# HuiyangYu/TGSFilter

Hardware: AMD Instinct MI355X
Metric: filtered Gbases/sec (end-to-end, excl. gzip I/O) (higher is better)
Workload: dtype u8

## Files before the change

include/tgsf.h:

```cpp
#ifndef TGSF_H
#define TGSF_H

#include <stddef.h>
#include <stdint.h>

#ifdef __cplusplus
extern "C" {
#endif

#define TGSF_ABI_VERSION 3
#define TGSF_MAX_ADAPTERS 32
#define TGSF_MAX_ADAPTER_LEN 8192
#define TGSF_N_DROPINFO 17
#define TGSF_N_QBINS 256
#define TGSF_BIN_WIDTH 100

typedef enum tgsf_status {
    TGSF_OK = 0,
    TGSF_E_INVALID = -1,
    TGSF_E_NO_DEVICE = -2,
    TGSF_E_HIP = -3,
    TGSF_E_CAPACITY = -4,
    TGSF_E_UNSUPPORTED = -5,
    TGSF_E_DATA = -6
} tgsf_status;

typedef struct tgsf_params {
    uint32_t struct_size;
    int32_t  min_len;
    int32_t  max_len;
    float    min_q;
    float    max_q;
    int32_t  bc_len;
    int32_t  head_trim;
    int32_t  tail_trim;
    int32_t  end_len;
    int32_t  end_match_len;
    int32_t  mid_match_len;
    int32_t  extra_len;
    float    end_sim;
    float    mid_sim;
    int32_t  discard;
    int32_t  filter;
    int32_t  only_qc;
    int32_t  min_repeat;
    int32_t  kmer;
    int32_t  qtype;
    int32_t  n_adapters;
    const char* adapters[TGSF_MAX_ADAPTERS];
    int32_t  adapter_len[TGSF_MAX_ADAPTERS];
    uint64_t max_batch_bases;
    uint32_t max_batch_reads;
    uint32_t max_read_len;
    int32_t  no_qual;
    int32_t  reserved;
} tgsf_params;

typedef struct tgsf_batch_in {
    const uint8_t*  seq;
    const uint8_t*  qual;
    const uint64_t* offsets;
    const uint32_t* lengths;
    uint32_t        n_reads;
    uint32_t        reserved;
    uint64_t        n_bytes;
    const uint64_t* qual_offsets;
} tgsf_batch_in;

#define TGSF_RF_LOWQ       0x01u
#define TGSF_RF_AD5P       0x02u
#define TGSF_RF_AD3P       0x04u
#define TGSF_RF_ADMID      0x08u
#define TGSF_RF_DISCARDED  0x10u

typedef struct tgsf_read_result {
    uint64_t sum_q;
    uint32_t flags;
    uint32_t n_frags;
    uint32_t frag_begin;
    uint32_t trimmed;
    int32_t  reserved0;
    int32_t  reserved1;
} tgsf_read_result;

#define TGSF_FF_PASS    0x01u
#define TGSF_FF_REPEAT  0x02u

typedef struct tgsf_fragment {
    uint64_t sum_q;
    uint32_t read;
    int32_t  start;
    int32_t  len;
    uint32_t flags;
} tgsf_fragment;

typedef struct tgsf_batch_out {
    tgsf_read_result* reads;
    tgsf_fragment*    frags;
    uint32_t          frag_capacity;
    uint32_t          n_frags;
} tgsf_batch_out;

#define TGSF_CTR_DROPINFO    0
#define TGSF_CTR_RAW_DIFFQ   17
#define TGSF_CTR_CLEAN_DIFFQ 273
#define TGSF_CTR_ROWS        529
#define TGSF_CTR_END_TABLES  533

enum { TGSF_T_RAW5P_QUAL = 0, TGSF_T_RAW5P_CNT, TGSF_T_RAW3P_QUAL, TGSF_T_RAW3P_CNT,
       TGSF_T_CLEAN5P_QUAL, TGSF_T_CLEAN5P_CNT, TGSF_T_CLEAN3P_QUAL, TGSF_T_CLEAN3P_CNT };
enum { TGSF_B_RAW_QUAL = 0, TGSF_B_RAW_CNT, TGSF_B_CLEAN_QUAL, TGSF_B_CLEAN_CNT };

static inline size_t tgsf_ctr_end_table(int t, int bc_len) {
    return (size_t)TGSF_CTR_END_TABLES + (size_t)t * (size_t)bc_len * 5u;
}
static inline size_t tgsf_ctr_bin_table(int b, int bc_len, uint32_t n_bins) {
    return (size_t)TGSF_CTR_END_TABLES + 8u * (size_t)bc_len * 5u + (size_t)b * (size_t)n_bins * 5u;
}
static inline size_t tgsf_ctr_len(int bc_len, uint32_t n_bins) {
    return tgsf_ctr_bin_table(4, bc_len, n_bins);
}
static inline uint32_t tgsf_n_bins(uint32_t max_read_len) { return max_read_len / TGSF_BIN_WIDTH + 1u; }

typedef struct tgsf_ctx tgsf_ctx;

int tgsf_abi_version(void);

const char* tgsf_backend(void);

int tgsf_prepare_device(int device);

int tgsf_device_location(int device, char* bus_id, int len, int* numa_node);

int tgsf_create(const tgsf_params* params, int device, tgsf_ctx** out_ctx);
void tgsf_destroy(tgsf_ctx* ctx);

int tgsf_submit(tgsf_ctx* ctx, const tgsf_batch_in* in, tgsf_batch_out* out);
int tgsf_submit_async(tgsf_ctx* ctx, const tgsf_batch_in* in, tgsf_batch_out* out);

#define TGSF_MAX_ENQUEUED 64
#define TGSF_NFRAGS_NOT_FINAL 0xFFFFFFFFu
int tgsf_submit_device(tgsf_ctx* ctx, const tgsf_batch_in* in, tgsf_batch_out* out,
                       uint32_t* d_n_frags, void* hip_stream);

int tgsf_wait(tgsf_ctx* ctx);

int tgsf_counters_len(tgsf_ctx* ctx, uint64_t* n_words, int32_t* bc_len, uint32_t* n_bins);
int tgsf_counters(tgsf_ctx* ctx, uint64_t* dst, uint64_t n_words);
int tgsf_counters_used(tgsf_ctx* ctx, uint64_t* dst, uint64_t n_words, uint64_t rows[2]);
int tgsf_counters_merge(tgsf_ctx* dst, tgsf_ctx* src);
int tgsf_counters_device(tgsf_ctx* ctx, void** d_ptr, uint64_t* n_words);
int tgsf_reset_counters(tgsf_ctx* ctx);

#define TGSF_N_STAGES 12
int tgsf_profile(tgsf_ctx* ctx, int enable);
int tgsf_stage_times(tgsf_ctx* ctx, float ms[TGSF_N_STAGES], uint32_t* n_batches);
const char* tgsf_stage_name(int stage);

int tgsf_align_windows(tgsf_ctx* ctx, const uint8_t* seq, uint64_t n_bytes,
                       const uint64_t* win_off, const uint32_t* win_len,
                       const uint8_t* adapter_id, const int32_t* k, uint32_t n,
                       int32_t* res, int32_t* ends);

const char* tgsf_last_error(tgsf_ctx* ctx);

#ifdef __cplusplus
}
#endif
#endif
```

tgsfilter_amd/capi.py:

```python
from __future__ import annotations

import ctypes as C
import os

import numpy as np

from . import abi

_HERE = os.path.dirname(os.path.abspath(__file__))
DEFAULT_LIB = os.path.join(_HERE, "libtgsf.so")
_LIBS = {}

SYMBOLS = [
    "tgsf_abi_version", "tgsf_backend", "tgsf_prepare_device", "tgsf_device_location", "tgsf_create", "tgsf_destroy", "tgsf_submit", "tgsf_submit_async", "tgsf_submit_device",
    "tgsf_wait",
    "tgsf_counters_len", "tgsf_counters", "tgsf_counters_used", "tgsf_counters_merge", "tgsf_counters_device", "tgsf_reset_counters", "tgsf_profile",
    "tgsf_stage_times", "tgsf_stage_name", "tgsf_align_windows", "tgsf_last_error",
]


class TgsfError(RuntimeError):
    def __init__(self, code, msg):
        super().__init__(f"tgsf error {code}: {msg}")
        self.code = code


def load(path: str | None = None):
    explicit = path is not None
    path = path or os.environ.get("TGSF_LIB") or DEFAULT_LIB
    if path in _LIBS:
        if not explicit and not _LIBS[path].tgsf_backend().startswith(b"hip"):
            raise RuntimeError(f"{path} is not the HIP build of libtgsf (there is no CPU fallback; is TGSF_LIB set by accident?)")
        return _LIBS[path]
    if not os.path.exists(path):
        raise FileNotFoundError(
            f"{path} not found: build the HIP extension first (python -c 'import __graft_entry__ as g; g.build()')")
    L = C.CDLL(path)
    vp, u32, u64, i32 = C.c_void_p, C.c_uint32, C.c_uint64, C.c_int32
    L.tgsf_abi_version.restype = C.c_int
    L.tgsf_backend.restype = C.c_char_p
    L.tgsf_prepare_device.argtypes = [C.c_int]
    L.tgsf_device_location.argtypes = [C.c_int, C.c_char_p, C.c_int, C.POINTER(C.c_int)]
    L.tgsf_create.argtypes = [C.POINTER(abi.Params), C.c_int, C.POINTER(vp)]
    L.tgsf_destroy.argtypes = [vp]
    L.tgsf_destroy.restype = None
    L.tgsf_submit.argtypes = [vp, C.POINTER(abi.BatchIn), C.POINTER(abi.BatchOut)]
    L.tgsf_submit_async.argtypes = [vp, C.POINTER(abi.BatchIn), C.POINTER(abi.BatchOut)]
    L.tgsf_submit_device.argtypes = [vp, C.POINTER(abi.BatchIn), C.POINTER(abi.BatchOut), vp, vp]
    L.tgsf_wait.argtypes = [vp]
    L.tgsf_counters_len.argtypes = [vp, C.POINTER(u64), C.POINTER(i32), C.POINTER(u32)]
    L.tgsf_counters.argtypes = [vp, vp, u64]
    L.tgsf_counters_used.argtypes = [vp, vp, u64, vp]
    L.tgsf_counters_merge.argtypes = [vp, vp]
    L.tgsf_counters_device.argtypes = [vp, C.POINTER(vp), C.POINTER(u64)]
    L.tgsf_reset_counters.argtypes = [vp]
    L.tgsf_profile.argtypes = [vp, C.c_int]
    L.tgsf_stage_times.argtypes = [vp, C.POINTER(C.c_float * abi.N_STAGES), C.POINTER(u32)]
    L.tgsf_stage_name.argtypes = [C.c_int]
    L.tgsf_stage_name.restype = C.c_char_p
    L.tgsf_align_windows.argtypes = [vp, vp, u64, vp, vp, vp, vp, u32, vp, vp]
    L.tgsf_last_error.argtypes = [vp]
    L.tgsf_last_error.restype = C.c_char_p
    if L.tgsf_abi_version() != abi.ABI_VERSION:
        raise RuntimeError("libtgsf ABI version mismatch")
    if not explicit and not L.tgsf_backend().startswith(b"hip"):
        raise RuntimeError(f"{path} is the {L.tgsf_backend().decode()!r} build of libtgsf, not the HIP build "
                           "(there is no CPU fallback; is TGSF_LIB set by accident?)")
    _LIBS[path] = L
    return L


class Context:

    def __init__(self, params: abi.Params, device: int = 0, lib_path: str | None = None):
        self.lib = load(lib_path)
        self.params = params
        h = C.c_void_p()
        rc = self.lib.tgsf_create(C.byref(params), device, C.byref(h))
        if rc != 0:
            raise TgsfError(rc, self.lib.tgsf_last_error(None).decode())
        self.h = h
        nw, bc, nb = C.c_uint64(), C.c_int32(), C.c_uint32()
        self._chk(self.lib.tgsf_counters_len(self.h, C.byref(nw), C.byref(bc), C.byref(nb)))
        self.ctr_words, self.bc_len, self.n_bins = nw.value, bc.value, nb.value

    def _chk(self, rc):
        if rc != 0:
            raise TgsfError(rc, self.lib.tgsf_last_error(self.h).decode())

    def close(self):
        if getattr(self, "h", None):
            self.lib.tgsf_destroy(self.h)
            self.h = None

    def __del__(self):
        try:
            self.close()
        except Exception:
            pass

    def submit(self, seq, qual, offsets, lengths=None, frag_capacity=None, qual_offsets=None):
        self.submit_async(seq, qual, offsets, lengths, frag_capacity, qual_offsets)
        return self.wait_result()

    def submit_async(self, seq, qual, offsets, lengths=None, frag_capacity=None, qual_offsets=None):
        seq = np.ascontiguousarray(seq, dtype=np.uint8)
        qual = np.ascontiguousarray(qual, dtype=np.uint8)
        offsets = np.ascontiguousarray(offsets, dtype=np.uint64)
        if lengths is not None:
            lengths = np.ascontiguousarray(lengths, dtype=np.uint32)
            n = len(lengths)
            total = int(lengths.sum())
        else:
            n = len(offsets) - 1
            total = int(offsets[-1] - offsets[0])
        if frag_capacity is None:
            frag_capacity = total // 100 + n + 16
        reads = np.zeros(n, dtype=abi.READ_RESULT_DTYPE)
        frags = np.zeros(frag_capacity, dtype=abi.FRAGMENT_DTYPE)
        if qual_offsets is not None:
            qual_offsets = np.ascontiguousarray(qual_offsets, dtype=np.uint64)
        same = qual is seq or (qual.ctypes.data == seq.ctypes.data)
        bi = abi.BatchIn(seq.ctypes.data, seq.ctypes.data if same else qual.ctypes.data, offsets.ctypes.data,
                         lengths.ctypes.data if lengths is not None else None, n, 0, seq.size,
                         qual_offsets.ctypes.data if qual_offsets is not None else None)
        bo = abi.BatchOut(reads.ctypes.data, frags.ctypes.data, frag_capacity, 0)
        self._pending = (reads, frags, bi, bo, seq, qual, offsets, lengths, qual_offsets)
        rc = self.lib.tgsf_submit_async(self.h, C.byref(bi), C.byref(bo))
        if rc != 0:
            self._pending = None
            self._chk(rc)

    def wait_result(self):
        pend, self._pending = self._pending, None
        if pend is None:
            raise RuntimeError("no batch pending")
        self._chk(self.lib.tgsf_wait(self.h))
        reads, frags, _, bo = pend[:4]
        return reads, frags[:bo.n_frags].copy()

    def submit_device(self, d_seq, d_qual, d_offsets, d_lengths, n_reads, n_bytes, d_reads, d_frags,
                      frag_capacity, d_nfrags=None, stream=None, d_qual_offsets=None):
        bi = abi.BatchIn(d_seq, d_qual, d_offsets, d_lengths, n_reads, 0, n_bytes, d_qual_offsets)
        bo = abi.BatchOut(d_reads, d_frags, frag_capacity, 0)
        self._chk(self.lib.tgsf_submit_device(self.h, C.byref(bi), C.byref(bo), d_nfrags, stream))

    def wait(self):
        self._chk(self.lib.tgsf_wait(self.h))

    def counters(self) -> np.ndarray:
        out = np.zeros(self.ctr_words, dtype=np.uint64)
        self._chk(self.lib.tgsf_counters(self.h, out.ctypes.data, self.ctr_words))
        return out

    def counters_used(self, out=None, with_rows=True):
        if out is None:
            out = np.zeros(self.ctr_words, dtype=np.uint64)
        rows = (C.c_uint64 * 2)()
        self._chk(self.lib.tgsf_counters_used(self.h, out.ctypes.data, out.size, rows if with_rows else None))
        return out, ((rows[0], rows[1]) if with_rows else None)

    def merge_from(self, other: "Context"):
        self._chk(self.lib.tgsf_counters_merge(self.h, other.h))

    def counters_device_ptr(self):
        p, n = C.c_void_p(), C.c_uint64()
        self._chk(self.lib.tgsf_counters_device(self.h, C.byref(p), C.byref(n)))
        return p.value, n.value

    def reset_counters(self):
        self._chk(self.lib.tgsf_reset_counters(self.h))

    def profile(self, enable=True):
        self._chk(self.lib.tgsf_profile(self.h, int(enable)))

    def stage_times(self):
        arr = (C.c_float * abi.N_STAGES)()
        nb = C.c_uint32()
        self._chk(self.lib.tgsf_stage_times(self.h, C.byref(arr), C.byref(nb)))
        names = [self.lib.tgsf_stage_name(i).decode() for i in range(abi.N_STAGES)]
        return dict(zip(names, list(arr))), nb.value

    def align_windows(self, seq: bytes, win_off, win_len, adapter_id, k):
        seq = np.frombuffer(seq, dtype=np.uint8) if isinstance(seq, (bytes, bytearray)) else np.ascontiguousarray(seq, np.uint8)
        win_off = np.ascontiguousarray(win_off, dtype=np.uint64)
        win_len = np.ascontiguousarray(win_len, dtype=np.uint32)
        adapter_id = np.ascontiguousarray(adapter_id, dtype=np.uint8)
        k = np.ascontiguousarray(k, dtype=np.int32)
        n = len(win_off)
        res = np.zeros((n, 4), dtype=np.int32)
        ends = np.zeros((n, 2), dtype=np.int32)
        self._chk(self.lib.tgsf_align_windows(self.h, seq.ctypes.data, seq.size, win_off.ctypes.data,
                                              win_len.ctypes.data, adapter_id.ctypes.data, k.ctypes.data, n,
                                              res.ctypes.data, ends.ctypes.data))
        return res, ends
```

tgsfilter_amd/csrc/tgsf_emul.h:

```cpp
#pragma once
#include <stdint.h>
#include <string.h>

#define TGSF_HD inline
#define TGSF_D inline
#define TGSF_KERNEL static void
#define TGSF_INLINE_LAMBDA
#define TGSF_BOUNDS(threads, waves_per_simd)
#define TGSF_SHARED static thread_local
#define TGSF_BLOCK_SYNC() ((void)0)
#define TGSF_WAVE_SYNC() ((void)0)
#define TGSF_COOP_BEGIN 0u
#define TGSF_COOP_STRIDE 1u
#define TGSF_WCOOP_BEGIN(lane) 0u
#define TGSF_WCOOP_STRIDE 1u
#define TGSF_ON_DEVICE(...)
#define TGSF_ON_EMUL(...) __VA_ARGS__
constexpr bool kTgsfEmul = true;
#define TGSF_WAVE_PRIO(p) ((void)0)

struct alignas(16) uint4 { uint32_t x, y, z, w; };
namespace tgsf_emul {
struct Dim3 { unsigned x, y, z; };
extern thread_local Dim3 threadIdx, blockIdx, blockDim, gridDim;
}
using tgsf_emul::threadIdx; using tgsf_emul::blockIdx; using tgsf_emul::blockDim; using tgsf_emul::gridDim;
template <class T> static inline T atomicAdd(T* p, T v) { T o = *p; *p = o + v; return o; }
template <class T> static inline T atomicMax(T* p, T v) { T o = *p; if (v > o) *p = v; return o; }
template <class T> static inline T atomicMin(T* p, T v) { T o = *p; if (v < o) *p = v; return o; }
template <class T> static inline T atomicExch(T* p, T v) { T o = *p; *p = v; return o; }
template <class T> static inline T atomicOr(T* p, T v) { T o = *p; *p = o | v; return o; }
template <class T> static inline T atomicCAS(T* p, T cmp, T v) { T o = *p; if (o == cmp) *p = v; return o; }

namespace tgsf {

TGSF_HD uint32_t popc32(uint32_t x) { return (uint32_t)__builtin_popcount(x); }
TGSF_HD uint32_t popc64(uint64_t x) { return (uint32_t)__builtin_popcountll(x); }
TGSF_HD uint32_t udot4(uint32_t a, uint32_t b, uint32_t c) {
    uint32_t s = c;
    for (int i = 0; i < 4; i++) s += ((a >> (8 * i)) & 0xFF) * ((b >> (8 * i)) & 0xFF);
    return s;
}
TGSF_HD uint32_t alignbyte(uint32_t hi, uint32_t lo, uint32_t sh) { return (uint32_t)((((uint64_t)hi << 32) | lo) >> (8 * sh)); }
TGSF_HD uint32_t alignbit(uint32_t hi, uint32_t lo, uint32_t sh) { return (uint32_t)((((uint64_t)hi << 32) | lo) >> (sh & 31u)); }
TGSF_HD uint32_t perm_bytes(uint32_t hi, uint32_t lo, uint32_t sel) {
    uint64_t v = ((uint64_t)hi << 32) | lo;
    uint32_t r = 0;
    for (int i = 0; i < 4; i++) r |= (uint32_t)((v >> (8 * ((sel >> (8 * i)) & 7u))) & 0xFF) << (8 * i);
    return r;
}
template <int TT>
TGSF_HD uint32_t bitop3(uint32_t a, uint32_t b, uint32_t c) {
    uint32_t r = 0;
    for (int i = 0; i < 32; i++) {
        const int idx = (int)(((a >> i) & 1u) << 2 | ((b >> i) & 1u) << 1 | ((c >> i) & 1u));
        r |= (uint32_t)((TT >> idx) & 1) << i;
    }
    return r;
}
TGSF_HD void pin(uint64_t&) {}
TGSF_HD void pin(uint32_t&) {}
struct QcConsts { uint32_t k[4]; };
TGSF_HD QcConsts qc_consts() { return QcConsts{{0x41414141u, 0x54545454u, 0x47474747u, 0x43434343u}}; }
TGSF_HD uint32_t xad7f(uint32_t x7, uint32_t k) { return (x7 ^ k) + 0x7F7F7F7Fu; }
TGSF_HD uint4 load16u(const uint8_t* p) { uint4 v; memcpy(&v, p, 16); return v; }

TGSF_HD uint64_t wave_sum(uint64_t v) { return v; }
TGSF_HD int32_t wave_sum_i32(int32_t v) { return v; }
TGSF_HD uint32_t wave_max(uint32_t v) { return v; }
TGSF_HD uint32_t wave_or(uint32_t v) { return v; }
TGSF_HD bool wave_leader() { return true; }
TGSF_HD bool wave_any(bool b) { return b; }
TGSF_HD uint32_t wave_bcast(uint32_t v, uint32_t) { return v; }
TGSF_HD uint32_t wave_pick(uint32_t v, uint32_t) { return v; }

}
```

tgsfilter_amd/csrc/tgsf_hip.h:

```cpp
#pragma once
#include <hip/hip_runtime.h>
#include <stdint.h>

#define TGSF_HD __host__ __device__ __forceinline__
#define TGSF_D __device__ __forceinline__
#define TGSF_KERNEL __global__ void
#define TGSF_INLINE_LAMBDA __attribute__((always_inline))
#define TGSF_BOUNDS(threads, waves_per_simd) __launch_bounds__(threads, waves_per_simd)
#define TGSF_SHARED __shared__
#define TGSF_BLOCK_SYNC() __syncthreads()
#define TGSF_WAVE_SYNC() do { __builtin_amdgcn_fence(__ATOMIC_SEQ_CST, "wavefront"); __builtin_amdgcn_wave_barrier(); } while (0)
#define TGSF_COOP_BEGIN threadIdx.x
#define TGSF_COOP_STRIDE blockDim.x
#define TGSF_WCOOP_BEGIN(lane) (lane)
#define TGSF_WCOOP_STRIDE 64u
#define TGSF_ON_DEVICE(...) __VA_ARGS__
#define TGSF_ON_EMUL(...)
constexpr bool kTgsfEmul = false;
#define TGSF_WAVE_PRIO(p) __builtin_amdgcn_s_setprio(p)

namespace tgsf {

TGSF_HD uint32_t popc32(uint32_t x) { return (uint32_t)__builtin_popcount(x); }
TGSF_HD uint32_t popc64(uint64_t x) { return (uint32_t)__builtin_popcountll(x); }
TGSF_D uint32_t udot4(uint32_t a, uint32_t b, uint32_t c) { return __builtin_amdgcn_udot4(a, b, c, false); }
TGSF_D uint32_t alignbyte(uint32_t hi, uint32_t lo, uint32_t sh) { return __builtin_amdgcn_alignbyte(hi, lo, sh); }
TGSF_D uint32_t alignbit(uint32_t hi, uint32_t lo, uint32_t sh) { return __builtin_amdgcn_alignbit(hi, lo, sh); }
TGSF_D uint32_t perm_bytes(uint32_t hi, uint32_t lo, uint32_t sel) { return __builtin_amdgcn_perm(hi, lo, sel); }
template <int TT>
TGSF_D uint32_t bitop3(uint32_t a, uint32_t b, uint32_t c) { return __builtin_amdgcn_bitop3_b32(a, b, c, TT); }
TGSF_D void pin(uint64_t& v) { asm volatile("" : "+v"(v)); }
TGSF_D void pin(uint32_t& v) { asm volatile("" : "+v"(v)); }
struct QcConsts { uint32_t k[4]; };
TGSF_D QcConsts qc_consts() {
    QcConsts c;
    asm volatile("v_mov_b32 %0, 0x41414141" : "=v"(c.k[0]));
    asm volatile("v_mov_b32 %0, 0x54545454" : "=v"(c.k[1]));
    asm volatile("v_mov_b32 %0, 0x47474747" : "=v"(c.k[2]));
    asm volatile("v_mov_b32 %0, 0x43434343" : "=v"(c.k[3]));
    return c;
}
TGSF_D uint32_t xad7f(uint32_t x7, uint32_t k) {
    uint32_t t;
    const uint32_t c7f = 0x7F7F7F7Fu;
    asm("v_xad_u32 %0, %1, %2, %3" : "=v"(t) : "v"(x7), "v"(k), "s"(c7f));
    return t;
}
struct __attribute__((packed, aligned(1))) U4u { uint32_t x, y, z, w; };
TGSF_D uint4 load16u(const uint8_t* p) { const U4u* q = reinterpret_cast<const U4u*>(p); return make_uint4(q->x, q->y, q->z, q->w); }

TGSF_D uint64_t wave_sum(uint64_t v) {
#pragma unroll
    for (int o = 32; o > 0; o >>= 1) v += __shfl_xor(v, o, 64);
    return v;
}
TGSF_D int32_t wave_sum_i32(int32_t v) {
    v += __builtin_amdgcn_update_dpp(0, v, 0xB1, 0xF, 0xF, false);
    v += __builtin_amdgcn_update_dpp(0, v, 0x4E, 0xF, 0xF, false);
    v += __builtin_amdgcn_update_dpp(0, v, 0x141, 0xF, 0xF, false);
    v += __builtin_amdgcn_update_dpp(0, v, 0x140, 0xF, 0xF, false);
    v += __builtin_amdgcn_update_dpp(0, v, 0x142, 0xA, 0xF, false);
    v += __builtin_amdgcn_update_dpp(0, v, 0x143, 0xC, 0xF, false);
    return __builtin_amdgcn_readlane(v, 63);
}
TGSF_D uint32_t wave_max(uint32_t v) {
#pragma unroll
    for (int o = 32; o > 0; o >>= 1) { uint32_t u = __shfl_xor(v, o, 64); v = u > v ? u : v; }
    return v;
}
TGSF_D uint32_t wave_or(uint32_t v) {
#pragma unroll
    for (int o = 32; o > 0; o >>= 1) v |= __shfl_xor(v, o, 64);
    return v;
}
TGSF_D bool wave_leader() { return (threadIdx.x & 63u) == 0u; }
TGSF_D bool wave_any(bool b) { return __builtin_amdgcn_ballot_w64(b) != 0ull; }
TGSF_D uint32_t wave_bcast(uint32_t v, uint32_t src_lane) { return (uint32_t)__shfl((int)v, (int)src_lane, 64); }
TGSF_D uint32_t wave_pick(uint32_t v, uint32_t src_lane) { return (uint32_t)__builtin_amdgcn_readlane((int)v, (int)src_lane); }

}
```

tgsfilter_amd/csrc/tgsf_kernels.h:

```cpp
#pragma once
#include <type_traits>
#include "tgsf_dev.h"
#include "../../include/tgsf.h"
static_assert(TGSF_CTR_END_TABLES == 533, "tally layout");

namespace tgsf {

typedef unsigned long long ull;

TGSF_D void wave_add_u64(uint64_t* dst, uint64_t v) {
    uint64_t t = wave_sum(v);
    if (wave_leader() && t) atomicAdd((ull*)dst, (ull)t);
}
TGSF_D void wave_max_u64(uint64_t* dst, uint32_t v) {
    uint32_t t = wave_max(v);
    if (wave_leader() && t) atomicMax((ull*)dst, (ull)t);
}
TGSF_D void set_status(const DevBatch& B, uint32_t code, uint32_t detail) {
    if (atomicMax(&B.status[0], code) < code) B.status[1] = detail;
}

TGSF_D bool pool_overflowed(const DevBatch& B) { return *B.ovf != 0u; }

TGSF_D uint32_t stored_frags(const DevBatch& B) { uint32_t nf = B.nfr[B.n]; return nf < B.fcap ? nf : B.fcap; }
// ... 2075 lines not shown
    uint32_t f = next_s;
    prefetch(f);
    while (f < nf) {
        const uint4* base; int a, L;
        chunks_of(f, base, a, L);
        const int total = L - k + 1;
        const int words = (a + L + 15) / 16;
        const int kwords = total > 0 ? (a + total + 15) / 16 : 0;
        const bool one_window = words <= W;
        TGSF_BLOCK_SYNC();
        if (tid == 0) { over_s = 0; next_s = take(); }
        TGSF_BLOCK_SYNC();
        if (kTgsfEmul) load_window(base, words, 0);
        else {
#pragma unroll
            for (int sl = 0; sl < kRepSlots; sl++) { const int g = tid + sl * NT; if (g < words) codes[g] = base_codes16(raw[sl]); }
            if (tid < 8) codes[(words < W ? words : W) + tid] = 0;
        }
        TGSF_BLOCK_SYNC();
        const uint32_t fnext = next_s;
        prefetch(fnext);
        bool drop = false;
        if (total <= 0) {
            drop = 0 < P.min_repeat;
        } else if (k >= 32) {
            ull first = 0;
            const uint8_t* seq = B.seq + B.frag_off[f];
            for (int i = 0; i < k; i++) first = (first << 2) | base_code(seq[i]);
            const int distinct = (total > 1 && first != 0ull) ? 2 : 1;
            drop = total - distinct < P.min_repeat;
        } else {
            uint32_t plog = 0;
            uint32_t rot = 19u;
            while (plog < 20u && ((uint32_t)total >> plog) > kRepShare) plog++;
            for (;;) {
                const uint32_t passes = 1u << plog;
                uint32_t repeat = 0;
                uint32_t flagged = 0;
                bool decided = false;
                for (uint32_t pass = 0; pass < passes && !decided; pass++) {
                    uint32_t c0 = 0, c1 = 0;
                    auto scan = [&](auto phase_tag, auto multi_tag) TGSF_INLINE_LAMBDA {
                        constexpr int PHASE = decltype(phase_tag)::value;
                        constexpr bool MULTI = decltype(multi_tag)::value;
                        auto hash_of = [&](uint32_t x0, uint32_t x1) TGSF_INLINE_LAMBDA -> uint32_t {
                            return KEY64 ? ((x1 & tail_mask) ^ alignbit(x0, x0, rot)) * 0x9E3779B1u : x0 * 0x9E3779B1u;
                        };
                        auto owned = [&](uint32_t h) TGSF_INLINE_LAMBDA -> bool {
                            return !MULTI || ((h ^ (h >> 7)) & (passes - 1u)) == pass;
                        };
                        auto a_word = [&](uint32_t h) TGSF_INLINE_LAMBDA -> uint32_t { return ((h >> 16) * (kRepAQ * 4u)) >> 16; };
                        auto a_mask = [&](uint32_t h) TGSF_INLINE_LAMBDA -> uint32_t {
                            const uint32_t g = h ^ (h >> 15);
                            return (1u << (g & 31u)) | (1u << ((g >> 5) & 31u)) | (1u << ((g >> 10) & 31u));
                        };
                        for (int wb = 0;; wb += W - OV) {
                            if (!one_window) {
                                TGSF_BLOCK_SYNC();
                                load_window(base, words, wb);
                            }
                            TGSF_BLOCK_SYNC();
                            const bool last = wb + W >= words;
                            const int gend = last ? kwords - wb : W - OV;
                            for (int g = tid; g < gend; g += NT) {
                                const uint32_t w0 = codes[g], w1 = codes[g + 1], w2 = codes[g + 2];
                                const int first = a - 16 * (wb + g);
                                const int v = a + total - 16 * (wb + g);
                                uint32_t m = 0x55555555u;
                                if (first <= 0 && v >= 16) {
                                    m = 0;
#pragma unroll
                                    for (int j0 = 0; j0 < 16; j0 += 8) {
                                        uint32_t hv[8], oldv[8], mkv[8];
#pragma unroll
                                        for (int jj = 0; jj < 8; jj++) {
                                            const int j = j0 + jj;
                                            const uint32_t x0 = j ? alignbit(w0, w1, 32u - 2u * (uint32_t)j) : w0;
                                            uint32_t h;
                                            if (KEY64) {
                                                const uint32_t x1 = j ? alignbit(w1, w2, 32u - 2u * (uint32_t)j) : w1;
                                                h = hash_of(x0, x1);
                                            } else {
                                                h = hash_of(x0 >> (32 - kb), 0u);
                                            }
                                            hv[jj] = h;
                                            if (PHASE == 0) {
                                                mkv[jj] = owned(h) ? a_mask(h) : 0u;
                                                oldv[jj] = atomicOr(&Am[a_word(h)], mkv[jj]);
                                            } else {
                                                oldv[jj] = Bm[h >> 19];
                                            }
                                        }
                                        uint32_t hits = 0;
#pragma unroll
                                        for (int jj = 0; jj < 8; jj++) {
                                            bool hit;
                                            if (PHASE == 0) hit = (mkv[jj] & ~oldv[jj]) == 0u && (!MULTI || mkv[jj] != 0u);
                                            else hit = ((oldv[jj] >> ((hv[jj] >> 14) & 31u)) & 1u) && owned(hv[jj]);
                                            if (hit) hits |= 1u << (30 - 2 * (j0 + jj));
                                        }
                                        if (PHASE == 0) {
                                            if (hits) {
                                                c0 += popc32(hits);
#pragma unroll
                                                for (int jj = 0; jj < 8; jj++)
                                                    if (hits & (1u << (30 - 2 * (j0 + jj)))) atomicOr(&Bm[hv[jj] >> 19], 1u << ((hv[jj] >> 14) & 31u));
                                            }
                                        } else {
                                            m |= hits;
                                        }
                                    }
                                } else {
                                    if (first > 0) m &= 0xFFFFFFFFu >> (2 * first);
                                    if (v < 16) m &= ~(0xFFFFFFFFu >> (2 * v));
                                }
                                while (m) {
                                    const int b = __builtin_ctz(m);
                                    m &= m - 1u;
                                    const uint32_t sb = (uint32_t)(30 - b);
                                    const uint32_t x0 = sb ? alignbit(w0, w1, 32u - sb) : w0;
                                    key_t key;
                                    uint32_t lo32, hi32 = 0, h;
                                    if (KEY64) {
                                        const uint32_t x1 = sb ? alignbit(w1, w2, 32u - sb) : w1;
                                        const ull k64 = (((ull)x0 << 32) | x1) >> (64 - kb);
                                        key = (key_t)k64;
                                        lo32 = (uint32_t)k64; hi32 = (uint32_t)(k64 >> 32);
                                        h = hash_of(x0, x1);
                                    } else {
                                        lo32 = x0 >> (32 - kb);
                                        key = (key_t)lo32;
                                        h = hash_of(lo32, 0u);
                                    }
                                    if (!owned(h)) continue;
                                    const uint32_t bbit = 1u << ((h >> 14) & 31u);
                                    if (PHASE == 0) {
                                        const uint32_t mk = a_mask(h);
                                        const uint32_t old = atomicOr(&Am[a_word(h)], mk);
                                        if ((mk & ~old) == 0u) { c0++; atomicOr(&Bm[h >> 19], bbit); }
                                    } else if (Bm[h >> 19] & bbit) {
                                        c0++;
                                        uint32_t slot = (((lo32 * 0xC2B2AE35u) ^ (hi32 * 0x27D4EB2Fu) ^ (lo32 >> 15)) * 0x165667B1u) >> (32u - TLOG);
                                        for (int probes = 0;; probes++) {
                                            const key_t old = atomicCAS(&tab[slot], kEmpty, key);
                                            if (old == kEmpty) { c1++; break; }
                                            if (old == key) break;
                                            if (probes >= 64) { over_s = 1; break; }
                                            slot = (slot + 1u) & ((1u << TLOG) - 1u);
                                        }
                                    }
                                }
                            }
                            if (last) break;
                        }
                    };
                    if (tid == 0) acc_s[0] = acc_s[1] = acc_s[2] = 0;
                    if (plog == 0) scan(std::integral_constant<int, 0>(), std::false_type());
                    else scan(std::integral_constant<int, 0>(), std::true_type());
                    TGSF_BLOCK_SYNC();
                    flagged = block_sum(c0, 0);
                    const bool skip = flagged == 0 || (pass + 1 == passes && repeat + flagged < (uint32_t)P.min_repeat);
                    if (skip) {
                        if (flagged) repeat += flagged;
                        TGSF_BLOCK_SYNC();
                        clear_maps(flagged != 0);
                        TGSF_BLOCK_SYNC();
                        continue;
                    }
                    for (uint32_t w = (uint32_t)tid; w < kRepTabQ; w += (uint32_t)NT) A4[w] = ones4;
                    c0 = c1 = 0;
                    if (plog == 0) scan(std::integral_constant<int, 1>(), std::false_type());
                    else scan(std::integral_constant<int, 1>(), std::true_type());
                    TGSF_BLOCK_SYNC();
                    const uint32_t occ = block_sum(c0, 1), ins = block_sum(c1, 2);
                    clear_maps(true);
                    TGSF_BLOCK_SYNC();
                    if (over_s) break;
                    repeat += occ - ins;
                    if (repeat >= (uint32_t)P.min_repeat) decided = true;
                }
                if (!over_s) { drop = !decided && repeat < (uint32_t)P.min_repeat; break; }
                TGSF_BLOCK_SYNC();
                if (tid == 0) over_s = 0;
                uint32_t want = plog + 1u;
                while (want < B.rep_max_plog && (flagged >> (want - plog)) > (1u << (TLOG - 1u))) want++;
                if (plog >= B.rep_max_plog) {
                    const uint32_t distinct = rep_distinct_in_memory(B, B.seq + B.frag_off[f], total, k, tid, NT, &acc_s[0]);
                    drop = (uint32_t)total - distinct < (uint32_t)P.min_repeat;
                    break;
                }
                plog = want;
                rot = (rot + 6u) & 31u;
                TGSF_BLOCK_SYNC();
            }
        }
        if (tid == 0 && drop) {
            B.frag_flags[f] |= TGSF_FF_REPEAT;
            drop_n++; drop_b += (uint64_t)L;
        }
        f = fnext;
    }
    if (tid == 0 && drop_n) {
        atomicAdd((ull*)&B.ctr[TGSF_CTR_DROPINFO + 15], (ull)drop_n);
        atomicAdd((ull*)&B.ctr[TGSF_CTR_DROPINFO + 16], (ull)drop_b);
    }
}

TGSF_KERNEL k_gate_frags(DevParams P, DevBatch B)
{
    if (pool_overflowed(B)) return;
    TGSF_SHARED ull hq[TGSF_N_QBINS];
    for (uint32_t i = TGSF_COOP_BEGIN; i < (uint32_t)TGSF_N_QBINS; i += TGSF_COOP_STRIDE) hq[i] = 0;
    TGSF_BLOCK_SYNC();
    const uint32_t nf = stored_frags(B);
    const bool diff = clean_by_difference(B);
    uint64_t lq_n = 0, lq_b = 0;
    uint32_t erows = 0;
    for (uint32_t f0 = blockIdx.x * blockDim.x; f0 < nf; f0 += gsize()) {
        const uint32_t f = f0 + threadIdx.x;
        if (f >= nf || (B.frag_flags[f] & TGSF_FF_REPEAT)) continue;
        const uint32_t L = B.frag_len[f];
        if (diff && B.whole[B.frag_read[f]]) B.frag_sum[f] = clean_by_product(B) ? B.spec_sum[B.frag_read[f]] : B.sumq[B.frag_read[f]];
        const double cm = mean_q(B.frag_sum[f], L);
        if (!P.no_qual) {
            if (P.filter && q_fail(cm, P.min_q, P.max_q)) { lq_n++; lq_b += L; continue; }
            if (!(cm >= 0.0 && cm < 256.0)) { set_status(B, DS_BAD_MEANQ, B.frag_read[f]); continue; }
            atomicAdd(&hq[(int)cm], (ull)L);
        }
        B.frag_flags[f] = TGSF_FF_PASS;
        uint32_t er = (uint32_t)P.bc_len < L ? (uint32_t)P.bc_len : L;
        erows = er > erows ? er : erows;
    }
    wave_add_u64(&B.ctr[TGSF_CTR_DROPINFO + 13], lq_n);
    wave_add_u64(&B.ctr[TGSF_CTR_DROPINFO + 14], lq_b);
    wave_max_u64(&B.ctr[TGSF_CTR_ROWS + 3], erows);
    TGSF_BLOCK_SYNC();
    for (uint32_t i = TGSF_COOP_BEGIN; i < (uint32_t)TGSF_N_QBINS; i += TGSF_COOP_STRIDE)
        if (hq[i]) atomicAdd((ull*)&B.ctr[TGSF_CTR_CLEAN_DIFFQ + i], hq[i]);
}

TGSF_KERNEL k_ctr_merge(uint64_t* dst, const uint64_t* src, uint64_t n)
{
    for (uint64_t i = gtid(); i < n; i += gsize()) {
        const uint64_t a = dst[i], b = src[i];
        dst[i] = (i >= TGSF_CTR_ROWS && i < TGSF_CTR_ROWS + 4) ? (a > b ? a : b) : a + b;
    }
}

TGSF_KERNEL k_finalize(DevBatch B, tgsf_read_result* out_reads, tgsf_fragment* out_frags,
                       uint32_t out_fcap, uint32_t* out_nfrags)
{
    if (pool_overflowed(B)) {
        if (gtid() == 0 && out_nfrags) *out_nfrags = TGSF_NFRAGS_NOT_FINAL;
        return;
    }
    const uint32_t nf = B.nfr[B.n];
    if (gtid() == 0) {
        if (out_nfrags) *out_nfrags = nf;
        if (nf > out_fcap) set_status(B, DS_FRAG_CAP, nf);
    }
    for (uint32_t r = gtid(); r < B.n; r += gsize()) {
        tgsf_read_result o;
        o.sum_q = B.sumq[r];
        o.flags = B.flags[r];
        o.n_frags = B.nfr[r + 1] - B.nfr[r];
        o.frag_begin = B.nfr[r];
        o.trimmed = B.trimmed[r];
        o.reserved0 = 0; o.reserved1 = 0;
        out_reads[r] = o;
    }
    for (uint32_t f = gtid(); f < nf && f < out_fcap; f += gsize()) {
        tgsf_fragment o;
        o.sum_q = B.frag_sum[f];
        o.read = B.frag_read[f];
        o.start = B.frag_start[f];
        o.len = (int32_t)B.frag_len[f];
        o.flags = B.frag_flags[f];
        out_frags[f] = o;
    }
}

template <int MAXNW>
TGSF_KERNEL k_align_windows(DevParams P, DevBatch B, const uint8_t* seq, const uint64_t* win_off, const uint32_t* win_len,
                            const uint8_t* adapter_id, const int32_t* kk, uint32_t n, int32_t* res, int32_t* ends)
{
    const uint32_t i = gtid();
    if (i >= n) return;
    const int a = adapter_id[i];
    const int Q = P.Q[a];
    int k = kk[i];
    if (k > Q) k = Q;
    const LaneScratch sc = lane_scratch(B, 0);
    const uint8_t* t = seq + win_off[i];
    const int T = (int)win_len[i];
    WinAln w = by_length<MAXNW>(Q, [=, &P](auto f) TGSF_INLINE_LAMBDA { return align_window<typename decltype(f)::col>(P, a, t, T, k, 0, sc, true); });
    res[i * 4 + 0] = w.best;
    res[i * 4 + 1] = w.best < 0 ? 0 : w.n;
    res[i * 4 + 2] = w.best < 0 ? 0 : w.mlen + w.best;
    res[i * 4 + 3] = w.best < 0 ? -1 : w.start0;
    ends[i * 2 + 0] = w.best < 0 ? -1 : w.first_end;
    ends[i * 2 + 1] = w.best < 0 ? -1 : w.last_end;
}

}
```

tgsfilter_amd/csrc/tgsf_lib.hip:

```cpp
#include <algorithm>
#include <type_traits>

#include "tgsf_kernels.h"
constexpr size_t kErrorCap = 512;
#include "tgsf_rt.h"
#if defined(TGSF_EMUL)
namespace tgsf_emul { thread_local Dim3 threadIdx, blockIdx, blockDim, gridDim; }
#endif

using namespace tgsf;

static const char* knob(const char* name)
{
    static const bool on = [] { const char* e = getenv("TGSF_DEBUG_KNOBS"); return e && e[0] == '1'; }();
    return on ? getenv(name) : nullptr;
}

struct tgsf_ctx : rt_ctx {
    tgsf_params params;
    std::vector<std::string> adapters;
    DevParams P;
    DevBatch B;
    rt_stream stream;
    rt_stream last_stream;
    bool own_stream;
    uint64_t cap_bases, cap_chunks;
    uint32_t cap_reads, max_read_len, n_bins;
    static constexpr unsigned endtab_grid = 512;
    static constexpr unsigned stats_grid = 768;
    bool flat_scan = true;
    int suffix_filter = 2;
    bool no_hot32 = false;
    uint64_t ctr_words;
    int scratch_cols;
    uint8_t *d_seq, *d_qual;
    uint64_t* d_off;
    uint64_t* d_qoff;
    uint32_t* d_lenin;
    tgsf_read_result* d_out_reads;
    tgsf_fragment* d_out_frags;
    uint32_t* d_out_nfrags;
    bool profile;
    float stage_ms[TGSF_N_STAGES];
    uint32_t prof_batches;
    static constexpr int kProfRing = 64;
    rt_event ev[kProfRing][TGSF_N_STAGES + 1];
    rt_event ev_aux[kProfRing][3];
    int prof_pending;
    rt_stream aux;
    rt_event ev_fork, ev_join;
    uint32_t* h_pinned = nullptr;
    static constexpr size_t kStageBytes = 32u << 20;
    uint8_t* stage[2] = {nullptr, nullptr};
    rt_event stage_ev[2] = {nullptr, nullptr};
    uint32_t h_words_[8];
    uint32_t* h_status;
    uint32_t* pend_nf_p;
    tgsf_batch_out* pend_out = nullptr;
    struct Pending { tgsf_batch_in in; tgsf_read_result* reads; tgsf_fragment* frags; uint32_t fcap; uint32_t* nfrags; rt_stream st; };
    Pending pending[TGSF_MAX_ENQUEUED];
    uint32_t n_pending = 0;
    uint32_t* ovf_ring = nullptr;
    uint32_t* bp_ring = nullptr;
    uint32_t h_ovf[TGSF_MAX_ENQUEUED];
    uint32_t pool_regrown = 0;
};

static const int kMaxLenParam = 1 << 28;
static void adapter_rules(const tgsf_params& p, DevParams& P)
{
    P.max_nw = 1;
    P.min_Q = 1 << 30;
    for (int a = 0; a < p.n_adapters; a++) {
        const int Q = p.adapter_len[a];
        P.Q[a] = Q;
        if (Q > 64 && P.max_nw < 2) P.max_nw = 2;
        if (Q > 128 && P.max_nw < 4) P.max_nw = 4;
        if (Q > 256) P.max_nw = kWideNW;
        if (Q < P.min_Q) P.min_Q = Q;
        int km = Q - p.mid_match_len + 1;
        int ke = Q - p.end_match_len + 1;
        P.k_mid[a] = km > Q - 1 ? Q - 1 : km;
        P.k_end[a] = ke > Q - 1 ? Q - 1 : ke;
        const float w = (float)Q / p.end_sim;
        P.w5[a] = p.end_len + (w < (float)kMaxLenParam ? (int)w : kMaxLenParam);
        P.need_end[a] = P.need_mid[a] = Q + 1;
        for (int m = Q; m >= 0; m--) {
            if (m >= p.end_match_len && (float)m / (float)Q >= p.end_sim) P.need_end[a] = m;
            if (m >= p.mid_match_len && (float)m / (float)Q >= p.mid_sim) P.need_mid[a] = m;
        }
    }
}

static void fill_peq(const std::vector<std::string>& adapters, size_t slots, int W, std::vector<uint64_t>& fwd, std::vector<uint64_t>& rev)
{
    const size_t per_ad = (size_t)256 * W;
    fwd.assign(slots * per_ad, 0);
    rev.assign(slots * per_ad, 0);
    for (size_t a = 0; a < adapters.size(); a++) {
        const std::string& s = adapters[a];
        const int Q = (int)s.size();
        for (int r = 0; r < Q && r < 64 * W; r++) {
            const uint8_t cf = (uint8_t)s[r], cr = (uint8_t)s[Q - 1 - r];
            fwd[a * per_ad + (size_t)cf * W + (r >> 6)] |= 1ull << (r & 63);
            rev[a * per_ad + (size_t)cr * W + (r >> 6)] |= 1ull << (r & 63);
        }
    }
}

static int build_tables(tgsf_ctx* c)
{
    DevParams& P = c->P;
    const int A = c->params.n_adapters;
    std::vector<uint8_t> ad((size_t)kMaxAdapters * kMaxQ, 0);
    std::vector<uint64_t> fwd, rev, top((size_t)kMaxAdapters * 256, 0);
    fill_peq(c->adapters, kMaxAdapters, kPeqW, fwd, rev);
    for (int a = 0; a < A; a++) {
        const int Q = P.Q[a];
        memcpy(&ad[(size_t)a * kMaxQ], c->adapters[a].data(), (size_t)Q);
        if (Q <= 64) {
            const int sh = 64 - Q;
            const uint64_t pad = sh ? ((1ull << sh) - 1ull) : 0ull;
            for (int sym = 0; sym < 256; sym++)
                top[(size_t)a * 256 + sym] = (fwd[((size_t)a * 256 + sym) * kPeqW] << sh) | pad;
        }
    }
    uint8_t* d_ad; uint64_t *d_f, *d_r, *d_t;
    int e;
    if ((e = dev_alloc(c, &d_ad, ad.size()))) return e;
    if ((e = dev_alloc(c, &d_f, fwd.size()))) return e;
    if ((e = dev_alloc(c, &d_r, rev.size()))) return e;
    if ((e = dev_alloc(c, &d_t, top.size()))) return e;
    rt_h2d(d_ad, ad.data(), ad.size(), c->stream);
    rt_h2d(d_f, fwd.data(), fwd.size() * 8, c->stream);
    rt_h2d(d_r, rev.data(), rev.size() * 8, c->stream);
    rt_h2d(d_t, top.data(), top.size() * 8, c->stream);
    rt_sync(c->stream);
    P.adapter = d_ad; P.peq_fwd = d_f; P.peq_rev = d_r; P.peq_top = d_t;
    P.peq_fwd_w = P.peq_rev_w = nullptr;
    if (P.max_nw > 4) {
        fill_peq(c->adapters, (size_t)A, kWideNW, fwd, rev);
        uint64_t *d_fw, *d_rw;
        if ((e = dev_alloc(c, &d_fw, fwd.size()))) return e;
        if ((e = dev_alloc(c, &d_rw, rev.size()))) return e;
        rt_h2d(d_fw, fwd.data(), fwd.size() * 8, c->stream);
        rt_h2d(d_rw, rev.data(), rev.size() * 8, c->stream);
        rt_sync(c->stream);
        P.peq_fwd_w = d_fw; P.peq_rev_w = d_rw;
    }
    return 0;
}

extern "C" int tgsf_abi_version(void) { return TGSF_ABI_VERSION; }
extern "C" const char* tgsf_backend(void) { return kTgsfEmul ? "emulation" : "hip:gfx950"; }

#if !defined(TGSF_EMUL)
__global__ void k_noop(int* p) { if (p) *p = 0; }
static void set_wait_mode(int device)
{
    const char* e = getenv("TGSF_SYNC");
    if (!e || strcmp(e, "blocking") != 0) return;
    if (hipSetDevice(device) == hipSuccess) { (void)hipSetDeviceFlags(hipDeviceScheduleBlockingSync); (void)hipGetLastError(); }
}
#endif
extern "C" int tgsf_prepare_device(int device)
{
#if !defined(TGSF_EMUL)
    int ndev = 0;
    if (hipGetDeviceCount(&ndev) != hipSuccess || device < 0 || device >= ndev) return TGSF_E_NO_DEVICE;
    set_wait_mode(device);
    if (hipSetDevice(device) != hipSuccess) return TGSF_E_HIP;
    hipLaunchKernelGGL(k_noop, dim3(1), dim3(64), 0, 0, (int*)nullptr);
    if (hipDeviceSynchronize() != hipSuccess) return TGSF_E_HIP;
    {
        static const char a0[] = "GTTTTCGCATTTATCGTGAAACGCTTTCGCGTTTTTCGTGCGCCGCTTCA";
        static const char a1[] = "TGAAGCGGCGCACGAAAAACGCGAAAGCGTTTCACGATAAATGCGAAAAC";
        tgsf_params p;
        memset(&p, 0, sizeof p);
        p.struct_size = sizeof p;
        p.min_len = 100; p.max_len = 2147483647; p.min_q = 0; p.max_q = 255; p.bc_len = 150;
        p.end_len = 150; p.end_match_len = 4; p.mid_match_len = 35; p.extra_len = 50;
        p.end_sim = 0.75f; p.mid_sim = 0.9f; p.filter = 1; p.qtype = 33; p.kmer = 11;
        p.n_adapters = 2; p.adapters[0] = a0; p.adapters[1] = a1; p.adapter_len[0] = p.adapter_len[1] = 50;
        p.max_batch_bases = 1 << 16; p.max_batch_reads = 16; p.max_read_len = 1 << 14;
        tgsf_ctx* c = nullptr;
        if (tgsf_create(&p, device, &c) == TGSF_OK) {
            std::vector<uint8_t> seq(8192), qual(8192, (uint8_t)'5');
            for (size_t i = 0; i < seq.size(); i++) seq[i] = "ACGT"[(i * 2654435761u >> 13) & 3];
            memcpy(&seq[4096 + 1000], a0, 50);
            const uint64_t off[2] = {0, 4096};
            const uint32_t len[2] = {3000, 4000};
            tgsf_read_result res[2];
            tgsf_fragment fr[64];
            tgsf_batch_in in;
            memset(&in, 0, sizeof in);
            in.seq = seq.data(); in.qual = qual.data(); in.offsets = off; in.lengths = len; in.n_reads = 2; in.n_bytes = seq.size();
            tgsf_batch_out out{res, fr, 64, 0};
            (void)tgsf_submit(c, &in, &out);
            tgsf_destroy(c);
        }
    }
#else
    (void)device;
#endif
    return TGSF_OK;
}

extern "C" int tgsf_device_location(int device, char* bus_id, int len, int* numa_node)
{
    if (numa_node) *numa_node = -1;
    if (bus_id && len > 0) bus_id[0] = 0;
#if !defined(TGSF_EMUL)
    int ndev = 0;
    if (hipGetDeviceCount(&ndev) != hipSuccess || device < 0 || device >= ndev) return TGSF_E_NO_DEVICE;
    char id[64] = {0};
    if (hipDeviceGetPCIBusId(id, (int)sizeof id, device) != hipSuccess) return TGSF_E_HIP;
    for (char* p = id; *p; p++) if (*p >= 'A' && *p <= 'F') *p = (char)(*p - 'A' + 'a');
    if (bus_id && len > 0) { strncpy(bus_id, id, (size_t)len - 1); bus_id[len - 1] = 0; }
    if (numa_node) {
        const std::string path = std::string("/sys/bus/pci/devices/") + id + "/numa_node";
        if (FILE* f = fopen(path.c_str(), "r")) {
            int v = -1;
            if (fscanf(f, "%d", &v) == 1) *numa_node = v;
            fclose(f);
        }
    }
    return TGSF_OK;
#else
    if (bus_id && len > 0) snprintf(bus_id, (size_t)len, "emul:%d", device);
    if (numa_node)
        if (const char* e = knob("TGSF_EMUL_NUMA")) {
            int k = 0;
            for (const char* c = e; *c; k++) {
                if (k == device) { *numa_node = atoi(c); break; }
                while (*c && *c != ',') c++;
                if (*c == ',') c++;
            }
        }
    return TGSF_OK;
#endif
}

extern "C" const char* tgsf_last_error(tgsf_ctx* ctx) { return ctx ? ctx->error.c_str() : g_create_error.c_str(); }

extern "C" void tgsf_destroy(tgsf_ctx* c)
{
    if (!c) return;
    if (c->B.bp_allowed && c->B.bp_state && knob("TGSF_TRACE_BP")) {
        uint32_t w[4] = {0, 0, 0, 0};
        uint64_t pl[4] = {0, 0, 0, 0};
        uint32_t sg[4] = {0, 0, 0, 0};
        if (!rt_d2h(w, c->B.bp_state, sizeof w, c->stream) && !rt_d2h(pl, c->B.plan, sizeof pl, c->stream) && !rt_d2h(sg, c->B.seg_info, sizeof sg, c->stream) && !rt_sync(c->stream))
            fprintf(stderr, "tgsf: clean tables as a by-product of the raw pass: %u batches speculated; the next would%s; the last batch: %llu bases a direct clean pass scans, "
                            "%llu bases its own did, %u work items in that pass\n", w[1], w[0] ? "" : " not", (unsigned long long)pl[2], (unsigned long long)pl[3], sg[2]);
    }
    if (c->stream) { (void)rt_set_device(c->device); (void)rt_sync(c->stream); }
    for (int k = 0; k < tgsf_ctx::kProfRing; k++) {
        for (rt_event e : c->ev[k]) rt_event_destroy(e);
        for (rt_event e : c->ev_aux[k]) rt_event_destroy(e);
    }
    if (c->h_pinned) rt_host_free(c->h_pinned);
    for (int i = 0; i < 2; i++) {
        if (c->stage[i]) rt_host_free(c->stage[i]);
        rt_event_destroy(c->stage_ev[i]);
    }
    rt_event_destroy(c->ev_fork);
    rt_event_destroy(c->ev_join);
    if (c->aux) rt_stream_destroy(c->aux);
    if (c->own_stream && c->stream) rt_stream_destroy(c->stream);
    dev_free_all(c);
    delete c;
}

static int check_params(const tgsf_params* p)
{
    if (p->struct_size != sizeof(tgsf_params))
        return fail(nullptr, TGSF_E_INVALID, "tgsf_params.struct_size %u != %zu (ABI mismatch)", p->struct_size, sizeof(tgsf_params));
    if (p->n_adapters < 0 || p->n_adapters > TGSF_MAX_ADAPTERS)
        return fail(nullptr, TGSF_E_INVALID, "n_adapters %d outside [0,%d]", p->n_adapters, TGSF_MAX_ADAPTERS);
    if (p->min_repeat > 0 && (p->kmer < 1 || p->kmer > 32))
        return fail(nullptr, TGSF_E_UNSUPPORTED, "kmer (-k) %d: the repeat gate supports k-mer sizes 1..32 (the reference's k-mers are 64 bits)", p->kmer);
    if (p->min_len < 0) return fail(nullptr, TGSF_E_INVALID, "min_len (-l) %d: must be >= 0", p->min_len);
    if (p->end_len > kMaxLenParam) return fail(nullptr, TGSF_E_INVALID, "end_len (-E) %d: must be <= 2^28", p->end_len);
    if (p->extra_len > kMaxLenParam) return fail(nullptr, TGSF_E_INVALID, "extra_len (-T) %d: must be <= 2^28", p->extra_len);
    if (p->qtype != 33 && p->qtype != 64) return fail(nullptr, TGSF_E_INVALID, "qtype must be 33 or 64");
    if (p->bc_len < 0 || p->bc_len > kMaxBcLenTotal) return fail(nullptr, TGSF_E_INVALID, "bc_len (-e) outside [0,%d]", kMaxBcLenTotal);
    if (p->filter && p->n_adapters > 0) {
        if (!(p->end_sim > 0.f)) return fail(nullptr, TGSF_E_INVALID, "end_sim must be > 0");
        if (!(p->mid_sim > 0.f)) return fail(nullptr, TGSF_E_INVALID, "mid_sim must be > 0");
        if (p->end_len < 0) return fail(nullptr, TGSF_E_INVALID, "end_len must be >= 0");
        if (p->extra_len < 0) return fail(nullptr, TGSF_E_INVALID, "extra_len must be >= 0");
        if (p->end_match_len < 1) return fail(nullptr, TGSF_E_INVALID, "end_match_len must be >= 1");
        if (p->mid_match_len < 1) return fail(nullptr, TGSF_E_INVALID, "mid_match_len must be >= 1");
    }
    for (int a = 0; a < p->n_adapters; a++) {
        if (!p->adapters[a] || p->adapter_len[a] < 1 || p->adapter_len[a] > TGSF_MAX_ADAPTER_LEN)
            return fail(nullptr, TGSF_E_UNSUPPORTED, "adapter %d: length %d outside [1,%d]", a, p->adapter_len[a], TGSF_MAX_ADAPTER_LEN);
    }
    if (!p->max_batch_bases) return fail(nullptr, TGSF_E_INVALID, "max_batch_bases must be set");
    if (!p->max_batch_reads) return fail(nullptr, TGSF_E_INVALID, "max_batch_reads must be set");
    if (!p->max_read_len) return fail(nullptr, TGSF_E_INVALID, "max_read_len must be set");
    if (p->max_read_len > (1u << 28)) return fail(nullptr, TGSF_E_INVALID, "max_read_len above 2^28");
    return TGSF_OK;
}

struct Sizing {
    DevBatch B;
    uint64_t cap_bytes, cap_chunks;
    size_t nitems, scratch_waves;
    int scratch_cols, seg_cols, suffix_filter;
    bool flat_scan, no_hot32;
};

static Sizing size_context(const tgsf_params& p, const DevParams& P)
{
    Sizing S;
    DevBatch& B = S.B;
    memset(&B, 0, sizeof B);
    S.seg_cols = kSegCols; S.no_hot32 = false; S.flat_scan = true; S.suffix_filter = 2;
    if (const char* e = knob("TGSF_NO_HOT32")) S.no_hot32 = atoi(e) > 0;
    if (const char* e = knob("TGSF_SEG_COLS")) { int v = atoi(e); if (v >= 256 && v <= 65536) S.seg_cols = v & ~15; }
    if (const char* e = knob("TGSF_MID_FLAT")) S.flat_scan = atoi(e) > 0;
    if (const char* e = knob("TGSF_MID_FILTER")) { int v = atoi(e); if (v >= 0 && v <= 2) S.suffix_filter = v; }
    B.flat_pmax = 256; B.flat_pmin = 16; B.flat_f0 = 224;
    if (const char* e = knob("TGSF_FLAT_PMIN")) { int v = atoi(e); if (v >= 1 && v <= (1 << 20)) B.flat_pmin = (uint32_t)v; }
    if (const char* e = knob("TGSF_FLAT_PMAX")) { int v = atoi(e); if (v >= 1 && v <= (1 << 20)) B.flat_pmax = (uint32_t)v; }
    if (const char* e = knob("TGSF_FLAT_F0")) { int v = atoi(e); if (v >= 0 && v <= 256) B.flat_f0 = (uint32_t)v; }
    B.flat_pmin = 1u << flat_log2(B.flat_pmin); B.flat_pmax = 1u << flat_log2(B.flat_pmax);
    if (B.flat_pmax < B.flat_pmin) B.flat_pmax = B.flat_pmin;
    const uint64_t cap_bases = p.max_batch_bases;
    const size_t n = p.max_batch_reads;
    const int A = p.n_adapters > 0 ? p.n_adapters : 1;
    S.cap_bytes = cap_bases + 16ull * n + 64;
    const int min_len = p.min_len > 0 ? p.min_len : 1;
    uint64_t fcap64 = p.filter ? (cap_bases / (uint64_t)min_len + 16) : (uint64_t)n + 16;
    if (fcap64 > cap_bases + 16) fcap64 = cap_bases + 16;
    if (fcap64 < n + 16 && !p.filter) fcap64 = n + 16;
    B.fcap = (uint32_t)std::min<uint64_t>(fcap64, 0x7FFFFFF0ull);
    B.max_tiles = (p.max_read_len + kTileBases - 1) / kTileBases;
    uint64_t pool = cap_bases / 64 + 65536 + (uint64_t)n * 16u * (uint64_t)A;
    B.pool_cap = (uint32_t)std::min<uint64_t>(pool, 1ull << 28);
    if (const char* e = knob("TGSF_POOL_CAP")) { const long long v = atoll(e); if (v >= 1 && v < (1ll << 28)) B.pool_cap = (uint32_t)v; }
    S.nitems = n + (size_t)B.fcap;
    S.cap_chunks = cap_bases / 16u + 2ull * n;
    if (S.cap_chunks >= 0xFFFFFFF0ull) S.flat_scan = false;
    if (S.cap_chunks >= (1ull << 30) || !S.flat_scan) S.suffix_filter = 0;
    bool any = false;
    for (int a = 0; a < p.n_adapters; a++) any |= P.Q[a] > 32 && P.Q[a] <= 64 && P.k_mid[a] >= 0 && P.k_mid[a] <= kSuffixMaxK;
    if (!any || !p.filter) S.suffix_filter = 0;
    if (S.suffix_filter) {
        B.rc_cap = (uint32_t)std::min<uint64_t>(S.cap_chunks / 25u + 4096u, 1ull << 24);
        if (const char* e = knob("TGSF_RECHECK_CAP")) { int v = atoi(e); if (v >= 0) B.rc_cap = (uint32_t)v; }
    }
    B.rep_long_cap = (uint32_t)std::min<uint64_t>((cap_bases + 16ull * n) / kRepShare + 16, (uint64_t)B.fcap + 16);
    if (p.min_repeat > 0 && p.kmer >= 12 && p.kmer <= 31) {
        B.rep_tab_log2 = 4;
        while (B.rep_tab_log2 < 40 && (1ull << B.rep_tab_log2) < 2ull * p.max_read_len) B.rep_tab_log2++;
        B.rep_max_plog = kRepMaxPlog;
        if (const char* e = knob("TGSF_REP_MAX_PLOG")) { int v = atoi(e); if (v >= 0 && v <= 20) B.rep_max_plog = (uint32_t)v; }
    }
    B.work_cap = (uint32_t)std::min<uint64_t>(2 * (cap_bases / kTileBases) + S.nitems + 16, 0x7FFFFFF0ull);
    B.clean_force = p.only_qc ? 1u : 0u;
    B.bp_allowed = (p.filter && !p.only_qc && (p.head_trim > 0 || p.tail_trim > 0) &&
                    p.head_trim >= 0 && p.tail_trim >= 0) ? 1u : 0u;
    static_assert(kTileBases < (1 << 13), "staged bytes of a tile fit the work list's 13 bits");
    if (const char* f = knob("TGSF_CLEAN_TABLES")) {
        if (!strcmp(f, "direct")) { B.clean_force = 1; B.bp_allowed = 0; }
        else if (!strcmp(f, "difference") && !p.only_qc) { B.clean_force = 2; B.bp_allowed = 0; }
        else if (!strcmp(f, "byproduct") && B.bp_allowed) B.clean_force = 3;
    }
    int maxcols = 1;
    for (int a = 0; a < p.n_adapters; a++) {
        int kmax = std::max(std::max(P.k_end[a], P.k_mid[a]), 0);
        maxcols = std::max(maxcols, P.Q[a] + std::min(P.Q[a], kmax) + 1);
    }
    S.scratch_cols = maxcols;
    int col_words = P.max_nw;
    if (P.max_nw > 4) { col_words = 1; for (int a = 0; a < p.n_adapters; a++) col_words = std::max(col_words, (P.Q[a] + 63) / 64); }
    size_t lane_words = (size_t)(maxcols + 1) * 2 * (size_t)col_words;
    if (P.max_nw > 4) lane_words = std::min<size_t>(lane_words, (1u << 17) + 2 * (size_t)col_words) + 4 * (size_t)col_words + 64;
    B.scratch_wave_words = lane_words * 64;
    B.scratch_mid_wave0 = ((size_t)n * A * 2 + 63) / 64 + 1;
    S.scratch_waves = B.scratch_mid_wave0 + ((size_t)n * A + 63) / 64 + 1;
    return S;
}

static int bring_up(tgsf_ctx* c)
{
    c->h_status = c->h_words_; c->pend_nf_p = c->h_words_ + 4;
#if !defined(TGSF_EMUL)
    int ndev = 0;
    hipError_t he = hipGetDeviceCount(&ndev);
    if (he != hipSuccess || ndev <= 0)
        return fail(nullptr, TGSF_E_NO_DEVICE, "no HIP device available (%s); libtgsf has no CPU fallback", hipGetErrorString(he));
    if (c->device < 0 || c->device >= ndev) return fail(nullptr, TGSF_E_NO_DEVICE, "device %d out of range (%d devices)", c->device, ndev);
    set_wait_mode(c->device);
    if ((he = hipSetDevice(c->device)) != hipSuccess) return fail(nullptr, TGSF_E_HIP, "hipSetDevice: %s", hipGetErrorString(he));
    if ((he = hipStreamCreateWithFlags(&c->stream, hipStreamNonBlocking)) != hipSuccess) return fail(nullptr, TGSF_E_HIP, "hipStreamCreate: %s", hipGetErrorString(he));
    c->own_stream = true;
    uint32_t* pw = nullptr;
    if (hipHostMalloc((void**)&pw, 64, hipHostMallocDefault) == hipSuccess && pw) {
        memset(pw, 0, 64);
        c->h_pinned = pw; c->h_status = pw; c->pend_nf_p = pw + 4;
    }
    int lo = 0, hi = 0;
    (void)hipDeviceGetStreamPriorityRange(&lo, &hi);
    he = hipStreamCreateWithPriority(&c->aux, hipStreamNonBlocking, hi);
    if (he != hipSuccess ||
        (he = hipEventCreateWithFlags(&c->ev_fork, hipEventDisableTiming)) != hipSuccess ||
        (he = hipEventCreateWithFlags(&c->ev_join, hipEventDisableTiming)) != hipSuccess)
        return fail(nullptr, TGSF_E_HIP, "auxiliary stream: %s", hipGetErrorString(he));
    if (c->params.max_batch_bases > (8u << 20)) {
        for (int i = 0; i < 2; i++)
            if (hipHostMalloc((void**)&c->stage[i], tgsf_ctx::kStageBytes, hipHostMallocDefault) != hipSuccess ||
                hipEventCreateWithFlags(&c->stage_ev[i], hipEventDisableTiming) != hipSuccess)
                return fail(nullptr, TGSF_E_HIP, "pinned staging buffers: allocation failed");
    }
#endif
    c->last_stream = c->stream;
    return TGSF_OK;
}

static int allocate(tgsf_ctx* c, const Sizing& S)
{
    DevBatch& B = c->B;
    const size_t n = c->cap_reads;
    const int A = std::max(c->params.n_adapters, 1);
    const size_t tiles = 2 * ((size_t)B.max_tiles + 2);
    int e = 0;
    if (!e) e = dev_alloc(c, &c->d_seq, S.cap_bytes);
    if (!e) e = dev_alloc(c, &c->d_qual, S.cap_bytes);
    if (!e) e = dev_alloc(c, &c->d_off, n + 1);
    if (!e) e = dev_alloc(c, &c->d_qoff, n + 1);
    if (!e) e = dev_alloc(c, &c->d_lenin, n);
    if (!e) e = dev_alloc(c, &B.len, n);
    if (!e) e = dev_alloc(c, &B.sumq, n);
    if (!e) e = dev_alloc(c, &B.flags, n);
    if (!e) e = dev_alloc(c, &B.clip5, n * A);
    if (!e) e = dev_alloc(c, &B.clip3, n * A);
    if (!e) e = dev_alloc(c, &B.mid_head, n);
    if (!e) e = dev_alloc(c, &B.mid_best, n * A);
    if (!e) e = dev_alloc(c, &B.mid_cnt, n);
    if (!e) e = dev_alloc(c, &B.mid_gate, n * A);
    if (!e) e = dev_alloc(c, &B.pool, (size_t)B.pool_cap);
    if (!e) e = dev_alloc(c, &B.pool_n, 4);
    if (!e) e = dev_alloc(c, &B.seg_cnt, n + 1);
    if (!e) e = dev_alloc(c, &B.chk_cnt, n + 1);
    if (c->suffix_filter) {
        if (!e) e = dev_alloc(c, &B.chk_mark, (size_t)4 * (size_t)(S.cap_chunks / 32u + 8u));
        if (!e) e = dev_alloc(c, &B.rc_list, (size_t)B.rc_cap + 1);
        if (!e) e = dev_alloc(c, &B.rc_n, 4);
    }
    if (!e) e = dev_alloc(c, &B.nfr, n + 1);
    if (!e) e = dev_alloc(c, &B.scan_part, n / kScanTile + 2);
    if (!e) e = dev_alloc(c, &B.trimmed, n);
    if (!e) e = dev_alloc(c, &B.rep_next, 2 + (size_t)B.rep_long_cap);
    if (B.rep_tab_log2) {
        if (!e) e = dev_alloc(c, &B.rep_tab, (size_t)1 << B.rep_tab_log2);
        if (!e) e = dev_alloc(c, &B.rep_lock, 4);
        if (!e) rt_memset(B.rep_lock, 0, 16, c->stream);
    }
    if (!e) e = dev_alloc(c, &B.tile_hist, tiles);
    if (!e) e = dev_alloc(c, &B.tile_cnt, tiles);
    if (!e) e = dev_alloc(c, &B.tile_base, tiles);
    if (!e) e = dev_alloc(c, &B.tile_fill, tiles);
    if (!e) e = dev_alloc(c, &B.seg_info, 4);
    if (!e) e = dev_alloc(c, &B.perm, S.nitems);
    if (!e) e = dev_alloc(c, &B.work, 2 * (size_t)B.work_cap);
    if (!e) e = dev_alloc(c, &B.frag_off, (size_t)B.fcap);
    if (!e) e = dev_alloc(c, &B.frag_qoff, (size_t)B.fcap);
    if (!e) e = dev_alloc(c, &B.frag_len, (size_t)B.fcap);
    if (!e) e = dev_alloc(c, &B.frag_sum, (size_t)B.fcap);
    if (!e) e = dev_alloc(c, &B.frag_read, (size_t)B.fcap);
    if (!e) e = dev_alloc(c, &B.frag_start, (size_t)B.fcap);
    if (!e) e = dev_alloc(c, &B.frag_flags, (size_t)B.fcap);
    if (!e) e = dev_alloc(c, &B.raw_tab, 2 * (size_t)c->n_bins * 5);
    if (!e) e = dev_alloc(c, &B.whole, n);
    if (!e) e = dev_alloc(c, &B.plan, 4);
    if (B.bp_allowed) {
        if (!e) e = dev_alloc(c, &B.spec, n);
        if (!e) e = dev_alloc(c, &B.spec_sum, n);
        if (!e) e = dev_alloc(c, &B.bp_state, 4);
        if (!e) e = dev_alloc(c, &c->bp_ring, TGSF_MAX_ENQUEUED);
    }
    if (!e) e = dev_alloc(c, &B.scratch, S.scratch_waves * B.scratch_wave_words);
    if (!e) e = dev_alloc(c, &B.ctr, (size_t)c->ctr_words);
    if (!e) e = dev_alloc(c, &B.status, 4);
    if (!e) e = dev_alloc(c, &c->ovf_ring, TGSF_MAX_ENQUEUED);
    if (!e) e = dev_alloc(c, &c->d_out_reads, n);
    if (!e) e = dev_alloc(c, &c->d_out_frags, (size_t)B.fcap);
    if (!e) e = dev_alloc(c, &c->d_out_nfrags, 4);
    if (e) return e;
    rt_memset(B.ctr, 0, c->ctr_words * 8, c->stream);
    rt_memset(B.status, 0, 16, c->stream);
    rt_memset(c->ovf_ring, 0, TGSF_MAX_ENQUEUED * 4, c->stream);
    B.ovf = c->ovf_ring;
    if (B.bp_allowed) {
        const uint32_t init[4] = {1u, 0u, 0u, 0u};
        rt_memset(c->bp_ring, 0, TGSF_MAX_ENQUEUED * 4, c->stream);
        (void)rt_h2d(B.bp_state, init, sizeof init, c->stream);
        B.bp_used = c->bp_ring;
    }
    rt_memset(B.raw_tab, 0, 2 * (size_t)c->n_bins * 5 * 8, c->stream);
    rt_sync(c->stream);
    return TGSF_OK;
}

extern "C" int tgsf_create(const tgsf_params* p, int device, tgsf_ctx** out)
{
    if (!p || !out) return fail(nullptr, TGSF_E_INVALID, "null argument");
    *out = nullptr;
    int e = check_params(p);
    if (e) return e;
    tgsf_ctx* c = new tgsf_ctx();
    c->alloc_slack = 64;
    c->params = *p;
    c->device = device;
    for (int a = 0; a < p->n_adapters; a++) {
        c->adapters.emplace_back(p->adapters[a], (size_t)p->adapter_len[a]);
        c->params.adapters[a] = c->adapters.back().data();
    }
    DevParams& P = c->P;
    P.min_len = p->min_len; P.max_len = p->max_len; P.min_q = p->min_q; P.max_q = p->max_q;
    P.bc_len = p->bc_len; P.head_trim = p->head_trim; P.tail_trim = p->tail_trim; P.end_len = p->end_len;
    P.end_match_len = p->end_match_len; P.mid_match_len = p->mid_match_len; P.extra_len = p->extra_len;
    P.end_sim = p->end_sim; P.mid_sim = p->mid_sim; P.discard = p->discard; P.filter = p->filter;
    P.only_qc = p->only_qc; P.qtype = p->qtype; P.n_adapters = p->n_adapters;
    P.no_qual = p->no_qual ? 1 : 0;
    P.min_repeat = p->min_repeat; P.kmer = p->kmer;
    c->cap_bases = p->max_batch_bases;
    c->cap_reads = p->max_batch_reads;
    c->max_read_len = p->max_read_len;
    c->n_bins = tgsf_n_bins(p->max_read_len);
    P.n_bins = c->n_bins;
    c->ctr_words = tgsf_ctr_len(p->bc_len, c->n_bins);
    adapter_rules(*p, P);
    const Sizing S = size_context(*p, P);
    c->B = S.B; c->cap_chunks = S.cap_chunks; c->scratch_cols = S.scratch_cols; P.seg_cols = S.seg_cols;
    c->flat_scan = S.flat_scan; c->suffix_filter = S.suffix_filter; c->no_hot32 = S.no_hot32;

    if ((e = bring_up(c)) || (e = build_tables(c)) || (e = allocate(c, S))) {
        if (!c->error.empty()) g_create_error = c->error;
        tgsf_destroy(c);
        return e;
    }
    *out = c;
    return TGSF_OK;
}

static const char* kStageNames[TGSF_N_STAGES] = {
    "prepare+sort", "stats_raw", "gate_reads", "end_tables_raw", "end_windows", "mid_scan",
    "mid_resolve", "regions", "repeat_gate", "stats_clean", "gate_frags+end_tables_clean", "finalize"};

extern "C" const char* tgsf_stage_name(int s) { return (s >= 0 && s < TGSF_N_STAGES) ? kStageNames[s] : ""; }

static unsigned blocks_for(uint64_t n, unsigned block) { return (unsigned)std::max<uint64_t>(1, (n + block - 1) / block); }

static int harvest_profile(tgsf_ctx* c, rt_stream st)
{
    if (!c->prof_pending) return TGSF_OK;
    const int he = rt_sync(st);
    if (he) return fail(c, TGSF_E_HIP, "stream synchronize failed: %s", rt_errstr(he));
    (void)rt_sync(c->aux);
    for (int k = 0; k < c->prof_pending; k++)
        for (int i = 0; i < TGSF_N_STAGES; i++) {
            float ms = 0.f;
            const int e = (i == 3 || i == 4) ? rt_event_ms(&ms, c->ev_aux[k][i - 3], c->ev_aux[k][i - 2])
                                             : rt_event_ms(&ms, c->ev[k][i], c->ev[k][i + 1]);
            if (!e) c->stage_ms[i] += ms;
        }
    c->prof_pending = 0;
    return TGSF_OK;
}

template <int V> using int_c = std::integral_constant<int, V>;

template <class F>
static void with_width(int max_nw, F&& f)
{
    if (max_nw > 4) f(int_c<kWideNW>());
    else if (max_nw > 2) f(int_c<4>());
    else f(int_c<2>());
}

template <int MAXNA, class F>
static void with_adapters(int na, F&& f)
{
    static_assert(MAXNA == 2 || MAXNA == 4, "a pass takes up to two or up to four adapters");
    if (na == 1) return f(int_c<1>());
    if constexpr (MAXNA == 4) {
        if (na == 3) return f(int_c<3>());
        if (na != 2) return f(int_c<4>());
    }
    f(int_c<2>());
}

static void scan_u32(const DevBatch& B, uint32_t* a, uint32_t n, rt_stream st, uint32_t* part = nullptr)
{
    if (!part) part = B.scan_part;
    const unsigned nb = (n + kScanTile - 1) / kScanTile;
    TGSF_LAUNCH_COOP(k_scan_tiles, nb, 256, st, a, n, part);
    TGSF_LAUNCH_COOP(k_scan_top, 1, 64, st, part, (uint32_t)nb, a + n);
    TGSF_LAUNCH_COOP(k_scan_add, nb, 256, st, a, n, (const uint32_t*)part);
}

static int drain_pending(tgsf_ctx* c, bool implicit = false);

struct Run {
    tgsf_ctx* c;
    const tgsf_batch_in* in;
    DevBatch B;
    rt_stream st, ax;
    bool redo, profile;
    rt_event *evs, *evx;
    int stage, A;
    uint32_t n;
    unsigned gsmall, gstats, gfold, gwork, gfr;
    size_t tl;
    bool flat;
    unsigned gflat, gseg;
    uint64_t flat_chunks, max_segs;
};
static constexpr unsigned kBlock = 256;
static_assert(kMidThreads == kBlock, "k_mid_flat / k_mid_scan1 are launched with kBlock lanes a workgroup");

static void stage_mark(Run& r)
{
    if (r.profile) (void)rt_event_record(r.evs[r.stage], r.st);
    r.stage++;
}

static void stage_prepare(Run& r)
{
    const DevParams& P = r.c->P; const DevBatch& B = r.B; const rt_stream st = r.st;
    rt_memset(B.ovf, 0, 4, st);
    rt_memset(B.tile_hist, 0, r.tl, st);
    rt_memset(B.tile_fill, 0, r.tl, st);
    rt_memset(B.pool_n, 0, 4, st);
    rt_memset(B.plan, 0, 32, st);
    TGSF_LAUNCH(k_prepare, r.gsmall, kBlock, st, P, B, r.c->max_read_len);
    TGSF_LAUNCH_COOP(k_tile_scan, 1, 64, st, B, B.bp_allowed ? 2u : 1u);
    TGSF_LAUNCH(k_tile_scatter<false>, r.gsmall, kBlock, st, P, B);
    TGSF_LAUNCH(k_build_work<false>, r.gwork, kBlock, st, P, B);
}

static void stage_raw_stats(Run& r)
{
    const DevParams& P = r.c->P; const DevBatch& B = r.B; const rt_stream st = r.st;
    if (B.bp_allowed) {
        TGSF_LAUNCH((k_stats<false, true, true>), r.gstats, 64 * kStatsWaves, st, P, B);
        if (P.tail_trim > 0) TGSF_LAUNCH(k_tail_fix, grid_cap(std::min(blocks_for(r.n, 1024), 128u)), 1024, st, P, B);
    } else TGSF_LAUNCH((k_stats<false, true>), r.gstats, 64 * kStatsWaves, st, P, B);
    if (!r.redo) TGSF_LAUNCH(k_fold_raw<false>, r.gfold, kBlock, st, P, B);
}

static void stage_fork_ends(Run& r)
{
    tgsf_ctx* c = r.c;
    const DevParams& P = c->P; const DevBatch& B = r.B; const rt_stream ax = r.ax;
    (void)rt_event_record(c->ev_fork, r.st);
    (void)rt_stream_wait(ax, c->ev_fork);
    if (r.profile) (void)rt_event_record(r.evx[0], ax);
    for (uint32_t slab = 0; !r.redo && slab * (uint32_t)kMaxBcLen < (uint32_t)P.bc_len; slab++)
        TGSF_LAUNCH(k_end_tables<false>, grid_cap(c->endtab_grid), 64 * kEndWaves, ax, P, B, slab);
    if (r.profile) (void)rt_event_record(r.evx[1], ax);
    if (P.filter && r.A > 0)
        with_width(P.max_nw, [&](auto nw) { TGSF_LAUNCH(k_end_windows<decltype(nw)::value>, blocks_for((uint64_t)r.n * r.A * 2, 64), 64, ax, P, B); });
    if (r.profile) (void)rt_event_record(r.evx[2], ax);
    (void)rt_event_record(c->ev_join, ax);
}

static void launch_scans(Run& r, uint32_t mode)
{
    tgsf_ctx* c = r.c;
    const DevParams& P = c->P; const rt_stream ms = r.st;
    const int A = r.A;
    DevBatch Bm = r.B;
    Bm.mid_mode = mode;
    int a = 0;
    while (a < A) {
        if (P.Q[a] > 256) { TGSF_LAUNCH(k_mid_scanw<BvW>, r.gseg, kBlock, ms, P, Bm, a); a++; continue; }
        if (P.Q[a] > 192) { TGSF_LAUNCH(k_mid_scanw<Bv<4>>, r.gseg, kBlock, ms, P, Bm, a); a++; continue; }
        if (P.Q[a] > 128) { TGSF_LAUNCH(k_mid_scanw<Bv<3>>, r.gseg, kBlock, ms, P, Bm, a); a++; continue; }
        if (P.Q[a] > 64) { TGSF_LAUNCH(k_mid_scanw<Bv<2>>, r.gseg, kBlock, ms, P, Bm, a); a++; continue; }
        auto cls = [&](int x) {
            if (P.Q[x] <= 32 && !c->no_hot32) return 0;
            if (r.flat && mode == 0 && c->suffix_filter && P.Q[x] > 32 && P.k_mid[x] >= 0 && P.k_mid[x] <= kSuffixMaxK) return 2;
            return 1;
        };
        const int kind = cls(a);
        const bool narrow = kind == 0;
        const int width = narrow ? 2 : 4;
        int na = 0;
        while (a + na < A && na < width && P.Q[a + na] <= 64 && cls(a + na) == kind) na++;
        if (kind == 2) {
            Bm.mark_stride = (uint32_t)((r.flat_chunks / 32u + 7u) & ~3ull);
            rt_memset(Bm.chk_mark, 0, (size_t)na * Bm.mark_stride * 4u, ms);
            rt_memset(Bm.rc_n, 0, 4, ms);
            with_adapters<4>(na, [&](auto nc) {
                constexpr int NA = decltype(nc)::value;
                if (c->suffix_filter == 1) TGSF_LAUNCH((k_mid_flat<NA, Hot32, 1>), r.gflat, kBlock, ms, P, Bm, a, na);
                else TGSF_LAUNCH((k_mid_flat<NA, Hot32, 2>), r.gflat, kBlock, ms, P, Bm, a, na);
            });
            const unsigned grc = grid_cap(blocks_for(r.flat_chunks / 32u + 1u, (unsigned)kRecheckWords));
            TGSF_LAUNCH_COOP(k_mid_marks, grc, kBlock, ms, P, Bm, a, na);
            TGSF_LAUNCH(k_mid_recheck, grid_cap(2048u), kBlock, ms, P, Bm, a, na);
        } else if (r.flat && mode == 0) {
            if (narrow) with_adapters<2>(na, [&](auto nc) { constexpr int NA = decltype(nc)::value; TGSF_LAUNCH((k_mid_flat<NA, Hot32>), r.gflat, kBlock, ms, P, Bm, a, na); });
            else with_adapters<4>(na, [&](auto nc) { constexpr int NA = decltype(nc)::value; TGSF_LAUNCH((k_mid_flat<NA, Hot>), r.gflat, kBlock, ms, P, Bm, a, na); });
        } else {
            if (narrow) with_adapters<2>(na, [&](auto nc) { constexpr int NA = decltype(nc)::value; TGSF_LAUNCH((k_mid_scan1<NA, Hot32>), r.gseg, kBlock, ms, P, Bm, a, na); });
            else with_adapters<4>(na, [&](auto nc) { constexpr int NA = decltype(nc)::value; TGSF_LAUNCH((k_mid_scan1<NA, Hot>), r.gseg, kBlock, ms, P, Bm, a, na); });
        }
        a += na;
    }
}

static void launch_resolve(Run& r, const DevBatch& B)
{
    with_width(r.c->P.max_nw, [&](auto nw) { TGSF_LAUNCH(k_mid_resolve<decltype(nw)::value>, blocks_for((uint64_t)r.n * r.A, 64), 64, r.st, r.c->P, B); });
}

static void stage_mid_scan(Run& r)
{
    tgsf_ctx* c = r.c;
    const DevBatch& B = r.B;
    r.flat = c->flat_scan;
    r.gflat = 1;
    r.flat_chunks = 0;
    scan_u32(B, B.seg_cnt, r.n, r.st);
    if (r.flat) {
        scan_u32(B, B.chk_cnt, r.n, r.st);
        FlatSchedule S;
        r.flat_chunks = std::min<uint64_t>(r.in->n_bytes / 16u + (uint64_t)r.n, c->cap_chunks);
        flat_schedule((uint32_t)r.flat_chunks, B.flat_pmax, B.flat_pmin, B.flat_f0, S);
        r.gflat = grid_cap(blocks_for((uint64_t)S.d0[S.nph] + 128ull * (B.flat_pmax / B.flat_pmin) + 512u, kBlock));
    }
    r.max_segs = r.in->n_bytes / (uint64_t)c->P.seg_cols + 2ull * r.n + 1;
    r.gseg = blocks_for(r.max_segs, kBlock);
    launch_scans(r, 0);
}

static int replay_in_order(Run& r)
{
    tgsf_ctx* c = r.c;
    const DevParams& P = c->P; DevBatch& B = r.B; const rt_stream ms = r.st;
    const int A = r.A;
    const uint64_t cells = r.max_segs * (uint64_t)A + 1;
    if (cells > 0xFFFFFFF0ull) return fail(c, TGSF_E_CAPACITY, "middle scan: too many (segment, adapter) cells for the position-ordered pass");
    uint32_t *seg_n = nullptr, *part = nullptr;
    if (rt_malloc((void**)&seg_n, (size_t)(cells + 1) * 4 + 64) || rt_malloc((void**)&part, (size_t)(cells / kScanTile + 4) * 4 + 64)) {
        if (seg_n) rt_free(seg_n);
        return fail(c, TGSF_E_CAPACITY, "middle scan: no device memory for the position-ordered pass (%.1f GB)", (double)cells * 4e-9);
    }
    B.seg_n = seg_n;
    int rc = TGSF_OK;
    do {
        rt_memset(seg_n, 0, (size_t)(cells + 1) * 4, ms);
        TGSF_LAUNCH(k_mid_reset, r.gsmall, kBlock, ms, B, A);
        launch_scans(r, 1);
        scan_u32(B, seg_n, (uint32_t)cells, ms, part);
        uint32_t need = 0;
        int he = rt_d2h(&need, seg_n + cells, 4, ms);
        if (!he) he = rt_sync(ms);
        if (he) { rc = fail(c, TGSF_E_HIP, "middle scan (counting pass) failed: %s", rt_errstr(he)); break; }
        if (need > B.pool_cap) {
            const uint64_t want = (uint64_t)need + 1024;
            if (want > 0x7FFFFFF0ull) { rc = fail(c, TGSF_E_CAPACITY, "middle-adapter candidates: %u columns tie their reads' minima, more than one batch can list", need); break; }
            void* np = nullptr;
            if (rt_malloc(&np, (size_t)want * sizeof(MidCand) + 64)) {
                rc = fail(c, TGSF_E_CAPACITY, "middle-adapter candidates: no device memory for %llu slots (%.1f GB)", (unsigned long long)want, (double)want * sizeof(MidCand) * 1e-9);
                break;
            }
            for (void*& q : c->allocs) if (q == (void*)c->B.pool) q = np;
            rt_free(c->B.pool);
            c->B.pool = (MidCand*)np; c->B.pool_cap = (uint32_t)want;
            B.pool = c->B.pool; B.pool_cap = c->B.pool_cap;
            c->pool_regrown++;
        }
        if (knob("TGSF_TRACE_POOL"))
            fprintf(stderr, "tgsf: candidate pool overflow (or a read with a long candidate list): %u columns at their reads' minima, pool of %u slots%s; scanning again in position order\n", need, B.pool_cap,
                    c->pool_regrown ? " (grown)" : "");
        rt_memset(B.ovf, 0, 4, ms);
        launch_scans(r, 2);
        TGSF_LAUNCH(k_mid_link, r.gsmall, kBlock, ms, B, A);
        DevBatch Bm = B;
        Bm.mid_mode = 2;
        launch_resolve(r, Bm);
        const unsigned geach = grid_cap(std::min(blocks_for(need, 64), 65536u));
        if (need) with_width(P.max_nw, [&](auto nw) { TGSF_LAUNCH(k_mid_resolve_each<decltype(nw)::value>, geach, 64, ms, P, Bm); });
        he = rt_sync(ms);
        if (he) rc = fail(c, TGSF_E_HIP, "middle scan (position-ordered pass) failed: %s", rt_errstr(he));
    } while (0);
    rt_free(seg_n);
    rt_free(part);
    B.seg_n = nullptr;
    return rc;
}

static void stage_regions(Run& r)
{
    const DevParams& P = r.c->P; const DevBatch& B = r.B; const rt_stream st = r.st;
    (void)rt_stream_wait(st, r.c->ev_join);
    TGSF_LAUNCH(k_regions<false>, r.gsmall, kBlock, st, P, B);
    scan_u32(B, B.nfr, r.n, st);
    TGSF_LAUNCH(k_regions<true>, r.gsmall, kBlock, st, P, B);
}

static void stage_repeat_gate(Run& r)
{
    const DevParams& P = r.c->P; const DevBatch& B = r.B; const rt_stream st = r.st;
    rt_memset(B.rep_next, 0, 2 * sizeof(uint32_t), st);
    if (P.kmer < 12) TGSF_LAUNCH(k_repeat, grid_cap(256u), kRepThreads, st, P, B);
    else {
        TGSF_LAUNCH(k_repeat_long, r.gsmall, kBlock, st, P, B);
        if (P.kmer <= 15) TGSF_LAUNCH(k_repeat_keys<false>, grid_cap(256u), kRepThreads, st, P, B);
        else TGSF_LAUNCH(k_repeat_keys<true>, grid_cap(256u), kRepThreads, st, P, B);
    }
}

static void stage_clean_stats(Run& r)
{
    const DevParams& P = r.c->P; const DevBatch& B = r.B; const rt_stream st = r.st;
    rt_memset(B.tile_hist, 0, r.tl, st);
    rt_memset(B.tile_fill, 0, r.tl, st);
    const unsigned gfr = r.gfr;
    TGSF_LAUNCH(k_clean_plan, r.gsmall, kBlock, st, P, B);
    if (B.bp_allowed && !r.redo) TGSF_LAUNCH(k_clean_plan_next, 1, 64, st, B);
    TGSF_LAUNCH(k_fold_raw<true>, r.gfold, kBlock, st, P, B);
    TGSF_LAUNCH(k_frag_prepare, gfr, kBlock, st, P, B);
    TGSF_LAUNCH_COOP(k_tile_scan, 1, 64, st, B, 2u);
    TGSF_LAUNCH(k_tile_scatter<true>, gfr, kBlock, st, P, B);
    TGSF_LAUNCH(k_build_work<true>, r.gwork, kBlock, st, P, B);
    TGSF_LAUNCH((k_stats<true, true>), r.gstats, 64 * kStatsWaves, st, P, B);
}

static void stage_clean_tables(Run& r)
{
    const DevParams& P = r.c->P; const DevBatch& B = r.B; const rt_stream st = r.st;
    TGSF_LAUNCH(k_gate_frags, r.gfr, kBlock, st, P, B);
    for (uint32_t slab = 0; slab * (uint32_t)kMaxBcLen < (uint32_t)P.bc_len; slab++)
// ... 88 lines not shown
            he |= (int)hipEventRecord(c->stage_ev[k], st);
        }
        return he;
    }
#endif
    (void)c;
    return rt_h2d(dst, src, n, st);
}

static int check_batch(tgsf_ctx* c, const tgsf_batch_in* in)
{
    if (!in || !in->seq || (!in->qual && !c->P.no_qual) || !in->offsets) return fail(c, TGSF_E_INVALID, "null batch pointer");
    if (in->n_reads == 0) return fail(c, TGSF_E_INVALID, "empty batch");
    if (in->n_reads > c->cap_reads) return fail(c, TGSF_E_CAPACITY, "batch has %u reads, context was sized for %u", in->n_reads, c->cap_reads);
    if (in->qual_offsets && !in->lengths) return fail(c, TGSF_E_INVALID, "qual_offsets requires explicit lengths");
    return TGSF_OK;
}

static int check_status(tgsf_ctx* c)
{
    const uint32_t code = c->h_status[0], detail = c->h_status[1];
    if (!code) return TGSF_OK;
    rt_memset(c->B.status, 0, 16, c->stream);
    rt_sync(c->stream);
    switch (code) {
    case DS_BAD_LEN: return fail(c, TGSF_E_DATA, "read %u: length 0 or above max_read_len %u", detail, c->max_read_len);
    case DS_TOO_MANY_REGIONS: return fail(c, TGSF_E_CAPACITY, "read %u has more than %d disjoint drop regions", detail, kMaxRegions);
    case DS_FRAG_CAP: return fail(c, TGSF_E_CAPACITY, "fragment capacity exceeded (%u)", detail);
    case DS_BAD_MEANQ: return fail(c, TGSF_E_DATA, "read %u: mean quality outside [0,256)", detail);
    default: return fail(c, TGSF_E_HIP, "device status %u", code);
    }
}

static int finish_pending(tgsf_ctx* c)
{
    tgsf_batch_out* out = c->pend_out;
    if (!out) return TGSF_OK;
    c->pend_out = nullptr;
    const uint32_t nf = *c->pend_nf_p;
    out->n_frags = nf;
    if (nf > out->frag_capacity || (nf && !out->frags))
        return fail(c, TGSF_E_CAPACITY, "batch produced %u fragments, caller provided room for %u", nf, out->frag_capacity);
    if (nf) {
        int he = rt_d2h(out->frags, c->d_out_frags, (size_t)nf * sizeof(tgsf_fragment), c->stream);
        if (!he) he = rt_sync(c->stream);
        if (he) return fail(c, TGSF_E_HIP, "device to host copy failed");
    }
    return TGSF_OK;
}

static int drain_pending(tgsf_ctx* c, bool implicit)
{
    int e = 0;
    const uint32_t np = c->n_pending;
    (void)rt_set_device(c->device);
    if (implicit) e = rt_device_sync();
    for (uint32_t i = 0; i < np && !e && !implicit; i++) {
        bool seen = c->pending[i].st == c->stream;
        for (uint32_t j = 0; j < i && !seen; j++) seen = c->pending[j].st == c->pending[i].st;
        if (!seen) e = rt_sync(c->pending[i].st);
    }
    if (!e) e = rt_sync(c->aux);
    if (!e) e = rt_d2h(c->h_status, c->B.status, 16, c->stream);
    if (!e && np) e = rt_d2h(c->h_ovf, c->ovf_ring, (size_t)np * 4, c->stream);
    if (!e) e = rt_sync(c->stream);
    c->n_pending = 0;
    if (e) { c->pend_out = nullptr; return fail(c, TGSF_E_HIP, "stream synchronize failed: %s", rt_errstr(e)); }
    e = check_status(c);
    if (e) { c->pend_out = nullptr; return e; }
    for (uint32_t i = 0; i < np; i++) {
        if (!c->h_ovf[i]) continue;
        if (implicit) {
            c->pend_out = nullptr;
            return fail(c, TGSF_E_INVALID, "batch %u of the %u enqueued since the last tgsf_wait has to be run again from its inputs (its middle-adapter candidates "
                                           "outgrew the pool) and only tgsf_wait may do that: call tgsf_wait at least every TGSF_MAX_ENQUEUED (%d) batches", i, np, TGSF_MAX_ENQUEUED);
        }
        const tgsf_ctx::Pending pd = c->pending[i];
        e = run_pipeline(c, &pd.in, pd.reads, pd.frags, pd.fcap, pd.nfrags, pd.st, true, i);
        if (!e && c->pend_out && pd.reads == c->d_out_reads) {
            int he = rt_d2h(c->pend_nf_p, c->d_out_nfrags, 4, pd.st);
            he |= rt_d2h(c->pend_out->reads, c->d_out_reads, (size_t)pd.in.n_reads * sizeof(tgsf_read_result), pd.st);
            if (he) e = fail(c, TGSF_E_HIP, "device to host copy failed");
        }
        uint32_t again = 0;
        if (!e) {
            int he = rt_d2h(c->h_status, c->B.status, 16, pd.st);
            if (!he) he = rt_d2h(&again, c->ovf_ring + i, 4, pd.st);
            if (!he) he = rt_sync(pd.st);
            if (!he) he = rt_sync(c->aux);
            if (he) e = fail(c, TGSF_E_HIP, "stream synchronize failed: %s", rt_errstr(he));
        }
        if (!e) e = check_status(c);
        if (!e && again) e = fail(c, TGSF_E_HIP, "middle-adapter candidate pool overflowed again after it was sized to fit");
        if (e) { c->pend_out = nullptr; return e; }
    }
    return TGSF_OK;
}

extern "C" int tgsf_wait(tgsf_ctx* c)
{
    if (!c) return TGSF_E_INVALID;
    const int e = drain_pending(c);
    if (e) return e;
    return finish_pending(c);
}

extern "C" int tgsf_submit_device(tgsf_ctx* c, const tgsf_batch_in* in, tgsf_batch_out* out,
                                  uint32_t* d_n_frags, void* hip_stream)
{
    if (!c) return TGSF_E_INVALID;
    int e = check_batch(c, in);
    if (e) return e;
    if (!out || !out->reads) return fail(c, TGSF_E_INVALID, "null output");
    if (((uintptr_t)in->seq & 15u) || (!c->P.no_qual && ((uintptr_t)in->qual & 15u))) return fail(c, TGSF_E_INVALID, "seq/qual device pointers must be 16-byte aligned");
    if (!in->n_bytes) return fail(c, TGSF_E_INVALID, "n_bytes is 0: a device batch must state the bytes it spans");
    if (in->n_bytes > c->cap_bases + 16ull * c->cap_reads) return fail(c, TGSF_E_CAPACITY, "batch spans %llu bytes, context was sized for %llu bases", (unsigned long long)in->n_bytes, (unsigned long long)c->cap_bases);
    (void)rt_set_device(c->device);
    rt_stream st = hip_stream ? (rt_stream)hip_stream : c->stream;
    return run_pipeline(c, in, out->reads, out->frags, out->frags ? out->frag_capacity : 0u, d_n_frags, st);
}

extern "C" int tgsf_submit_async(tgsf_ctx* c, const tgsf_batch_in* in, tgsf_batch_out* out)
{
    if (!c) return TGSF_E_INVALID;
    if (c->pend_out) return fail(c, TGSF_E_INVALID, "a batch is already pending on this context: call tgsf_wait first");
    int e = check_batch(c, in);
    if (e) return e;
    if (!out || !out->reads) return fail(c, TGSF_E_INVALID, "null output");
    const uint32_t n = in->n_reads;
    uint64_t span = in->n_bytes;
    if (!span) {
        span = in->lengths ? in->offsets[n - 1] + in->lengths[n - 1] : in->offsets[n];
        if (in->qual_offsets) span = std::max<uint64_t>(span, in->qual_offsets[n - 1] + in->lengths[n - 1]);
    }
    if (span > c->cap_bases + 16ull * c->cap_reads) return fail(c, TGSF_E_CAPACITY, "batch spans %llu bytes, context was sized for %llu bases", (unsigned long long)span, (unsigned long long)c->cap_bases);
    (void)rt_set_device(c->device);
    rt_stream st = c->stream;
    int he = 0;
    const bool one_buffer = in->qual == in->seq || c->P.no_qual;
    he |= text_h2d(c, c->d_seq, in->seq, span, st);
    if (!one_buffer) he |= text_h2d(c, c->d_qual, in->qual, span, st);
    he |= rt_h2d(c->d_off, in->offsets, (size_t)(in->lengths ? n : n + 1) * 8, st);
    if (in->lengths) he |= rt_h2d(c->d_lenin, in->lengths, (size_t)n * 4, st);
    if (in->qual_offsets) he |= rt_h2d(c->d_qoff, in->qual_offsets, (size_t)n * 8, st);
    if (he) return fail(c, TGSF_E_HIP, "host to device copy failed");
    tgsf_batch_in din = *in;
    din.seq = c->d_seq; din.qual = one_buffer ? c->d_seq : c->d_qual; din.offsets = c->d_off;
    din.lengths = in->lengths ? c->d_lenin : nullptr;
    din.qual_offsets = in->qual_offsets ? c->d_qoff : nullptr;
    din.n_bytes = span;
    e = run_pipeline(c, &din, c->d_out_reads, c->d_out_frags, c->B.fcap, c->d_out_nfrags, st);
    if (e) return e;
    *c->pend_nf_p = 0;
    he |= rt_d2h(c->pend_nf_p, c->d_out_nfrags, 4, st);
    he |= rt_d2h(out->reads, c->d_out_reads, (size_t)n * sizeof(tgsf_read_result), st);
    if (he) return fail(c, TGSF_E_HIP, "device to host copy failed");
    c->pend_out = out;
    return TGSF_OK;
}

extern "C" int tgsf_submit(tgsf_ctx* c, const tgsf_batch_in* in, tgsf_batch_out* out)
{
    const int e = tgsf_submit_async(c, in, out);
    return e ? e : tgsf_wait(c);
}

extern "C" int tgsf_counters_len(tgsf_ctx* c, uint64_t* n_words, int32_t* bc_len, uint32_t* n_bins)
{
    if (!c) return TGSF_E_INVALID;
    if (n_words) *n_words = c->ctr_words;
    if (bc_len) *bc_len = c->P.bc_len;
    if (n_bins) *n_bins = c->n_bins;
    return TGSF_OK;
}

extern "C" int tgsf_counters(tgsf_ctx* c, uint64_t* dst, uint64_t n_words)
{
    if (!c || !dst) return TGSF_E_INVALID;
    if (n_words < c->ctr_words) return fail(c, TGSF_E_CAPACITY, "counter buffer too small");
    int e = tgsf_wait(c);
    if (e) return e;
    int he = rt_d2h(dst, c->B.ctr, c->ctr_words * 8, c->stream);
    if (!he) he = rt_sync(c->stream);
    return he ? fail(c, TGSF_E_HIP, "device to host copy failed") : TGSF_OK;
}

extern "C" int tgsf_counters_used(tgsf_ctx* c, uint64_t* dst, uint64_t n_words, uint64_t rows[2])
{
    if (!c || !dst) return TGSF_E_INVALID;
    if (n_words < c->ctr_words) return fail(c, TGSF_E_CAPACITY, "counter buffer too small");
    int e = tgsf_wait(c);
    if (e) return e;
    const size_t head = tgsf_ctr_bin_table(0, c->P.bc_len, c->n_bins);
    int he = rt_d2h(dst, c->B.ctr, head * 8, c->stream);
    if (!he) he = rt_sync(c->stream);
    if (he) return fail(c, TGSF_E_HIP, "device to host copy failed");
    const uint64_t used[2] = {std::min<uint64_t>(dst[TGSF_CTR_ROWS], c->n_bins), std::min<uint64_t>(dst[TGSF_CTR_ROWS + 1], c->n_bins)};
    for (int b = 0; b < 4 && !he; b++) {
        const size_t at = tgsf_ctr_bin_table(b, c->P.bc_len, c->n_bins);
        const uint64_t r = used[b >> 1];
        if (r) he = rt_d2h(dst + at, c->B.ctr + at, (size_t)r * 5 * 8, c->stream);
    }
    if (!he) he = rt_sync(c->stream);
    if (rows) { rows[0] = used[0]; rows[1] = used[1]; }
    return he ? fail(c, TGSF_E_HIP, "device to host copy failed") : TGSF_OK;
}

extern "C" int tgsf_counters_merge(tgsf_ctx* dst, tgsf_ctx* src)
{
    if (!dst || !src || dst == src) return TGSF_E_INVALID;
    if (dst->ctr_words != src->ctr_words || dst->P.bc_len != src->P.bc_len || dst->device != src->device)
        return fail(dst, TGSF_E_INVALID, "tgsf_counters_merge: the contexts differ in tally layout or device");
    int e = tgsf_wait(src);
    if (e) return fail(dst, e, "%s", src->error.c_str());
    if ((e = tgsf_wait(dst))) return e;
    TGSF_LAUNCH(k_ctr_merge, grid_cap(blocks_for(dst->ctr_words, 256)), 256, dst->stream, dst->B.ctr, (const uint64_t*)src->B.ctr, dst->ctr_words);
    const int he = rt_sync(dst->stream);
    return he ? fail(dst, TGSF_E_HIP, "tgsf_counters_merge failed") : TGSF_OK;
}

extern "C" int tgsf_counters_device(tgsf_ctx* c, void** d_ptr, uint64_t* n_words)
{
    if (!c || !d_ptr) return TGSF_E_INVALID;
    *d_ptr = c->B.ctr;
    if (n_words) *n_words = c->ctr_words;
    return TGSF_OK;
}

extern "C" int tgsf_reset_counters(tgsf_ctx* c)
{
    if (!c) return TGSF_E_INVALID;
    int he = rt_memset(c->B.ctr, 0, c->ctr_words * 8, c->stream);
    if (!he) he = rt_memset(c->B.raw_tab, 0, 2 * (size_t)c->n_bins * 5 * 8, c->stream);
    if (!he) he = rt_sync(c->stream);
    return he ? fail(c, TGSF_E_HIP, "memset failed") : TGSF_OK;
}

extern "C" int tgsf_profile(tgsf_ctx* c, int enable)
{
    if (!c) return TGSF_E_INVALID;
    { int e = harvest_profile(c, c->last_stream); if (e) return e; }
    c->profile = enable != 0;
    memset(c->stage_ms, 0, sizeof c->stage_ms);
    c->prof_batches = 0;
    return TGSF_OK;
}

extern "C" int tgsf_stage_times(tgsf_ctx* c, float ms[TGSF_N_STAGES], uint32_t* n_batches)
{
    if (!c || !ms) return TGSF_E_INVALID;
    { int e = harvest_profile(c, c->last_stream); if (e) return e; }
    memcpy(ms, c->stage_ms, sizeof c->stage_ms);
    if (n_batches) *n_batches = c->prof_batches;
    return TGSF_OK;
}

extern "C" int tgsf_align_windows(tgsf_ctx* c, const uint8_t* seq, uint64_t n_bytes, const uint64_t* win_off,
                                  const uint32_t* win_len, const uint8_t* adapter_id, const int32_t* k, uint32_t n,
                                  int32_t* res, int32_t* ends)
{
    if (!c || !seq || !win_off || !win_len || !adapter_id || !k || !res || !ends) return TGSF_E_INVALID;
    if (!n) return TGSF_OK;
    for (uint32_t i = 0; i < n; i++) {
        if (adapter_id[i] >= c->P.n_adapters) return fail(c, TGSF_E_INVALID, "problem %u: adapter id out of range", i);
        if (win_len[i] == 0 || win_off[i] + win_len[i] > n_bytes) return fail(c, TGSF_E_INVALID, "problem %u: window outside the buffer", i);
        if (k[i] < 0) return fail(c, TGSF_E_INVALID, "problem %u: k < 0", i);
        const int Q = c->P.Q[adapter_id[i]];
        if (Q + std::min(Q, (int)k[i]) + 1 > c->scratch_cols)
            return fail(c, TGSF_E_CAPACITY, "problem %u: k larger than the context's thresholds allow for", i);
    }
    if ((size_t)n > (size_t)c->cap_reads * std::max(c->P.n_adapters, 1) * 2)
        return fail(c, TGSF_E_CAPACITY, "more alignment problems than the context was sized for");
    (void)rt_set_device(c->device);
    uint8_t *d_seq = nullptr, *d_aid = nullptr; uint64_t* d_off = nullptr; uint32_t* d_len = nullptr;
    int32_t *d_k = nullptr, *d_res = nullptr, *d_ends = nullptr;
    int e = 0;
    e |= rt_malloc((void**)&d_seq, n_bytes + 16);
    e |= rt_malloc((void**)&d_aid, n);
    e |= rt_malloc((void**)&d_off, (size_t)n * 8);
    e |= rt_malloc((void**)&d_len, (size_t)n * 4);
    e |= rt_malloc((void**)&d_k, (size_t)n * 4);
    e |= rt_malloc((void**)&d_res, (size_t)n * 16);
    e |= rt_malloc((void**)&d_ends, (size_t)n * 8);
    rt_stream st = c->stream;
    if (!e) {
        e |= rt_h2d(d_seq, seq, n_bytes, st);
        e |= rt_h2d(d_aid, adapter_id, n, st);
        e |= rt_h2d(d_off, win_off, (size_t)n * 8, st);
        e |= rt_h2d(d_len, win_len, (size_t)n * 4, st);
        e |= rt_h2d(d_k, k, (size_t)n * 4, st);
    }
    if (!e) {
        with_width(c->P.max_nw, [&](auto nw) {
            TGSF_LAUNCH(k_align_windows<decltype(nw)::value>, blocks_for(n, 64), 64, st, c->P, c->B, (const uint8_t*)d_seq, (const uint64_t*)d_off,
                        (const uint32_t*)d_len, (const uint8_t*)d_aid, (const int32_t*)d_k, n, d_res, d_ends);
        });
        e |= rt_d2h(res, d_res, (size_t)n * 16, st);
        e |= rt_d2h(ends, d_ends, (size_t)n * 8, st);
        e |= rt_sync(st);
    }
    rt_free(d_seq); rt_free(d_aid); rt_free(d_off); rt_free(d_len); rt_free(d_k); rt_free(d_res); rt_free(d_ends);
    return e ? fail(c, TGSF_E_HIP, "tgsf_align_windows: device operation failed") : TGSF_OK;
}
```

tgsfilter_amd/host/api.cpp:

```cpp
#include "api.h"
#include "cputime.h"
#include "fatal.h"

#include <dlfcn.h>
#include <unistd.h>

#include <chrono>
#include <cstdio>
#include <cstdlib>
#include <iostream>
#include <string>
#include <thread>

#ifndef TGSF_LIB_REL
#define TGSF_LIB_REL "../libtgsf.so"
#endif
#ifndef TGSF_EXPECT_BACKEND
#define TGSF_EXPECT_BACKEND "hip"
#endif

namespace host {

namespace {
Api g_api;
std::thread g_thread;
std::string g_error;
double g_load_s = 0, g_device_s = 0;
bool g_started = false;

double now_s() { return std::chrono::duration<double>(std::chrono::steady_clock::now().time_since_epoch()).count(); }

std::string lib_path()
{
    if (const char* e = getenv("TGSF_LIB")) return e;
    char exe[4096];
    const ssize_t n = readlink("/proc/self/exe", exe, sizeof exe - 1);
    std::string dir = n > 0 ? std::string(exe, (size_t)n) : std::string(".");
    const size_t slash = dir.rfind('/');
    dir = slash == std::string::npos ? "." : dir.substr(0, slash);
    return dir + "/" + TGSF_LIB_REL;
}

void load(std::vector<int> devices)
{
    CpuScope cpu(CPU_LOADER);
    const double t0 = now_s();
    const std::string path = lib_path();
    void* h = dlopen(path.c_str(), RTLD_NOW | RTLD_LOCAL);
    if (!h) { g_error = std::string("cannot load ") + path + ": " + dlerror() + " (there is no CPU fallback)"; return; }
#define BIND(field, sym) \
    g_api.field = reinterpret_cast<decltype(g_api.field)>(dlsym(h, sym)); \
    if (!g_api.field) { g_error = std::string("symbol ") + sym + " missing in " + path; return; }
    BIND(abi_version, "tgsf_abi_version")
    BIND(backend, "tgsf_backend")
    BIND(prepare_device, "tgsf_prepare_device")
    BIND(create, "tgsf_create")
    BIND(destroy, "tgsf_destroy")
    BIND(submit, "tgsf_submit")
    BIND(wait, "tgsf_wait")
    BIND(counters_len, "tgsf_counters_len")
    BIND(counters, "tgsf_counters")
    BIND(counters_used, "tgsf_counters_used")
    BIND(align_windows, "tgsf_align_windows")
    BIND(last_error, "tgsf_last_error")
    BIND(profile, "tgsf_profile")
    BIND(stage_times, "tgsf_stage_times")
    BIND(stage_name, "tgsf_stage_name")
    BIND(device_location, "tgsf_device_location")
    BIND(counters_merge, "tgsf_counters_merge")
#undef BIND
    if (g_api.abi_version() != TGSF_ABI_VERSION) { g_error = path + ": ABI version mismatch"; return; }
    {
        const char* b = g_api.backend();
        const std::string want = TGSF_EXPECT_BACKEND;
        if (!b || std::string(b).compare(0, want.size(), want) != 0) {
            g_error = path + " is the \"" + (b ? b : "?") + "\" build of the library; this program runs on the \"" + want +
                      "\" build only (there is no CPU fallback; is TGSF_LIB set by accident?)";
            return;
        }
    }
    g_load_s = now_s() - t0;
    std::vector<std::thread> up;
    for (size_t i = 1; i < devices.size(); i++) {
        bool seen = false;
        for (size_t j = 0; j < i; j++) seen = seen || devices[j] == devices[i];
        if (!seen) up.emplace_back([d = devices[i]] { CpuScope c2(CPU_LOADER); (void)g_api.prepare_device(d); });
    }
    if (!devices.empty()) (void)g_api.prepare_device(devices[0]);
    for (std::thread& t : up) t.join();
    g_device_s = now_s() - t0 - g_load_s;
}
}

void lib_start(const std::vector<int>& devices)
{
    g_started = true;
    g_thread = std::thread(load, devices);
}

const Api& lib()
{
    if (!g_started) lib_start({});
    if (g_thread.joinable()) g_thread.join();
    if (!g_error.empty()) {
        std::cerr << "Error: " << g_error << std::endl;
        quit(255);
    }
    return g_api;
}

namespace {
RcclApi g_rccl;
bool g_rccl_ok = false, g_rccl_started = false;
std::thread g_rccl_thread;

void load_rccl()
{
    std::string path = lib_path();
    const size_t slash = path.rfind('/');
    path = (slash == std::string::npos ? std::string(".") : path.substr(0, slash)) + "/libtgsf_rccl.so";
    void* h = dlopen(path.c_str(), RTLD_NOW | RTLD_LOCAL);
    if (!h) return;
#define BIND(field, sym) g_rccl.field = reinterpret_cast<decltype(g_rccl.field)>(dlsym(h, sym)); if (!g_rccl.field) return;
    BIND(unique_id, "tgsf_rccl_unique_id")
    BIND(comm_init, "tgsf_rccl_comm_init")
    BIND(comm_count, "tgsf_rccl_comm_count")
    BIND(comm_destroy, "tgsf_rccl_comm_destroy")
    BIND(allreduce_counters, "tgsf_rccl_allreduce_counters")
    BIND(last_error, "tgsf_rccl_last_error")
#undef BIND
    g_rccl_ok = true;
}
}

void rccl_start()
{
    if (g_rccl_started) return;
    g_rccl_started = true;
    g_rccl_thread = std::thread(load_rccl);
}

const RcclApi* rccl_lib()
{
    rccl_start();
    if (g_rccl_thread.joinable()) g_rccl_thread.join();
    return g_rccl_ok ? &g_rccl : nullptr;
}

void lib_times(double& load_s, double& device_s) { load_s = g_load_s; device_s = g_device_s; }

}
```

tgsfilter_amd/host/api.h:

```cpp
#pragma once
#include <vector>

#include "tgsf.h"
#include "tgsf_rccl.h"

namespace host {

struct Api {
    decltype(&tgsf_abi_version) abi_version;
    decltype(&tgsf_backend) backend;
    decltype(&tgsf_prepare_device) prepare_device;
    decltype(&tgsf_create) create;
    decltype(&tgsf_destroy) destroy;
    decltype(&tgsf_submit) submit;
    decltype(&tgsf_wait) wait;
    decltype(&tgsf_counters_len) counters_len;
    decltype(&tgsf_counters) counters;
    decltype(&tgsf_counters_used) counters_used;
    decltype(&tgsf_align_windows) align_windows;
    decltype(&tgsf_last_error) last_error;
    decltype(&tgsf_profile) profile;
    decltype(&tgsf_stage_times) stage_times;
    decltype(&tgsf_stage_name) stage_name;
    decltype(&tgsf_device_location) device_location;
    decltype(&tgsf_counters_merge) counters_merge;
};

struct RcclApi {
    decltype(&tgsf_rccl_unique_id) unique_id;
    decltype(&tgsf_rccl_comm_init) comm_init;
    decltype(&tgsf_rccl_comm_count) comm_count;
    decltype(&tgsf_rccl_comm_destroy) comm_destroy;
    decltype(&tgsf_rccl_allreduce_counters) allreduce_counters;
    decltype(&tgsf_rccl_last_error) last_error;
};
void rccl_start();
const RcclApi* rccl_lib();

void lib_start(const std::vector<int>& devices);
const Api& lib();
void lib_times(double& load_s, double& device_s);

}
```

tgsfilter_amd/host/prepass.cpp:

```cpp
#include "prepass.h"
#include <chrono>
#include <cstdio>

#include <unistd.h>

#include <algorithm>
#include <cstdlib>
#include <cstring>
#include <iostream>
#include <thread>
#include <unordered_map>
#include <vector>

#include "api.h"
#include "fatal.h"

namespace host {

const char* const kAdapterLib[22] = {
    "ATCTCTCTCTTTTCCTCCTCCTCCGTTGTTGTTGTTGAGAGAGAT",
    "ATCTCTCTCAACAACAACAACGGAGGAGGAGGAAAAGAGAGAGAT",
    "AAAAAAAAAAAAAAAAAATTAACGGAGGAGGAGGA",
    "TCCTCCTCCTCCGTTAATTTTTTTTTTTTTTTTTT",
    "AATGTACTTCGTTCAGTTACGTATTGCT",
    "AGCAATACGTAACTGAACGAAGTACATT",
    "GCAATACGTAACTGAACGAAGT",
    "ACTTCGTTCAGTTACGTATTGC",
    "GTTTTCGCATTTATCGTGAAACGCTTTCGCGTTTTTCGTGCGCCGCTTCA",
    "TGAAGCGGCGCACGAAAAACGCGAAAGCGTTTCACGATAAATGCGAAAAC",
    "GGCGTCTGCTTGGGTGTTTAACCTTTTTGTCAGAGAGGTTCCAAGTCAGAGAGGTTCCT",
    "AGGAACCTCTCTGACTTGGAACCTCTCTGACAAAAAGGTTAAACACCCAAGCAGACGCC",
    "GGAACCTCTCTGACTTGGAACCTCTCTGACAAAAAGGTTAAACACCCAAGCAGACGCCAGCAAT",
    "ATTGCTGGCGTCTGCTTGGGTGTTTAACCTTTTTGTCAGAGAGGTTCCAAGTCAGAGAGGTTCC",
    "TTTTTTTTCCTGTACTTCGTTCAGTTACGTATTGCT",
    "AGCAATACGTAACTGAACGAAGTACAGGAAAAAAAA",
    "GCAATACGTAACTGAACGAAGTACAGG",
    "CCTGTACTTCGTTCAGTTACGTATTGC",
    "ACGTAACTGAACGAAGTACAGG",
    "CCTGTACTTCGTTCAGTTACGT",
    "CTTGCGGGCGGCGGACTCTCCTCTGAAGATAGAGCGACAGGCAAG",
    "CTTGCCTGTCGCTCTATCTTCAGAGGAGAGTCCGCCGCCCGCAAG",
};

std::string rev_comp(const std::string& s)
{
    static char comp[256];
    static bool init = false;
    if (!init) {
        memset(comp, 'N', sizeof comp);
        const char* a = "AGCTagctMRWSYKmrwsyk";
        const char* b = "TCGAtcgaKYWSRMkywsrm";
        for (int i = 0; a[i]; i++) comp[(unsigned char)a[i]] = b[i];
        init = true;
    }
    std::string r;
    r.reserve(s.size());
    for (size_t i = s.size(); i-- > 0;) r += comp[(unsigned char)s[i]];
    return r;
}

static int check_base_content(const std::vector<std::string>& ends, int check_len, int seq_num, float end_bias)
{
    static const struct Col { uint8_t of[256]; Col() { memset(of, 4, sizeof of); of['A'] = of['a'] = 0; of['T'] = of['t'] = 1; of['G'] = of['g'] = 2; of['C'] = of['c'] = 3; } } col;
    std::vector<int> cnt5((size_t)check_len * 5, 0);
    for (const std::string& s : ends) {
        const size_t n = std::min(s.size(), (size_t)check_len);
        for (size_t i = 0; i < n; i++) cnt5[i * 5 + col.of[(unsigned char)s[i]]]++;
    }
    std::vector<int> cnt((size_t)check_len * 4, 0);
    for (int i = 0; i < check_len; i++) for (int j = 0; j < 4; j++) cnt[(size_t)i * 4 + j] = cnt5[(size_t)i * 5 + j];
    const int max_diff = (int)((seq_num * end_bias) / 100);
    int trim = 0;
    for (int i = 1; i < check_len - 1; i++) {
        const int ld = std::min(i, 5), rd = std::min(check_len - i - 1, 5);
        bool left = false, right = false;
        for (int j = 0; j < 4; j++) {
            for (int x = 1; x <= ld; x++)
                if (abs(cnt[(size_t)i * 4 + j] - cnt[(size_t)(i - x) * 4 + j]) > max_diff) { left = true; break; }
            for (int x = 1; x <= rd; x++)
                if (abs(cnt[(size_t)(i + x) * 4 + j] - cnt[(size_t)i * 4 + j]) > max_diff) { right = true; break; }
        }
        if (left && right) trim = i + 1;
    }
    return trim;
}

static double pp_now() { return std::chrono::duration<double>(std::chrono::steady_clock::now().time_since_epoch()).count(); }
static double g_pp_create = 0, g_pp_align = 0; static int g_pp_calls = 0;

static void adapter_search(const Options& o, const std::vector<std::string>& ends, std::string& adapter, float& depth)
{
    adapter.clear(); depth = 0.f;
    float min_sim = o.mid_sim;
    if (min_sim < 0.9) min_sim = 0.9f;
    if (ends.empty()) return;

    tgsf_params p;
    memset(&p, 0, sizeof p);
    p.struct_size = sizeof p;
    p.min_len = 100; p.max_len = 2147483647; p.min_q = 0; p.max_q = 255; p.bc_len = 0;
    p.end_len = 0; p.extra_len = 0; p.end_sim = 0.75f; p.mid_sim = 0.9f; p.filter = 1; p.qtype = 33;
    p.n_adapters = 22;
    int k[22];
    size_t max_q = 0;
    for (int a = 0; a < 22; a++) {
        p.adapters[a] = kAdapterLib[a];
        p.adapter_len[a] = (int)strlen(kAdapterLib[a]);
        k[a] = (int)((1 - min_sim) * p.adapter_len[a]) + 1;
        max_q = std::max(max_q, (size_t)p.adapter_len[a]);
    }
    p.end_match_len = 2; p.mid_match_len = (int)max_q;
    const size_t per_call = 4096;
    p.max_batch_reads = (uint32_t)(per_call * 22 / (22 * 2) + 64);
    p.max_batch_bases = 1 << 20; p.max_read_len = 1 << 16;
    tgsf_ctx* ctx = nullptr;
    const double c0 = pp_now();
    if (lib().create(&p, o.devices.empty() ? o.device : o.devices[0], &ctx) != TGSF_OK) { std::cerr << "Error: " << lib().last_error(nullptr) << std::endl; quit(255); }

    g_pp_create += pp_now() - c0;
    std::unordered_map<int, int> maps;
    std::vector<uint8_t> buf; std::vector<uint64_t> off; std::vector<uint32_t> len; std::vector<uint8_t> aid;
    std::vector<int32_t> kk, res, eds;
    for (size_t b = 0; b < ends.size(); b += per_call) {
        const size_t e = std::min(ends.size(), b + per_call);
        buf.clear(); off.clear(); len.clear(); aid.clear(); kk.clear();
        for (size_t i = b; i < e; i++) {
            const uint64_t o0 = buf.size();
            buf.insert(buf.end(), ends[i].begin(), ends[i].end());
            if (ends[i].empty()) continue;
            for (int a = 0; a < 22; a++) { off.push_back(o0); len.push_back((uint32_t)ends[i].size()); aid.push_back((uint8_t)a); kk.push_back(k[a]); }
        }
        const uint32_t n = (uint32_t)off.size();
        if (!n) continue;
        res.assign((size_t)n * 4, 0); eds.assign((size_t)n * 2, 0);
        const double a0 = pp_now();
        if (lib().align_windows(ctx, buf.data(), buf.size(), off.data(), len.data(), aid.data(), kk.data(), n, res.data(), eds.data()) != TGSF_OK) {
            std::cerr << "Error: " << lib().last_error(ctx) << std::endl; quit(255);
        }
        g_pp_align += pp_now() - a0; g_pp_calls++;
        for (uint32_t i = 0; i < n; i++)
            if (res[(size_t)i * 4 + 1] > 0)
                maps[(int)aid[i]] += res[(size_t)i * 4 + 2] - res[(size_t)i * 4 + 0];
    }
    lib().destroy(ctx);
    std::vector<std::pair<int, int>> vec(maps.begin(), maps.end());
    std::sort(vec.begin(), vec.end(), [](const std::pair<int, int>& a, const std::pair<int, int>& b) { return a.second > b.second; });
    if (vec.empty()) return;
    const int best = vec.front().first;
    const std::string cand = kAdapterLib[best];
    const float mean_dep = (float)maps[best] / (float)cand.size();
    if (mean_dep >= 2 * min_sim) { adapter = cand; depth = mean_dep; }
}

PrepassResult run_prepass(Options& o, const std::function<bool(Rec&)>& next_record)
{
    PrepassResult R;
    const double t0 = pp_now();
    int check_len = std::max(std::max(o.end_len, o.bc_len), 100);
    int min_len = std::max(o.min_len, 2 * check_len);
    const int max_seq = std::max(o.ad_num, o.bc_num);
    std::vector<std::string> ends5, ends3;
    const bool need5 = o.filter && (o.head_trim < 0 || o.adapter_file.empty());
    const bool need3 = o.filter && (o.tail_trim < 0 || o.adapter_file.empty());
    int seq_num = 0, min_qc = 255, max_qc = 0;
    {
        Rec r;
        const bool has_qual = o.in_type != 0;
        while (next_record(r)) {
            const int L = (int)r.len;
            if (L < min_len) continue;
            if (seq_num >= max_seq) break;
            seq_num++;
            if (need5) ends5.emplace_back(r.seq, (size_t)check_len);
            if (need3) ends3.emplace_back(rev_comp(std::string(r.seq + (L - check_len), (size_t)check_len)));
            if (has_qual)
                for (int i = 0; i < check_len; i++) { const char c = r.qual[i]; if (min_qc > c) min_qc = c; if (max_qc < c) max_qc = c; }
        }
    }
    const double t_read = pp_now() - t0;
    if (o.in_type == 1 || o.in_type == 2) {
        if (min_qc >= 33 && min_qc <= 78 && max_qc >= 33 && max_qc <= 127) R.qtype = 33;
        else if (min_qc >= 64 && min_qc <= 108 && max_qc >= 64 && max_qc <= 127) R.qtype = 64;
        else R.qtype = min_qc < 55 ? 33 : 64;
        std::cerr << "INFO: base quality scoring: Phred" << R.qtype << std::endl;
        const int maxq = max_qc - R.qtype;
        if (o.min_q >= 0) {
            if (o.min_q >= maxq) {
                std::cerr << "Warning: max base quality score was: " << maxq << std::endl;
                std::cerr << "INFO: Please reset -q parameter." << std::endl;
                quit(255);
            }
        } else {
            if (maxq > 10 && o.read_type == "clr") o.min_q = 10;
            else if (maxq > 20 && o.read_type == "hifi") o.min_q = 20;
            else if (maxq > 10 && o.read_type == "ont") o.min_q = 10;
            else o.min_q = 0;
        }
    }
    const double t1 = pp_now();
    double t_bc = 0;
    if (o.filter) {
        {
            std::thread t3;
            if (o.tail_trim < 0) t3 = std::thread([&] { R.trim3p = check_base_content(ends3, check_len, seq_num, o.end_bias); });
            if (o.head_trim < 0) R.trim5p = check_base_content(ends5, check_len, seq_num, o.end_bias);
            if (t3.joinable()) t3.join();
        }
        if (o.head_trim < 0 && o.tail_trim < 0 && R.trim5p > o.bc_len) R.trim5p = o.bc_len;
        t_bc = pp_now() - t1;
        if (o.adapter_file.empty()) {
            adapter_search(o, ends5, R.adapter5p, R.depth5p);
            adapter_search(o, ends3, R.adapter3p, R.depth3p);
        }
    }
    if (getenv("TGSF_TIMING"))
        fprintf(stderr, "PREPASS: %d reads looked at in %.3f s | base content %.3f | adapter search %.3f (contexts %.3f, %d alignment calls %.3f)\n",
                seq_num, t_read, t_bc, pp_now() - t1 - t_bc, g_pp_create, g_pp_calls, g_pp_align);
    return R;
}

}
```

tgsfilter_amd/host/prepass.h:

```cpp
#pragma once
#include <functional>
#include <string>
#include <vector>

#include "fastx.h"
#include "options.h"

namespace host {

extern const char* const kAdapterLib[22];

std::string rev_comp(const std::string& s);

struct PrepassResult {
    int qtype = 0;
    int trim5p = 0, trim3p = 0;
    std::string adapter5p, adapter3p;
    float depth5p = 0.f, depth3p = 0.f;
};

PrepassResult run_prepass(Options& o, const std::function<bool(Rec&)>& next_record);

}
```

tgsfilter_amd/host/run.h:

```cpp
#pragma once
#include <memory>

#include "api.h"
#include "pipeline.h"
#include "prepass.h"
#include "report.h"
#include "shard.h"

namespace host {

int cpu_budget();
[[noreturn]] void leave(int code);
bool detached();

struct Run {
    explicit Run(Options& opts) : o(opts) {}

    int set_up_ranks();
    int check_file_types();
    void open_input();
    void open_output_early();
    void prepass();
    void make_contexts();
    void filter_pass();
    void downsample();
    void sum_tallies();
    void report();
    void timing_lines();

    Options& o;
    RankLink link;
    bool shard_may_use_rccl = false;
    bool sharded = false;
    bool timing = false;
    double t_epoch0 = 0, t_start = 0;
    double t_prepass = 0, t_pipe = 0, t_parse = 0, t_gpu = 0, t_write = 0, t_widle = 0, t_first = 0;

    std::string html;
    bool fasta_in = false;
    InputBytes in;
    bool streaming = false;
    size_t chunk_bytes = 64u << 20;
    int scan_threads = 1;
    size_t text_off = 0, text_size = 0;
    const char* text = nullptr;
    std::unique_ptr<RecordIndex> records_p;
    std::unique_ptr<ChunkReader> open_stream();

    std::string out_path;
    bool plain_file_out() const;
    MappedWriter mapped;
    Output out;
    bool fastq_out = false, run_filter_pass = true;

    PrepassResult pp;
    std::vector<std::string> adapters;

    uint64_t batch_text = 0;
    uint32_t batch_reads = 1u << 16;
    const Api* api = nullptr;
    double t_load = 0, t_dev = 0, t_libwait = 0;
    const RcclApi* R = nullptr;
    struct RcclUp { std::atomic<int> done{0}; int rc = TGSF_OK; std::string err; void* comm = nullptr; };
    std::shared_ptr<RcclUp> rccl_state = std::make_shared<RcclUp>();
    std::thread rccl_up;
    bool use_rccl = false;
    bool ranks_own_gpus = false;
    tgsf_params p;
    std::vector<int> ctx_dev;
    std::vector<tgsf_ctx*> ctxs;
    double t_p0 = 0;

    std::unique_ptr<Channel<std::shared_ptr<Batch>>> to_gpu, to_writer;
    std::vector<int> raw_lens, clean_lens;
    uint64_t raw_bases = 0, clean_bases = 0;
    uint64_t own_raw_bases = 0;
    std::vector<CleanRec> clean_recs;
    BatchStore store;
    std::atomic<uint64_t> stream_text{0};
    std::atomic<double> stream_share{0.0};
    std::mutex gpu_time_m;
    bool numa_bind = false;
    std::vector<int> dev_node;
    std::vector<double> dev_submit_s;
    std::vector<uint64_t> dev_bytes, dev_batches;
    int fill_threads = 1, populate_threads = 1;
    uint64_t fill_min = 1u << 20, stride_bytes = 2ull << 30;
    bool release_input = false, release_output = false;
    bool mapped_out = false;
    void reader_body();
    void feed(size_t k);
    void bind_to_node_of(size_t k);
    void writer_body();
    void fill_job(const std::shared_ptr<Batch>& b, size_t lo, size_t hi);
    void batch_done(std::shared_ptr<Batch> b);

    MappedWriter down_mapped;
    bool open_down_mapped(uint64_t capacity, uint64_t speculative);
    uint64_t down_bases = 0, down_job_recs = 0, down_job_bases = 0;
    std::vector<int> down_lens;
    std::vector<uint64_t> down_t;
    double t_dsel = 0, t_dcreate = 0, t_dqc = 0, t_dwrite = 0, t_dclose = 0, t_dsubmit = 0, t_dfirst = 0, d_kept = 0, d_span = 0;
    int n_dsubmit = 0;
    bool d_in_place = false, d_mapped = false;
    std::vector<char> select_kept();
    void second_pass(const std::vector<char>& keep);
    std::thread start_qc_feed(const std::vector<char>& keep, tgsf_ctx*& qctx, tgsf_ctx*& qctx2);
    void feed_in_place(const std::vector<uint32_t>& by_addr, const tgsf_params& qp, uint64_t kept_span, tgsf_ctx* qctx, tgsf_ctx*& qctx2);
    void feed_packed(const std::vector<char>& keep, const tgsf_params& qp, size_t room, tgsf_ctx* qctx);
    void write_kept(const std::vector<char>& keep);
    void merge_down_tallies(tgsf_ctx* qctx, tgsf_ctx* qctx2);

    uint64_t nw = 0;
    int32_t bc = 0;
    uint32_t nbins = 0;
    std::vector<uint64_t> t;
    double t_x0 = 0, t_rccl_wait = 0, t_allreduce = 0;
    int rccl_ranks = 0;
    std::string tally_route;
    bool reports() const { return !sharded || link.rank == 0; }
};

void add_tallies(std::vector<uint64_t>& v, const std::vector<uint64_t>& part, int32_t bc, uint32_t nbins);
std::vector<uint64_t> pack_rows(const std::vector<uint64_t>& v, int32_t bc, uint32_t nbins);
void add_rows(std::vector<uint64_t>& v, const std::vector<uint64_t>& ru, int32_t bc, uint32_t nbins);

}
```

tgsfilter_amd/host/run_pipeline.cpp:

```cpp
#include "run.h"

#include <sched.h>

namespace host {

void Run::reader_body()
{
    CpuScope cpu(CPU_BATCHER);
    if (!run_filter_pass) { for (size_t d = 0; d < ctxs.size(); d++) to_gpu->put(nullptr); return; }
    std::unique_ptr<RecordIndex::Cursor> rd;
    if (!streaming) rd.reset(new RecordIndex::Cursor(*records_p));
    std::unique_ptr<ChunkReader> cr;
    if (streaming) cr = open_stream();
    std::shared_ptr<Chunk> ch;
    size_t ch_at = 0;
    bool over = false;
    Rec r;
    auto fresh = [&] { return store.get(); };
    std::shared_ptr<Batch> b = fresh();
    const double t0 = now_s();
    double waited = 0;
    uint64_t next_id = 0;
    auto flush = [&] {
        if (b->recs.empty()) return;
        const double w0 = now_s();
        b->id = next_id++;
        to_gpu->put(std::move(b));
        waited += now_s() - w0;
        b = fresh();
    };
    auto next_record = [&]() {
        if (!streaming) return rd->next(r);
        while (!over && (!ch || ch_at >= ch->recs.size())) {
            flush();
            if (ch && !ch->message.empty()) std::cerr << ch->message << std::endl;
            if (ch && ch->last) { over = true; break; }
            ch = cr->next(o.in_file);
            ch_at = 0;
            if (!ch) { over = true; break; }
            stream_text.store(cr->text_bytes());
            stream_share.store(cr->consumed());
        }
        if (over) return false;
        r = ch->recs[ch_at++];
        return true;
    };
    auto bad_cut = [&](size_t at) {
        die("--ranks / --shard: the input cannot be cut near byte " + std::to_string(at) + " the way one sequential reader would read it "
            "(lines the reader skips, or a malformed record, near there): run it without --ranks / --shard");
    };
    const char* last_end = nullptr;
    while (next_record()) {
        const size_t L = r.len;
        if (L > p.max_read_len) die("read longer than the supported maximum");
        const char* rec_end = (fasta_in ? r.seq : r.qual) + L;
        if (sharded && !last_end && link.rank > 0 && r.name != text + 1) bad_cut(text_off);
        last_end = rec_end;
        if (!b->recs.empty() && ((uint64_t)(rec_end - b->base) > batch_text || b->recs.size() >= batch_reads)) flush();
        if (b->recs.empty()) { b->base = r.name; b->hold = ch; }
        b->off.push_back((uint64_t)(r.seq - b->base));
        b->qoff.push_back(fasta_in ? b->off.back() : (uint64_t)(r.qual - b->base));
        b->len.push_back((uint32_t)L); b->recs.push_back(r);
        b->span = (uint64_t)(rec_end - b->base);
        if (b->span > p.max_batch_bases) die("record larger than a batch");
        b->bases += L;
        raw_bases += L; raw_lens.push_back((int)L);
    }
    if (sharded && link.rank + 1 < link.world) {
        const char* e = last_end ? last_end : text;
        const char* const end = text + text_size;
        if (e < end && *e == '\r') e++;
        if (e < end && *e == '\n') e++;
        if (e != end || !records_p->end_message().empty()) bad_cut(text_off + text_size);
    }
    flush();
    for (size_t d = 0; d < ctxs.size(); d++) to_gpu->put(nullptr);
    t_parse = now_s() - t0 - waited;
    std::sort(raw_lens.begin(), raw_lens.end());
}

void Run::bind_to_node_of(size_t k)
{
    const Api& L = *api;
    int node = -1;
    char bus[64];
    if (L.device_location(ctx_dev[k], bus, (int)sizeof bus, &node) == TGSF_OK && node >= 0) {
        const char* sysfs = knob("TGSF_SYSFS_NODES");
        std::ifstream f(std::string(sysfs ? sysfs : "/sys/devices/system/node") + "/node" + std::to_string(node) + "/cpulist");
        std::string list;
        cpu_set_t set;
        CPU_ZERO(&set);
        int n_set = 0;
        if (f && std::getline(f, list)) {
            size_t i = 0;
            while (i < list.size()) {
                const int a = atoi(list.c_str() + i);
                int b = a;
                size_t j = list.find_first_of(",-", i);
                if (j != std::string::npos && list[j] == '-') { b = atoi(list.c_str() + j + 1); j = list.find(',', j); }
                for (int c2 = a; c2 <= b && c2 < CPU_SETSIZE; c2++) { CPU_SET(c2, &set); n_set++; }
                i = j == std::string::npos ? list.size() : j + 1;
            }
        }
        cpu_set_t allowed;
        if (n_set > 0 && sched_getaffinity(0, sizeof allowed, &allowed) == 0) {
            n_set = 0;
            for (int c2 = 0; c2 < CPU_SETSIZE; c2++) {
                if (CPU_ISSET(c2, &set) && !CPU_ISSET(c2, &allowed)) CPU_CLR(c2, &set);
                if (CPU_ISSET(c2, &set)) n_set++;
            }
        }
        if (n_set > 0 && sched_setaffinity(0, sizeof set, &set) == 0) dev_node[k] = node;
    }
}

void Run::feed(size_t k)
{
    CpuScope cpu(CPU_FEEDER);
    const Api& L = *api;
    if (numa_bind) bind_to_node_of(k);
    if (L.create(&p, ctx_dev[k], &ctxs[k]) != TGSF_OK) die(L.last_error(nullptr));
    tgsf_ctx* fctx = ctxs[k];
    if (timing) (void)L.profile(fctx, 1);
    for (;;) {
        std::shared_ptr<Batch> b = to_gpu->get();
        if (!b) break;
        const double g0 = now_s();
        if (b->res.size() < b->recs.size()) b->res.resize(b->recs.size());
        const size_t fneed = (size_t)(b->bases / (uint64_t)std::max(p.min_len, 1)) + b->recs.size() + 16;
        if (b->frags.size() < fneed) b->frags.resize(fneed);
        const uint8_t* btext = reinterpret_cast<const uint8_t*>(b->base);
        tgsf_batch_in bi;
        memset(&bi, 0, sizeof bi);
        bi.seq = btext; bi.qual = btext;
        bi.offsets = b->off.data(); bi.qual_offsets = b->qoff.data(); bi.lengths = b->len.data();
        bi.n_reads = (uint32_t)b->recs.size(); bi.n_bytes = b->span;
        tgsf_batch_out bo{b->res.data(), b->frags.data(), (uint32_t)b->frags.size(), 0};
        if (L.submit(fctx, &bi, &bo) != TGSF_OK) die(L.last_error(fctx));
        { std::lock_guard<std::mutex> l(gpu_time_m); t_gpu += now_s() - g0; if (t_first == 0) t_first = now_s() - t_p0; }
        dev_submit_s[k] += now_s() - g0; dev_bytes[k] += b->span; dev_batches[k]++;
        b->n_frags = bo.n_frags;
        to_writer->put(std::move(b));
    }
    to_writer->put(nullptr);
}

void Run::batch_done(std::shared_ptr<Batch> b)
{
    if (b->out_bytes && release_output) mapped.release(b->dst, b->out_bytes);
    if (release_input) mapped.release(b->base, b->span);
    store.put(std::move(b));
}

void Run::filter_pass()
{
    to_gpu.reset(new Channel<std::shared_ptr<Batch>>(2 + ctxs.size()));
    to_writer.reset(new Channel<std::shared_ptr<Batch>>(256));
    if (!run_filter_pass) {
        RecordIndex::Cursor rd(*records_p);
        Rec r;
        while (rd.next(r)) {
            clean_recs.push_back({std::string_view(r.name, r.name_len), 1, r.seq, r.qual, r.len});
            clean_bases += r.len;
        }
    }

    std::thread reader([this] { reader_body(); });

    numa_bind = o.devices.size() > 1 || (link.world > 1 && ranks_own_gpus);
    if (const char* e = getenv("TGSF_NUMA")) numa_bind = atoi(e) > 0;
    dev_node.assign(ctx_dev.size(), -1);
    dev_submit_s.assign(ctx_dev.size(), 0.0);
    dev_bytes.assign(ctx_dev.size(), 0);
    dev_batches.assign(ctx_dev.size(), 0);
    std::vector<std::thread> feeders;
    for (size_t k = 0; k < ctxs.size(); k++) feeders.emplace_back([this, k] { feed(k); });

    fill_threads = std::max(1, std::min(o.n_thread, 16));
    fill_min = 1u << 20;
    if (const char* e = knob("TGSF_FILL_MIN_BYTES")) { const long long v = atoll(e); if (v > 0) fill_min = (uint64_t)v; }
    populate_threads = std::max(1, std::min(o.n_thread, 32));
    if (const char* e = knob("TGSF_POPULATE_THREADS")) { const int v = atoi(e); if (v >= 1 && v <= 64) populate_threads = v; }
    stride_bytes = streaming ? (128ull << 20) : (2ull << 30);
    if (const char* e = knob("TGSF_STRIDE_BYTES")) { const long long v = atoll(e); if (v > 0) stride_bytes = (uint64_t)v; }
    mapped.start_reserving(populate_threads, stride_bytes, (!streaming && text_size > (256u << 20)) ? (uint64_t)text_size / 4 : 0);
    {
        uint64_t early_min = 1ull << 30;
        if (const char* e = knob("TGSF_DOWN_EARLY_MIN")) early_min = strtoull(e, nullptr, 10);
        if (o.downsample && !streaming && in.mapped() && (uint64_t)text_size >= early_min) {
            uint64_t spec = (uint64_t)text_size / 4;
            if (o.genome_size > 0 && o.desired_depth > 0) spec = std::min<uint64_t>(spec, (2 * o.genome_size * (uint64_t)o.desired_depth) / (uint64_t)link.world + (uint64_t)text_size / 64);
            open_down_mapped(4 * (uint64_t)text_size + (1ull << 30), spec);
        }
    }
    const bool sync_exit = !detached();
    release_input = sync_exit && !streaming && in.mapped() && !o.downsample;
    release_output = sync_exit || streaming;
    mapped.start_filling(fill_threads, 16u << 20);
    std::thread writer([this] { writer_body(); });
    reader.join();
    for (std::thread& f : feeders) f.join();
    writer.join();
    mapped_out = mapped.is_open();
    mapped.finish();
    t_pipe = now_s() - t_p0;
}

}
```

tgsfilter_amd/host/run_report.cpp:

```cpp
#include "run.h"

#include <sys/stat.h>

namespace host {

std::vector<uint64_t> pack_rows(const std::vector<uint64_t>& v, int32_t bc2, uint32_t nb2)
{
    const size_t head = tgsf_ctr_bin_table(0, bc2, nb2);
    std::vector<uint64_t> out(v.begin(), v.begin() + (long)head);
    for (int b = 0; b < 4; b++) {
        const size_t at = tgsf_ctr_bin_table(b, bc2, nb2), n = (size_t)std::min<uint64_t>(v[TGSF_CTR_ROWS + (b >> 1)], nb2) * 5;
        out.insert(out.end(), v.begin() + (long)at, v.begin() + (long)(at + n));
    }
    return out;
}

void add_tallies(std::vector<uint64_t>& v, const std::vector<uint64_t>& part, int32_t bc2, uint32_t nb2)
{
    uint64_t rows[4];
    for (int q = 0; q < 4; q++) rows[q] = std::max(v[TGSF_CTR_ROWS + q], part[TGSF_CTR_ROWS + q]);
    const size_t head = tgsf_ctr_bin_table(0, bc2, nb2);
    for (size_t i = 0; i < head; i++) v[i] += part[i];
    for (int b = 0; b < 4; b++) {
        const size_t at = tgsf_ctr_bin_table(b, bc2, nb2), n = (size_t)std::min<uint64_t>(part[TGSF_CTR_ROWS + (b >> 1)], nb2) * 5;
        for (size_t i = 0; i < n; i++) v[at + i] += part[at + i];
    }
    for (int q = 0; q < 4; q++) v[TGSF_CTR_ROWS + q] = rows[q];
}

void add_rows(std::vector<uint64_t>& v, const std::vector<uint64_t>& ru, int32_t bc2, uint32_t nb2)
{
    const size_t head = tgsf_ctr_bin_table(0, bc2, nb2);
    if (ru.size() < head) die("a rank of the job sent a tally vector of another layout");
    std::vector<uint64_t> whole(v.size(), 0);
    std::copy(ru.begin(), ru.begin() + (long)head, whole.begin());
    size_t from = head;
    for (int b = 0; b < 4; b++) {
        const size_t at = tgsf_ctr_bin_table(b, bc2, nb2), n = (size_t)std::min<uint64_t>(ru[TGSF_CTR_ROWS + (b >> 1)], nb2) * 5;
        if (from + n > ru.size()) die("a rank of the job sent a tally vector of another layout");
        std::copy(ru.begin() + (long)from, ru.begin() + (long)(from + n), whole.begin() + (long)at);
        from += n;
    }
    add_tallies(v, whole, bc2, nb2);
}

static void add_context(const Api& L, tgsf_ctx* c, std::vector<uint64_t>& v, std::vector<uint64_t>& part, int32_t bc, uint32_t nbins)
{
    if (L.counters_used(c, part.data(), part.size(), nullptr) != TGSF_OK) die(L.last_error(c));
    add_tallies(v, part, bc, nbins);
}

void Run::sum_tallies()
{
    const Api& L = *api;
    tgsf_ctx* ctx = ctxs[0];
    void* rccl_comm = nullptr;
    int rccl_rc = TGSF_OK;
    std::string rccl_err;
    L.counters_len(ctx, &nw, &bc, &nbins);
    t.assign(nw, 0);
    std::vector<uint64_t> part(nw);
    t_x0 = now_s();
    own_raw_bases = raw_bases;
    const char* ex = getenv("TGSF_SHARD_EXCHANGE");
    const bool must_rccl = ex && !strcmp(ex, "rccl");
    for (tgsf_ctx* c : ctxs) add_context(L, c, t, part, bc, nbins);
    if (!sharded) return;

    if (use_rccl) {
        double rccl_patience = 120.0;
        if (const char* e = knob("TGSF_RCCL_INIT_TIMEOUT_S")) rccl_patience = atof(e);
        while (!rccl_state->done.load(std::memory_order_acquire) && now_s() - t_x0 < rccl_patience) usleep(2000);
        if (rccl_state->done.load(std::memory_order_acquire)) {
            rccl_up.join();
            rccl_rc = rccl_state->rc; rccl_err = rccl_state->err; rccl_comm = rccl_state->comm;
        } else {
            rccl_up.detach();
            rccl_rc = TGSF_E_HIP;
            rccl_err = "the communicator was not up " + std::to_string((int)rccl_patience) + " s after the filtering ended";
        }
        t_rccl_wait = now_s() - t_x0;
        if (link.max_u64(rccl_rc != TGSF_OK ? 1 : 0) != 0) {
            if (must_rccl) die("RCCL communicator: " + (rccl_err.empty() ? std::string("it failed on another rank") : rccl_err));
            if (rccl_rc != TGSF_OK) std::cerr << "Warning: rank " << link.rank << ": RCCL communicator: " << rccl_err << " -- the tallies are summed over the ranks' sockets" << std::endl;
            rccl_comm = nullptr;
            use_rccl = false;
        }
    }
    std::vector<uint64_t> reduced;
    if (use_rccl) {
        for (size_t k = 1; k < ctxs.size(); k++)
            if (L.counters_merge(ctxs[0], ctxs[k]) != TGSF_OK) die(L.last_error(ctxs[0]));
        struct Reduce { std::atomic<int> done{0}; int rc = TGSF_OK; std::string err; double s = 0; };
        const std::shared_ptr<Reduce> rd = std::make_shared<Reduce>();
        double patience = 60.0;
        if (const char* e = knob("TGSF_RCCL_ALLREDUCE_TIMEOUT_S")) patience = atof(e);
        const double a0 = now_s();
        std::thread helper([R = R, rd, c0 = ctxs[0], rccl_comm, rank = link.rank, world = link.world, a0] {
            if (const char* e = knob("TGSF_RCCL_ALLREDUCE_STALL_S")) usleep((useconds_t)(atof(e) * 1e6));
            rd->rc = R->allreduce_counters(c0, rccl_comm, rank, world, 0, nullptr);
            if (rd->rc != TGSF_OK) rd->err = R->last_error();
            rd->s = now_s() - a0;
            rd->done.store(1, std::memory_order_release);
        });
        while (!rd->done.load(std::memory_order_acquire) && now_s() - a0 < patience) usleep(500);
        int bad = 0;
        if (rd->done.load(std::memory_order_acquire)) {
            helper.join();
            t_allreduce = rd->s;
            if (rd->rc != TGSF_OK) { bad = 1; rccl_err = "tally all-reduce: " + rd->err; }
        } else {
            helper.detach();
            bad = 1;
            rccl_err = "the tally all-reduce had not returned after " + std::to_string((int)patience) + " s";
        }
        if (link.max_u64((uint64_t)bad) != 0) {
            if (must_rccl) die(rccl_err.empty() ? std::string("tally all-reduce: it failed on another rank") : rccl_err);
            if (bad) std::cerr << "Warning: rank " << link.rank << ": " << rccl_err << " -- the tallies summed over the ranks' sockets are used" << std::endl;
            use_rccl = false;
        } else {
            (void)R->comm_count(rccl_comm, &rccl_ranks);
            reduced.assign(nw, 0);
            add_context(L, ctxs[0], reduced, part, bc, nbins);
        }
    }
    BlobOut mine;
    mine.pod(raw_bases); mine.pod(clean_bases);
    mine.vec(raw_lens); mine.vec(clean_lens);
    mine.vec(pack_rows(t, bc, nbins));
    const std::vector<std::string> all = link.gather(mine.s);
    for (int k = 1; k < (int)all.size(); k++) {
        BlobIn in2(all[(size_t)k]);
        uint64_t rb = 0, cb = 0;
        std::vector<int> rl, cl;
        std::vector<uint64_t> ru;
        in2.pod(rb); in2.pod(cb); in2.vec(rl); in2.vec(cl); in2.vec(ru);
        raw_bases += rb; clean_bases += cb;
        const size_t r0 = raw_lens.size(), c0 = clean_lens.size();
        raw_lens.insert(raw_lens.end(), rl.begin(), rl.end());
        clean_lens.insert(clean_lens.end(), cl.begin(), cl.end());
        std::inplace_merge(raw_lens.begin(), raw_lens.begin() + (long)r0, raw_lens.end());
        if (!o.downsample) std::inplace_merge(clean_lens.begin(), clean_lens.begin() + (long)c0, clean_lens.end());
        add_rows(t, ru, bc, nbins);
    }
    tally_route = "summed on rank 0 over the ranks' sockets";
    if (use_rccl) {
        tally_route = "RCCL all-reduce on the devices";
        if (link.rank == 0) {
            if (pack_rows(reduced, bc, nbins) == pack_rows(t, bc, nbins)) { t.swap(reduced); tally_route += ", equal to the sum over the ranks' sockets"; }
            else {
                if (must_rccl) die("the all-reduced tally vector differs from the sum of the ranks' vectors over their sockets");
                std::cerr << "Warning: the all-reduced tally vector differs from the sum of the ranks' vectors over their sockets -- the sockets' sum is used" << std::endl;
                tally_route += " (DIFFERENT from the sum over the ranks' sockets, which is used)";
            }
        }
    }
    if (timing)
        fprintf(stderr, "SHARD %d/%d: bytes [%zu, %zu) of the text on device %d -> %s | tallies: %s (communicator ready after %.3f s of waiting, all-reduce %.4f s, %d ranks in it), exchange + gather %.3f s\n",
                link.rank, link.world, text_off, text_off + text_size, o.device, out_path.c_str(), tally_route.c_str(), t_rccl_wait, t_allreduce, rccl_ranks, now_s() - t_x0);
    if (use_rccl) R->comm_destroy(rccl_comm);
}

void Run::report()
{
    auto tables = [&](const std::vector<uint64_t>& v, bool clean) {
        SideTables s;
        s.bin_qual = &v[tgsf_ctr_bin_table(clean ? TGSF_B_CLEAN_QUAL : TGSF_B_RAW_QUAL, bc, nbins)];
        s.bin_cnt = &v[tgsf_ctr_bin_table(clean ? TGSF_B_CLEAN_CNT : TGSF_B_RAW_CNT, bc, nbins)];
        s.bin_rows = v[TGSF_CTR_ROWS + (clean ? 1 : 0)];
        s.q5 = &v[tgsf_ctr_end_table(clean ? TGSF_T_CLEAN5P_QUAL : TGSF_T_RAW5P_QUAL, bc)];
        s.c5 = &v[tgsf_ctr_end_table(clean ? TGSF_T_CLEAN5P_CNT : TGSF_T_RAW5P_CNT, bc)];
        s.q3 = &v[tgsf_ctr_end_table(clean ? TGSF_T_CLEAN3P_QUAL : TGSF_T_RAW3P_QUAL, bc)];
        s.c3 = &v[tgsf_ctr_end_table(clean ? TGSF_T_CLEAN3P_CNT : TGSF_T_RAW3P_CNT, bc)];
        s.end_rows = v[TGSF_CTR_ROWS + (clean ? 3 : 2)];
        s.diff_qual = &v[clean ? TGSF_CTR_CLEAN_DIFFQ : TGSF_CTR_RAW_DIFFQ];
        return s;
    };
    SideStats raw, clean;
    const int clean_num = (int)clean_lens.size();
    if (run_filter_pass && reports()) {
        if (raw_lens.empty()) die("no reads in the input");
        std::sort(raw_lens.begin(), raw_lens.end());
        side_stats(bc, raw_lens, raw_bases, tables(t, false), raw);
        if (!o.only_qc && !o.downsample) {
            if (clean_lens.empty()) die("no reads passed the filters");
            std::sort(clean_lens.begin(), clean_lens.end());
            side_stats(bc, clean_lens, clean_bases, tables(t, true), clean);
        }
        const uint64_t* d = &t[TGSF_CTR_DROPINFO];
        std::cerr << "INFO: " << raw_lens.size() << " reads with a total of " << raw_bases << " bases were input." << std::endl;
        if (!o.only_qc) {
            std::cerr << "INFO: " << d[0] << " reads were discarded with " << d[1] << " bases due to low quality." << std::endl;
            std::cerr << "INFO: " << d[2] << " reads have adapter at 5', 3' and middle." << std::endl;
            std::cerr << "INFO: " << d[3] << " reads have adapter at 5' and middle." << std::endl;
            std::cerr << "INFO: " << d[4] << " reads have adapter at 3' and middle." << std::endl;
            std::cerr << "INFO: " << d[5] << " reads have adapter at 5' and 3' end." << std::endl;
            std::cerr << "INFO: " << d[6] << " reads only have adapter at middle." << std::endl;
            std::cerr << "INFO: " << d[7] << " reads only have adapter at 5' end." << std::endl;
            std::cerr << "INFO: " << d[8] << " reads only have adapter at 3' end." << std::endl;
            std::cerr << "INFO: " << d[9] << " reads didn't have any adapter." << std::endl;
            std::cerr << "INFO: " << d[10] << " bases were trimmed due to the adapter or base content bias." << std::endl;
            std::cerr << "INFO: " << d[11] << " reads were discarded with " << d[12] << " bases due to the short length." << std::endl;
            std::cerr << "INFO: " << d[13] << " reads were discarded with " << d[14] << " bases due to low quality after split." << std::endl;
            if (o.min_repeat > 0)
                std::cerr << "INFO: " << d[15] << " reads were discarded with " << d[16] << " bases due to short repeat length." << std::endl;
            std::cerr << "INFO: " << clean_num << " reads with a total of " << clean_bases << " bases after filtering." << std::endl;
            if (!o.downsample && !o.out_file.empty()) {
                if (!sharded) std::cerr << "INFO: Filtered reads were written to: " << o.out_file << "." << std::endl;
                else std::cerr << "INFO: Filtered reads were written to: " << o.out_file << ".part0 ... " << o.out_file << ".part" << link.world - 1
                               << " (" << link.world << " parts; concatenated in this order they are the reads in input order)." << std::endl;
            }
        }
    }
    if (reports() && sharded && !o.out_file.empty() && !o.only_qc && !o.only_adapters) {
        const std::string list = o.out_file + ".parts";
        std::vector<std::string> earlier;
        {
            std::ifstream f(list);
            std::string line;
            if (f && std::getline(f, line) && line == "# tgsfilter parts, in order")
                while (std::getline(f, line)) if (!line.empty()) earlier.push_back(line);
        }
        std::vector<std::string> mine;
        for (int k = 0; k < link.world; k++) mine.push_back(o.out_file + ".part" + std::to_string(k));
        for (const std::string& e : earlier) {
            if (std::find(mine.begin(), mine.end(), e) != mine.end()) continue;
            const std::string stem = o.out_file + ".part";
            if (e.compare(0, stem.size(), stem) != 0 || e.size() == stem.size() || e.find_first_not_of("0123456789", stem.size()) != std::string::npos) continue;
            struct stat st;
            if (lstat(e.c_str(), &st) == 0 && S_ISREG(st.st_mode) && unlink(e.c_str()) == 0)
                std::cerr << "Warning: " << e << ", a part of an earlier job with more ranks, was removed." << std::endl;
        }
        for (int k = link.world; k < link.world + 1024; k++) {
            const std::string other = o.out_file + ".part" + std::to_string(k);
            struct stat st;
            if (lstat(other.c_str(), &st) != 0) { if (k >= link.world + 64) break; else continue; }
            std::cerr << "Warning: " << other << " exists and is not a part of this job (nor of an earlier one this tool listed): `cat " << o.out_file
                      << ".part*` would take it in -- the parts of this job are listed in " << list << "." << std::endl;
        }
        std::ofstream f(list, std::ios::trunc);
        f << "# tgsfilter parts, in order\n";
        for (const std::string& m : mine) f << m << "\n";
    }
    if (o.downsample && reports()) {
        if (down_lens.empty()) die("no reads to downsample");
        std::sort(down_lens.begin(), down_lens.end());
        side_stats(bc, down_lens, down_bases, tables(down_t, false), clean);
        clean.tab[8] = limit_decimals(std::round(clean.mean_qual * 1000) / 1000.0, 2);
        if (!o.filter)
            std::cerr << "INFO: " << (sharded ? down_job_recs : clean_recs.size()) << " reads with a total of " << (sharded ? down_job_bases : clean_bases) << " bases were input." << std::endl;
        std::cerr << "INFO: " << down_lens.size() << " reads with a total of " << down_bases << " bases after downsampling." << std::endl;
        if (!o.out_file.empty()) {
            if (!sharded) std::cerr << "INFO: Downsampled reads were written to: " << o.out_file << "." << std::endl;
            else std::cerr << "INFO: Downsampled reads were written to: " << o.out_file << ".part0 ... " << o.out_file << ".part" << link.world - 1
                           << " (" << link.world << " parts; concatenated in this order they are the reads in input order)." << std::endl;
        }
    }
    std::string qc = fasta_in ? "0" : "1";
    qc += o.only_qc ? "0" : ((!o.filter && o.downsample) ? "1" : "2");
    if (reports()) {
        std::ofstream ofs(html);
        write_report(ofs, qc, raw, clean);
        ofs.close();
        std::cerr << "INFO: Quality control report was written to: " << html << "." << std::endl;
    }
}

void Run::timing_lines()
{
    const Api& L = *api;
    if (timing) {
        Pool& fills = mapped.pool();
        const double t_busy = fills.busy_s();
        fprintf(stderr, "POOL: %zu jobs, busy %.3f, freeing job state %.3f, longest job %.3f, first job at %.3f, last job done at %.3f (pipeline start = 0, planner done at %.3f)\n",
                fills.jobs_, t_busy, fills.destroy_, fills.longest_, fills.first_ - t_p0, fills.last_ - t_p0, mapped.t_planned - t_p0);
        fprintf(stderr, "TIMING: total %.3f s | index+prepass %.3f | waiting for the library %.3f (load %.3f + device %.3f, beside the pre-pass) | "
                        "pipeline %.3f (batching %.3f, tgsf_submit summed over %zu feeders %.3f, plan+write %.3f, planner waiting %.3f, "
                        "first batch filtered after %.3f, fill tail %.3f, closing the output %.3f; stages overlap) | stats+report %.3f | %s (fallocate %.3f, mapping the reserved pages %.3f, fill threads busy %.3f summed)\n",
                now_s() - t_start, t_prepass, t_libwait, t_load, t_dev, t_pipe, t_parse, ctxs.size(), t_gpu, t_write, t_widle, t_first,
                mapped.t_fill_tail, mapped.t_close, now_s() - t_p0 - t_pipe, mapped_out ? "output: fallocate + mapped fill" : "output: writev", mapped.sink.t_falloc, mapped.t_populate_wait(), t_busy);
        fprintf(stderr, "RESERVE: planner waited %.3f s for pages of the output file\n", mapped.t_claim_wait);
    }
    if (timing) {
        float tot[TGSF_N_STAGES] = {0};
        uint32_t nb = 0;
        for (tgsf_ctx* c : ctxs) {
            float ms[TGSF_N_STAGES]; uint32_t n1 = 0;
            if (c && L.stage_times(c, ms, &n1) == TGSF_OK) { nb += n1; for (int i = 0; i < TGSF_N_STAGES; i++) tot[i] += ms[i]; }
        }
        double sum = 0;
        for (int i = 0; i < TGSF_N_STAGES; i++) sum += tot[i];
        char piece[256];
        snprintf(piece, sizeof piece, "GPU: kernels %.3f s summed over %zu contexts and %u batches (upper bound of the busy time: contexts overlap) = %.4f of the run |", sum * 1e-3, ctxs.size(), nb,
                 sum * 1e-3 / std::max(1e-9, now_s() - t_start));
        std::string line = piece;
        for (int i = 0; i < TGSF_N_STAGES; i++) if (tot[i] > 0) { snprintf(piece, sizeof piece, " %s %.1f ms", L.stage_name(i), tot[i]); line += piece; }
        line += "\n";
        fputs(line.c_str(), stderr);
    }
    if (timing) {
        for (size_t di = 0; di < o.devices.size(); di++) {
            if (std::find(o.devices.begin(), o.devices.begin() + (long)di, o.devices[di]) != o.devices.begin() + (long)di) continue;
            double sub = 0; uint64_t by = 0, nb2 = 0; int nf2 = 0, node = -1;
            for (size_t k = 0; k < ctx_dev.size(); k++)
                if (ctx_dev[k] == o.devices[di]) { sub += dev_submit_s[k]; by += dev_bytes[k]; nb2 += dev_batches[k]; nf2++; node = std::max(node, dev_node[k]); }
            fprintf(stderr, "DEVICE %d: %llu batches, %.2f GB of text through %d feeders, tgsf_submit %.3f s summed = %.1f GB/s per feeder, %.1f GB/s for the device over the pipeline's %.3f s%s\n",
                    o.devices[di], (unsigned long long)nb2, by * 1e-9, nf2, sub, sub > 0 ? by * 1e-9 / sub : 0.0, t_pipe > 0 ? by * 1e-9 / t_pipe : 0.0, t_pipe,
                    node >= 0 ? (" (feeders bound to NUMA node " + std::to_string(node) + ")").c_str() : "");
        }
    }
    if (timing) {
        const double proc = process_cpu_s();
        double own = 0;
        std::string line;
        char piece[160];
        for (int s = 0; s < CPU_N; s++) {
            double v = (double)cpu_ns()[s].load() * 1e-9;
            if (s == CPU_MAIN) v += (double)thread_cpu_ns() * 1e-9 - (double)cpu_ns()[CPU_PREPASS].load() * 1e-9;
            own += v;
            if (v >= 0.0005) { snprintf(piece, sizeof piece, "%s %s %.3f", line.empty() ? "" : ",", cpu_stage_name(s), v); line += piece; }
        }
        snprintf(piece, sizeof piece, "CPU: %.3f s of CPU time (user + system) for %.3f Gbases = %.4f CPU-s per Gbase |", proc, (double)own_raw_bases * 1e-9,
                 own_raw_bases ? proc / ((double)own_raw_bases * 1e-9) : 0.0);
        std::string head = piece;
        snprintf(piece, sizeof piece, " | threads of the runtime and others %.3f\n", proc - own);
        fputs((head + line + piece).c_str(), stderr);
    }
    if (timing && o.downsample)
        fprintf(stderr, "DOWN: selection %.3f | QC pass over the kept reads (%s, %.2f GB of them in %.2f GB of text): context %.3f, batches + submits %.3f (its own thread; %d submits %.3f, the first %.3f) | writing them %.3f (%s) | closing the output %.3f\n",
                t_dsel, d_in_place ? "read in place" : "packed", d_kept * 1e-9, d_span * 1e-9, t_dcreate, t_dqc, n_dsubmit, t_dsubmit, t_dfirst, t_dwrite, d_mapped ? "fallocate + threads into a mapping" : "writev", t_dclose);
    if (timing) {
        struct timespec ts; clock_gettime(CLOCK_REALTIME, &ts);
        fprintf(stderr, "CLOCK: main entered at %.6f, leaving at %.6f (epoch seconds)\n", t_epoch0, (double)ts.tv_sec + ts.tv_nsec * 1e-9);
    }
}

}
```

tgsfilter_amd/host/run_setup.cpp:

```cpp
#include "run.h"

#include <sched.h>
#include <sys/stat.h>

namespace host {

int Run::set_up_ranks()
{
    if (o.ranks >= 1 && o.shard_world > 0) { std::cerr << "Error: --ranks starts the ranks itself; --shard is for a rank started by another launcher" << std::endl; return 1; }
    if (o.ranks >= 1 || o.shard_world >= 1) {
        const int world = o.ranks >= 1 ? o.ranks : o.shard_world;
        const char* why = nullptr;
        if (o.out_file.empty() && !o.only_qc && !o.only_adapters) why = "every rank writes a part file of its own: -o is needed";
        else if (file_type(o.in_file) == 2 || (o.in_file.size() > 3 && o.in_file.compare(o.in_file.size() - 3, 3, ".gz") == 0))
            why = "the ranks take byte ranges of a plain FASTQ / FASTA text";
        if (why) { std::cerr << "Error: --ranks / --shard: " << why << std::endl; return 1; }
        if (world > 1024) { std::cerr << "Error: --ranks " << world << std::endl; return 1; }
        {
            std::vector<int> dv;
            for (int r = 0; r < world && o.ranks >= 1; r++) dv.push_back(o.devices.empty() ? r : o.devices[(size_t)r % o.devices.size()]);
            std::sort(dv.begin(), dv.end());
            shard_may_use_rccl = o.ranks < 1 || std::adjacent_find(dv.begin(), dv.end()) == dv.end();
            const char* ex = getenv("TGSF_SHARD_EXCHANGE");
            if (ex && !strcmp(ex, "socket")) shard_may_use_rccl = false;
        }
        if (o.ranks >= 1) {
            fork_ranks(world, link);
            o.device = o.devices.empty() ? link.rank : o.devices[(size_t)link.rank % o.devices.size()];
        } else {
            if (o.rendezvous.empty()) { std::cerr << "Error: --shard needs --rendezvous <path>: where the ranks of the job meet (a unix socket)" << std::endl; return 1; }
            setenv("HSA_ENABLE_IPC_MODE_LEGACY", "0", 0);
            link.rendezvous(o.shard_rank, world, o.rendezvous);
        }
        o.devices.assign(1, o.device);
        o.n_thread = std::max(2, std::min(o.n_thread, std::max(o.n_thread / world, cpu_budget() / world)));
    }
    sharded = o.ranks >= 1 || o.shard_world >= 1;
    return 0;
}

int Run::check_file_types()
{
    o.in_type = file_type(o.in_file);
    const std::string prefix = file_prefix(o.in_file);
    html = prefix + ".html";
    if (!o.out_file.empty() && !o.only_qc) {
        html = file_prefix(o.out_file) + ".html";
        o.out_type = file_type(o.out_file);
        if (file_extension(o.out_file) == "gz") o.out_gz = true;
    } else {
        o.out_type = o.fasta_out ? 0 : (o.in_type == 2 ? 1 : o.in_type);
    }
    if (o.in_type == 3 || o.out_type == 3) {
        std::cerr << "Error: The file name suffix should be '.[fastq|fq|fasta|fa][.gz] or .[sam|bam]'" << std::endl;
        if (o.in_type == 3) std::cerr << "Error: Please check your input file name: " << o.in_file << std::endl;
        else std::cerr << "Error: Please check your output file name: " << o.out_file << std::endl;
        return 1;
    }
    if (o.in_type == 0 && o.out_type == 1) { std::cerr << "Error: Fasta format input file can't output fastq format file" << std::endl; return 1; }
    fasta_in = o.in_type == 0;
    return 0;
}

std::unique_ptr<ChunkReader> Run::open_stream()
{
    std::string err;
    std::unique_ptr<TextSource> src = open_text(in.data(), in.size(), o.in_type == 2, err);
    if (!src) { std::cerr << "Error: " << err << " (" << o.in_file << ")" << std::endl; fflush(nullptr); _exit(255); }
    return std::unique_ptr<ChunkReader>(new ChunkReader(std::move(src), !fasta_in, chunk_bytes, 20));
}

void Run::open_input()
{
    if (o.devices.empty()) o.devices.push_back(o.device);
    lib_start(o.devices);
    if (sharded && shard_may_use_rccl) rccl_start();

    const bool coded = o.in_type == 2 || (o.in_file.size() > 3 && o.in_file.compare(o.in_file.size() - 3, 3, ".gz") == 0);
    uint64_t stream_min = 256ull << 20;
    if (const char* e = knob("TGSF_STREAM_MIN_BYTES")) stream_min = strtoull(e, nullptr, 10);
    if (coded && !o.downsample) {
        if (!in.open_raw(o.in_file)) leave(1);
        streaming = in.size() >= stream_min;
    }
    if (!streaming && !in.open(o.in_file, o.in_type == 2)) leave(1);
    chunk_bytes = [] { const char* e = knob("TGSF_CHUNK_BYTES"); return e ? (size_t)strtoull(e, nullptr, 10) : (size_t)(64u << 20); }();
    const int budget = std::max(1, cpu_budget() / link.world);
    scan_threads = std::max(1, std::min({o.n_thread, 32, std::max(2, budget / 2)}));
    text_off = 0; text_size = in.size();
    if (sharded) {
        if (streaming || (in.size() > 0 && !in.mapped())) die("--ranks / --shard: the input is not a plain text file");
        const size_t lo = find_record_start(in.data(), in.size(), (size_t)((unsigned __int128)in.size() * (unsigned)link.rank / (unsigned)link.world), !fasta_in);
        const size_t hi = link.rank + 1 == link.world ? in.size()
                        : find_record_start(in.data(), in.size(), (size_t)((unsigned __int128)in.size() * (unsigned)(link.rank + 1) / (unsigned)link.world), !fasta_in);
        text_off = lo; text_size = hi > lo ? hi - lo : 0;
    }
    text = in.data() + text_off;
    if (!streaming) records_p.reset(new RecordIndex(text, text_size, !fasta_in, scan_threads));
}

void Run::open_output_early()
{
    out_path = sharded && !o.out_file.empty() ? o.out_file + ".part" + std::to_string(link.rank) : o.out_file;
    {
        uint64_t early_min = 256ull << 20;
        if (const char* e = knob("TGSF_EARLY_OPEN_MIN")) early_min = strtoull(e, nullptr, 10);
        const bool may_map_early = plain_file_out() && !o.only_qc && !o.downsample && (o.filter || o.only_qc) &&
                                   !o.only_adapters && !streaming && in.mapped() && (uint64_t)text_size >= early_min;
        if (may_map_early && mapped.open(out_path, 4 * (uint64_t)text_size + (1ull << 30), true))
            mapped.reserve_early((uint64_t)text_size / 4);
    }
}

}
```

Baseline: 7.524.

## Precreate adapter-search context in loader thread and reduce totals on device

Adds a device kernel that aligns every read end against all library adapters and reduces matched lengths, hit counts and first-hit index with wave reductions and atomics, so the pre-pass no longer builds per-window host arrays and scans per-window results. The adapter-search context is created and warmed up ahead of time on the library-loading thread and published through a condition variable, so pre-pass context creation overlaps other start-up work. Read ends are stored flat instead of as a vector of strings. Map insertion order now follows first-hit order, so ties in the adapter ranking could resolve differently than before. Extra timing prints are added.

After: 7.296. 0.97x the previous value.

```diff
diff --git a/include/tgsf.h b/include/tgsf.h
--- a/include/tgsf.h
+++ b/include/tgsf.h
@@ -162,6 +162,9 @@
                        const uint8_t* adapter_id, const int32_t* k, uint32_t n,
                        int32_t* res, int32_t* ends);
 
+int tgsf_adapter_totals(tgsf_ctx* ctx, const uint8_t* ends, uint32_t n_ends, uint32_t stride, uint32_t end_len,
+                        const int32_t* k, int64_t* totals, uint32_t* hits, uint32_t* first_end);
+
 const char* tgsf_last_error(tgsf_ctx* ctx);
 
 #ifdef __cplusplus
diff --git a/tgsfilter_amd/capi.py b/tgsfilter_amd/capi.py
--- a/tgsfilter_amd/capi.py
+++ b/tgsfilter_amd/capi.py
@@ -15,7 +15,7 @@
     "tgsf_abi_version", "tgsf_backend", "tgsf_prepare_device", "tgsf_device_location", "tgsf_create", "tgsf_destroy", "tgsf_submit", "tgsf_submit_async", "tgsf_submit_device",
     "tgsf_wait",
     "tgsf_counters_len", "tgsf_counters", "tgsf_counters_used", "tgsf_counters_merge", "tgsf_counters_device", "tgsf_reset_counters", "tgsf_profile",
-    "tgsf_stage_times", "tgsf_stage_name", "tgsf_align_windows", "tgsf_last_error",
+    "tgsf_stage_times", "tgsf_stage_name", "tgsf_align_windows", "tgsf_adapter_totals", "tgsf_last_error",
 ]
 
 
@@ -59,6 +59,7 @@
     L.tgsf_stage_name.argtypes = [C.c_int]
     L.tgsf_stage_name.restype = C.c_char_p
     L.tgsf_align_windows.argtypes = [vp, vp, u64, vp, vp, vp, vp, u32, vp, vp]
+    L.tgsf_adapter_totals.argtypes = [vp, vp, u32, u32, u32, vp, vp, vp, vp]
     L.tgsf_last_error.argtypes = [vp]
     L.tgsf_last_error.restype = C.c_char_p
     if L.tgsf_abi_version() != abi.ABI_VERSION:
@@ -194,3 +195,15 @@
                                               win_len.ctypes.data, adapter_id.ctypes.data, k.ctypes.data, n,
                                               res.ctypes.data, ends.ctypes.data))
         return res, ends
+
+    def adapter_totals(self, ends, n_ends, stride, end_len, k):
+        ends = np.frombuffer(ends, dtype=np.uint8) if isinstance(ends, (bytes, bytearray)) else np.ascontiguousarray(ends, np.uint8)
+        k = np.ascontiguousarray(k, dtype=np.int32)
+        A = self.params.n_adapters
+        assert len(k) == A and (n_ends == 0 or ends.size >= (n_ends - 1) * stride + end_len)
+        totals = np.zeros(A, dtype=np.int64)
+        hits = np.zeros(A, dtype=np.uint32)
+        first = np.zeros(A, dtype=np.uint32)
+        self._chk(self.lib.tgsf_adapter_totals(self.h, ends.ctypes.data, n_ends, stride, end_len, k.ctypes.data,
+                                               totals.ctypes.data, hits.ctypes.data, first.ctypes.data))
+        return totals, hits, first
diff --git a/tgsfilter_amd/csrc/tgsf_emul.h b/tgsfilter_amd/csrc/tgsf_emul.h
--- a/tgsfilter_amd/csrc/tgsf_emul.h
+++ b/tgsfilter_amd/csrc/tgsf_emul.h
@@ -68,6 +68,7 @@
 TGSF_HD uint64_t wave_sum(uint64_t v) { return v; }
 TGSF_HD int32_t wave_sum_i32(int32_t v) { return v; }
 TGSF_HD uint32_t wave_max(uint32_t v) { return v; }
+TGSF_HD uint32_t wave_min_u32(uint32_t v) { return v; }
 TGSF_HD uint32_t wave_or(uint32_t v) { return v; }
 TGSF_HD bool wave_leader() { return true; }
 TGSF_HD bool wave_any(bool b) { return b; }
diff --git a/tgsfilter_amd/csrc/tgsf_hip.h b/tgsfilter_amd/csrc/tgsf_hip.h
--- a/tgsfilter_amd/csrc/tgsf_hip.h
+++ b/tgsfilter_amd/csrc/tgsf_hip.h
@@ -68,6 +68,11 @@
     for (int o = 32; o > 0; o >>= 1) { uint32_t u = __shfl_xor(v, o, 64); v = u > v ? u : v; }
     return v;
 }
+TGSF_D uint32_t wave_min_u32(uint32_t v) {
+#pragma unroll
+    for (int o = 32; o > 0; o >>= 1) { uint32_t u = __shfl_xor(v, o, 64); v = u < v ? u : v; }
+    return v;
+}
 TGSF_D uint32_t wave_or(uint32_t v) {
 #pragma unroll
     for (int o = 32; o > 0; o >>= 1) v |= __shfl_xor(v, o, 64);
diff --git a/tgsfilter_amd/csrc/tgsf_kernels.h b/tgsfilter_amd/csrc/tgsf_kernels.h
--- a/tgsfilter_amd/csrc/tgsf_kernels.h
+++ b/tgsfilter_amd/csrc/tgsf_kernels.h
@@ -2401,4 +2401,35 @@
     ends[i * 2 + 1] = w.best < 0 ? -1 : w.last_end;
 }
 
-}
+struct TotalsK { int32_t k[TGSF_MAX_ADAPTERS]; };
+template <int MAXNW>
+TGSF_KERNEL k_adapter_totals(DevParams P, DevBatch B, const uint8_t* ends, uint32_t n_ends, uint32_t stride, uint32_t end_len,
+                             TotalsK kk, uint64_t wave0, uint64_t* totals, uint32_t* hits, uint32_t* first_end)
+{
+    const uint32_t A = (uint32_t)P.n_adapters;
+    const uint64_t t = wave0 + blockIdx.x;
+    const int a = (int)(t % A);
+    const uint64_t e = (t / A) * 64u + (threadIdx.x & 63u);
+    const int Q = P.Q[a];
+    int k = kk.k[a];
+    if (k > Q) k = Q;
+    uint64_t mlen = 0;
+    uint32_t hit = 0, first = 0xFFFFFFFFu;
+    if (e < n_ends) {
+        const LaneScratch sc = lane_scratch(B, 0);
+        const uint8_t* w0 = ends + e * stride;
+        const int T = (int)end_len;
+        const WinAln w = by_length<MAXNW>(Q, [=, &P](auto f) TGSF_INLINE_LAMBDA { return align_window<typename decltype(f)::col>(P, a, w0, T, k, 0, sc, true); });
+        if (w.best >= 0 && w.n > 0) { mlen = (uint64_t)w.mlen; hit = 1; first = (uint32_t)e; }
+    }
+    mlen = wave_sum(mlen);
+    hit = (uint32_t)wave_sum((uint64_t)hit);
+    first = wave_min_u32(first);
+    if (wave_leader() && hit) {
+        atomicAdd((ull*)&totals[a], (ull)mlen);
+        atomicAdd(&hits[a], hit);
+        atomicMin(&first_end[a], first);
+    }
+}
+
+}
diff --git a/tgsfilter_amd/csrc/tgsf_lib.hip b/tgsfilter_amd/csrc/tgsf_lib.hip
--- a/tgsfilter_amd/csrc/tgsf_lib.hip
+++ b/tgsfilter_amd/csrc/tgsf_lib.hip
@@ -33,6 +33,10 @@
     bool no_hot32 = false;
     uint64_t ctr_words;
     int scratch_cols;
+    size_t scratch_waves;
+    uint8_t* tot_ends = nullptr;
+    size_t tot_ends_cap = 0;
+    uint8_t* tot_res = nullptr;
     uint8_t *d_seq, *d_qual;
     uint64_t* d_off;
     uint64_t* d_qoff;
@@ -269,6 +273,8 @@
     if (c->aux) rt_stream_destroy(c->aux);
     if (c->own_stream && c->stream) rt_stream_destroy(c->stream);
     dev_free_all(c);
+    if (c->tot_ends) rt_free(c->tot_ends);
+    if (c->tot_res) rt_free(c->tot_res);
     delete c;
 }
 
@@ -536,7 +542,7 @@
     c->ctr_words = tgsf_ctr_len(p->bc_len, c->n_bins);
     adapter_rules(*p, P);
     const Sizing S = size_context(*p, P);
-    c->B = S.B; c->cap_chunks = S.cap_chunks; c->scratch_cols = S.scratch_cols; P.seg_cols = S.seg_cols;
+    c->B = S.B; c->cap_chunks = S.cap_chunks; c->scratch_cols = S.scratch_cols; c->scratch_waves = S.scratch_waves; P.seg_cols = S.seg_cols;
     c->flat_scan = S.flat_scan; c->suffix_filter = S.suffix_filter; c->no_hot32 = S.no_hot32;
 
     if ((e = bring_up(c)) || (e = build_tables(c)) || (e = allocate(c, S))) {
@@ -1231,3 +1237,61 @@
     rt_free(d_seq); rt_free(d_aid); rt_free(d_off); rt_free(d_len); rt_free(d_k); rt_free(d_res); rt_free(d_ends);
     return e ? fail(c, TGSF_E_HIP, "tgsf_align_windows: device operation failed") : TGSF_OK;
 }
+
+extern "C" int tgsf_adapter_totals(tgsf_ctx* c, const uint8_t* ends, uint32_t n_ends, uint32_t stride, uint32_t end_len,
+                                   const int32_t* k, int64_t* totals, uint32_t* hits, uint32_t* first_end)
+{
+    if (!c || !ends || !k || !totals || !hits || !first_end) return c ? fail(c, TGSF_E_INVALID, "tgsf_adapter_totals: null argument") : TGSF_E_INVALID;
+    if (end_len == 0 || end_len > (uint32_t)kMaxLenParam) return fail(c, TGSF_E_INVALID, "tgsf_adapter_totals: end_len of %u (1 .. 2^28)", end_len);
+    if (stride < end_len) return fail(c, TGSF_E_INVALID, "tgsf_adapter_totals: stride %u below end_len %u", stride, end_len);
+    const int A = c->P.n_adapters;
+    TotalsK kk;
+    memset(&kk, 0, sizeof kk);
+    for (int a = 0; a < A; a++) {
+        if (k[a] < 0) return fail(c, TGSF_E_INVALID, "adapter %d: k < 0", a);
+        const int Q = c->P.Q[a];
+        if (Q + std::min(Q, (int)k[a]) + 1 > c->scratch_cols)
+            return fail(c, TGSF_E_CAPACITY, "adapter %d: k larger than the context's thresholds allow for", a);
+        kk.k[a] = k[a];
+    }
+    for (int a = 0; a < A; a++) { totals[a] = 0; hits[a] = 0; first_end[a] = 0xFFFFFFFFu; }
+    if (!n_ends || !A) return TGSF_OK;
+    (void)rt_set_device(c->device);
+    rt_stream st = c->stream;
+    const size_t n_bytes = (size_t)(n_ends - 1) * stride + end_len;
+    int e = 0;
+    if (n_bytes > c->tot_ends_cap) {
+        if (c->tot_ends) rt_free(c->tot_ends);
+        c->tot_ends = nullptr; c->tot_ends_cap = 0;
+        e = rt_malloc((void**)&c->tot_ends, n_bytes + 64);
+        if (!e) c->tot_ends_cap = n_bytes;
+    }
+    if (!e && !c->tot_res) e = rt_malloc((void**)&c->tot_res, (size_t)TGSF_MAX_ADAPTERS * 16);
+    if (e) return fail(c, TGSF_E_HIP, "tgsf_adapter_totals: device allocation failed: %s", rt_errstr(e));
+    uint64_t* d_tot = (uint64_t*)c->tot_res;
+    uint32_t* d_hits = (uint32_t*)(c->tot_res + (size_t)A * 8);
+    uint32_t* d_first = d_hits + A;
+    e |= rt_h2d(c->tot_ends, ends, n_bytes, st);
+    e |= rt_memset(d_tot, 0, (size_t)A * 12, st);
+    e |= rt_memset(d_first, 0xFF, (size_t)A * 4, st);
+    uint64_t per_launch = std::min<uint64_t>(c->scratch_waves, 1u << 30);
+    if (const char* v = knob("TGSF_TOTALS_WAVES")) { const long long w = atoll(v); if (w >= 1 && (uint64_t)w < per_launch) per_launch = (uint64_t)w; }
+    const uint64_t waves = (uint64_t)((n_ends + 63u) / 64u) * (uint64_t)A;
+    if (!e) {
+        for (uint64_t w0 = 0; w0 < waves; w0 += per_launch) {
+            const unsigned grid = (unsigned)std::min<uint64_t>(per_launch, waves - w0);
+            with_width(c->P.max_nw, [&](auto nw) {
+                TGSF_LAUNCH(k_adapter_totals<decltype(nw)::value>, grid, 64, st, c->P, c->B, (const uint8_t*)c->tot_ends, n_ends, stride, end_len,
+                            kk, w0, d_tot, d_hits, d_first);
+            });
+        }
+        uint64_t h[TGSF_MAX_ADAPTERS * 2];
+        e |= rt_d2h(h, c->tot_res, (size_t)A * 16, st);
+        e |= rt_sync(st);
+        if (!e) {
+            const uint32_t* hh = (const uint32_t*)(h + A);
+            for (int a = 0; a < A; a++) { totals[a] = (int64_t)h[a]; hits[a] = hh[a]; first_end[a] = hh[A + a]; }
+        }
+    }
+    return e ? fail(c, TGSF_E_HIP, "tgsf_adapter_totals: device operation failed") : TGSF_OK;
+}
diff --git a/tgsfilter_amd/host/api.cpp b/tgsfilter_amd/host/api.cpp
--- a/tgsfilter_amd/host/api.cpp
+++ b/tgsfilter_amd/host/api.cpp
@@ -6,11 +6,15 @@
 #include <unistd.h>
 
 #include <chrono>
+#include <condition_variable>
 #include <cstdio>
 #include <cstdlib>
 #include <iostream>
+#include <mutex>
 #include <string>
 #include <thread>
+
+#include "prepass.h"
 
 #ifndef TGSF_LIB_REL
 #define TGSF_LIB_REL "../libtgsf.so"
@@ -27,6 +31,17 @@
 std::string g_error;
 double g_load_s = 0, g_device_s = 0;
 bool g_started = false;
+std::mutex g_search_m;
+std::condition_variable g_search_cv;
+bool g_search_published = false;
+tgsf_ctx* g_search_ctx = nullptr;
+
+void publish_search(tgsf_ctx* c)
+{
+    { std::lock_guard<std::mutex> l(g_search_m); g_search_ctx = c; g_search_published = true; }
+    g_search_cv.notify_all();
+}
+struct PublishAtExit { ~PublishAtExit() { if (!g_search_published) publish_search(nullptr); } };
 
 double now_s() { return std::chrono::duration<double>(std::chrono::steady_clock::now().time_since_epoch()).count(); }
 
@@ -41,9 +56,10 @@
     return dir + "/" + TGSF_LIB_REL;
 }
 
-void load(std::vector<int> devices)
+void load(std::vector<int> devices, bool search)
 {
     CpuScope cpu(CPU_LOADER);
+    PublishAtExit publish_at_exit;
     const double t0 = now_s();
     const std::string path = lib_path();
     void* h = dlopen(path.c_str(), RTLD_NOW | RTLD_LOCAL);
@@ -62,6 +78,7 @@
     BIND(counters, "tgsf_counters")
     BIND(counters_used, "tgsf_counters_used")
     BIND(align_windows, "tgsf_align_windows")
+    BIND(adapter_totals, "tgsf_adapter_totals")
     BIND(last_error, "tgsf_last_error")
     BIND(profile, "tgsf_profile")
     BIND(stage_times, "tgsf_stage_times")
@@ -86,16 +103,36 @@
         for (size_t j = 0; j < i; j++) seen = seen || devices[j] == devices[i];
         if (!seen) up.emplace_back([d = devices[i]] { CpuScope c2(CPU_LOADER); (void)g_api.prepare_device(d); });
     }
+    if (search && !devices.empty()) {
+        tgsf_params sp;
+        int32_t k[22];
+        search_params(0.9f, sp, k);
+        tgsf_ctx* c = nullptr;
+        if (g_api.create(&sp, devices[0], &c) == TGSF_OK) {
+            const std::string end(100, 'A');
+            int64_t tot[22]; uint32_t hits[22], first[22];
+            (void)g_api.adapter_totals(c, reinterpret_cast<const uint8_t*>(end.data()), 1, 100, 100, k, tot, hits, first);
+        } else c = nullptr;
+        publish_search(c);
+    } else publish_search(nullptr);
     if (!devices.empty()) (void)g_api.prepare_device(devices[0]);
     for (std::thread& t : up) t.join();
     g_device_s = now_s() - t0 - g_load_s;
 }
 }
 
-void lib_start(const std::vector<int>& devices)
+void lib_start(const std::vector<int>& devices, bool search_context)
 {
     g_started = true;
-    g_thread = std::thread(load, devices);
+    g_thread = std::thread(load, devices, search_context);
+}
+
+SearchContext search_context()
+{
+    if (!g_started) lib_start({});
+    std::unique_lock<std::mutex> l(g_search_m);
+    g_search_cv.wait(l, [] { return g_search_published; });
+    return SearchContext{&g_api, g_search_ctx};
 }
 
 const Api& lib()
diff --git a/tgsfilter_amd/host/api.h b/tgsfilter_amd/host/api.h
--- a/tgsfilter_amd/host/api.h
+++ b/tgsfilter_amd/host/api.h
@@ -18,6 +18,7 @@
     decltype(&tgsf_counters) counters;
     decltype(&tgsf_counters_used) counters_used;
     decltype(&tgsf_align_windows) align_windows;
+    decltype(&tgsf_adapter_totals) adapter_totals;
     decltype(&tgsf_last_error) last_error;
     decltype(&tgsf_profile) profile;
     decltype(&tgsf_stage_times) stage_times;
@@ -37,8 +38,10 @@
 void rccl_start();
 const RcclApi* rccl_lib();
 
-void lib_start(const std::vector<int>& devices);
+void lib_start(const std::vector<int>& devices, bool search_context = false);
 const Api& lib();
+struct SearchContext { const Api* api; tgsf_ctx* ctx; };
+SearchContext search_context();
 void lib_times(double& load_s, double& device_s);
 
 }
diff --git a/tgsfilter_amd/host/prepass.cpp b/tgsfilter_amd/host/prepass.cpp
--- a/tgsfilter_amd/host/prepass.cpp
+++ b/tgsfilter_amd/host/prepass.cpp
@@ -59,13 +59,13 @@
     return r;
 }
 
-static int check_base_content(const std::vector<std::string>& ends, int check_len, int seq_num, float end_bias)
+static int check_base_content(const std::vector<uint8_t>& ends, int check_len, int seq_num, float end_bias)
 {
     static const struct Col { uint8_t of[256]; Col() { memset(of, 4, sizeof of); of['A'] = of['a'] = 0; of['T'] = of['t'] = 1; of['G'] = of['g'] = 2; of['C'] = of['c'] = 3; } } col;
     std::vector<int> cnt5((size_t)check_len * 5, 0);
-    for (const std::string& s : ends) {
-        const size_t n = std::min(s.size(), (size_t)check_len);
-        for (size_t i = 0; i < n; i++) cnt5[i * 5 + col.of[(unsigned char)s[i]]]++;
+    for (size_t at = 0; at + (size_t)check_len <= ends.size(); at += (size_t)check_len) {
+        const uint8_t* s = ends.data() + at;
+        for (size_t i = 0; i < (size_t)check_len; i++) cnt5[i * 5 + col.of[s[i]]]++;
     }
     std::vector<int> cnt((size_t)check_len * 4, 0);
     for (int i = 0; i < check_len; i++) for (int j = 0; j < 4; j++) cnt[(size_t)i * 4 + j] = cnt5[(size_t)i * 5 + j];
@@ -88,20 +88,13 @@
 static double pp_now() { return std::chrono::duration<double>(std::chrono::steady_clock::now().time_since_epoch()).count(); }
 static double g_pp_create = 0, g_pp_align = 0; static int g_pp_calls = 0;
 
-static void adapter_search(const Options& o, const std::vector<std::string>& ends, std::string& adapter, float& depth)
-{
-    adapter.clear(); depth = 0.f;
-    float min_sim = o.mid_sim;
-    if (min_sim < 0.9) min_sim = 0.9f;
-    if (ends.empty()) return;
-
-    tgsf_params p;
+void search_params(float min_sim, tgsf_params& p, int32_t k[22])
+{
     memset(&p, 0, sizeof p);
     p.struct_size = sizeof p;
     p.min_len = 100; p.max_len = 2147483647; p.min_q = 0; p.max_q = 255; p.bc_len = 0;
     p.end_len = 0; p.extra_len = 0; p.end_sim = 0.75f; p.mid_sim = 0.9f; p.filter = 1; p.qtype = 33;
     p.n_adapters = 22;
-    int k[22];
     size_t max_q = 0;
     for (int a = 0; a < 22; a++) {
         p.adapters[a] = kAdapterLib[a];
@@ -110,39 +103,28 @@
         max_q = std::max(max_q, (size_t)p.adapter_len[a]);
     }
     p.end_match_len = 2; p.mid_match_len = (int)max_q;
-    const size_t per_call = 4096;
-    p.max_batch_reads = (uint32_t)(per_call * 22 / (22 * 2) + 64);
+    p.max_batch_reads = (uint32_t)(4096 * 22 / (22 * 2) + 64);
     p.max_batch_bases = 1 << 20; p.max_read_len = 1 << 16;
-    tgsf_ctx* ctx = nullptr;
-    const double c0 = pp_now();
-    if (lib().create(&p, o.devices.empty() ? o.device : o.devices[0], &ctx) != TGSF_OK) { std::cerr << "Error: " << lib().last_error(nullptr) << std::endl; quit(255); }
-
-    g_pp_create += pp_now() - c0;
+}
+
+static void adapter_search(const SearchContext& S, const int32_t* k, float min_sim, const std::vector<uint8_t>& ends, int check_len,
+                           std::string& adapter, float& depth)
+{
+    adapter.clear(); depth = 0.f;
+    if (ends.empty()) return;
+    int64_t totals[22]; uint32_t hits[22], first_end[22];
+    const double a0 = pp_now();
+    if (S.api->adapter_totals(S.ctx, ends.data(), (uint32_t)(ends.size() / (size_t)check_len), (uint32_t)check_len, (uint32_t)check_len,
+                              k, totals, hits, first_end) != TGSF_OK) {
+        std::cerr << "Error: " << S.api->last_error(S.ctx) << std::endl; quit(255);
+    }
+    g_pp_align += pp_now() - a0; g_pp_calls++;
+    std::vector<std::pair<uint32_t, int>> order;
+    for (int a = 0; a < 22; a++) if (hits[a]) order.emplace_back(first_end[a], a);
+    std::sort(order.begin(), order.end());
     std::unordered_map<int, int> maps;
-    std::vector<uint8_t> buf; std::vector<uint64_t> off; std::vector<uint32_t> len; std::vector<uint8_t> aid;
-    std::vector<int32_t> kk, res, eds;
-    for (size_t b = 0; b < ends.size(); b += per_call) {
-        const size_t e = std::min(ends.size(), b + per_call);
-        buf.clear(); off.clear(); len.clear(); aid.clear(); kk.clear();
-        for (size_t i = b; i < e; i++) {
-            const uint64_t o0 = buf.size();
-            buf.insert(buf.end(), ends[i].begin(), ends[i].end());
-            if (ends[i].empty()) continue;
-            for (int a = 0; a < 22; a++) { off.push_back(o0); len.push_back((uint32_t)ends[i].size()); aid.push_back((uint8_t)a); kk.push_back(k[a]); }
-        }
-        const uint32_t n = (uint32_t)off.size();
-        if (!n) continue;
-        res.assign((size_t)n * 4, 0); eds.assign((size_t)n * 2, 0);
-        const double a0 = pp_now();
-        if (lib().align_windows(ctx, buf.data(), buf.size(), off.data(), len.data(), aid.data(), kk.data(), n, res.data(), eds.data()) != TGSF_OK) {
-            std::cerr << "Error: " << lib().last_error(ctx) << std::endl; quit(255);
-        }
-        g_pp_align += pp_now() - a0; g_pp_calls++;
-        for (uint32_t i = 0; i < n; i++)
-            if (res[(size_t)i * 4 + 1] > 0)
-                maps[(int)aid[i]] += res[(size_t)i * 4 + 2] - res[(size_t)i * 4 + 0];
-    }
-    lib().destroy(ctx);
+    for (const std::pair<uint32_t, int>& fa : order) maps[fa.second] += 0;
+    for (const std::pair<uint32_t, int>& fa : order) maps[fa.second] = (int)totals[fa.second];
     std::vector<std::pair<int, int>> vec(maps.begin(), maps.end());
     std::sort(vec.begin(), vec.end(), [](const std::pair<int, int>& a, const std::pair<int, int>& b) { return a.second > b.second; });
     if (vec.empty()) return;
@@ -159,7 +141,7 @@
     int check_len = std::max(std::max(o.end_len, o.bc_len), 100);
     int min_len = std::max(o.min_len, 2 * check_len);
     const int max_seq = std::max(o.ad_num, o.bc_num);
-    std::vector<std::string> ends5, ends3;
+    std::vector<uint8_t> ends5, ends3;
     const bool need5 = o.filter && (o.head_trim < 0 || o.adapter_file.empty());
     const bool need3 = o.filter && (o.tail_trim < 0 || o.adapter_file.empty());
     int seq_num = 0, min_qc = 255, max_qc = 0;
@@ -171,8 +153,8 @@
             if (L < min_len) continue;
             if (seq_num >= max_seq) break;
             seq_num++;
-            if (need5) ends5.emplace_back(r.seq, (size_t)check_len);
-            if (need3) ends3.emplace_back(rev_comp(std::string(r.seq + (L - check_len), (size_t)check_len)));
+            if (need5) ends5.insert(ends5.end(), r.seq, r.seq + check_len);
+            if (need3) { const std::string rc = rev_comp(std::string(r.seq + (L - check_len), (size_t)check_len)); ends3.insert(ends3.end(), rc.begin(), rc.end()); }
             if (has_qual)
                 for (int i = 0; i < check_len; i++) { const char c = r.qual[i]; if (min_qc > c) min_qc = c; if (max_qc < c) max_qc = c; }
         }
@@ -208,9 +190,21 @@
         }
         if (o.head_trim < 0 && o.tail_trim < 0 && R.trim5p > o.bc_len) R.trim5p = o.bc_len;
         t_bc = pp_now() - t1;
-        if (o.adapter_file.empty()) {
-            adapter_search(o, ends5, R.adapter5p, R.depth5p);
-            adapter_search(o, ends3, R.adapter3p, R.depth3p);
+        if (o.adapter_file.empty() && (!ends5.empty() || !ends3.empty())) {
+            float min_sim = o.mid_sim;
+            if (min_sim < 0.9) min_sim = 0.9f;
+            tgsf_params sp;
+            int32_t k[22];
+            search_params(min_sim, sp, k);
+            const double c0 = pp_now();
+            SearchContext S = search_context();
+            if (!S.ctx) {
+                S.api = &lib();
+                if (S.api->create(&sp, o.devices.empty() ? o.device : o.devices[0], &S.ctx) != TGSF_OK) { std::cerr << "Error: " << S.api->last_error(nullptr) << std::endl; quit(255); }
+            }
+            g_pp_create += pp_now() - c0;
+            adapter_search(S, k, min_sim, ends5, check_len, R.adapter5p, R.depth5p);
+            adapter_search(S, k, min_sim, ends3, check_len, R.adapter3p, R.depth3p);
         }
     }
     if (getenv("TGSF_TIMING"))
diff --git a/tgsfilter_amd/host/prepass.h b/tgsfilter_amd/host/prepass.h
--- a/tgsfilter_amd/host/prepass.h
+++ b/tgsfilter_amd/host/prepass.h
@@ -5,12 +5,15 @@
 
 #include "fastx.h"
 #include "options.h"
+#include "tgsf.h"
 
 namespace host {
 
 extern const char* const kAdapterLib[22];
 
 std::string rev_comp(const std::string& s);
+
+void search_params(float min_sim, tgsf_params& p, int32_t k[22]);
 
 struct PrepassResult {
     int qtype = 0;
diff --git a/tgsfilter_amd/host/run.h b/tgsfilter_amd/host/run.h
--- a/tgsfilter_amd/host/run.h
+++ b/tgsfilter_amd/host/run.h
@@ -80,6 +80,8 @@
     std::atomic<uint64_t> stream_text{0};
     std::atomic<double> stream_share{0.0};
     std::mutex gpu_time_m;
+    double t_create_max = 0, t_first_enter = 0;
+    std::atomic<bool> first_entered{false};
     bool numa_bind = false;
     std::vector<int> dev_node;
     std::vector<double> dev_submit_s;
diff --git a/tgsfilter_amd/host/run_pipeline.cpp b/tgsfilter_amd/host/run_pipeline.cpp
--- a/tgsfilter_amd/host/run_pipeline.cpp
+++ b/tgsfilter_amd/host/run_pipeline.cpp
@@ -119,13 +119,16 @@
     CpuScope cpu(CPU_FEEDER);
     const Api& L = *api;
     if (numa_bind) bind_to_node_of(k);
+    const double c0 = now_s();
     if (L.create(&p, ctx_dev[k], &ctxs[k]) != TGSF_OK) die(L.last_error(nullptr));
+    { std::lock_guard<std::mutex> l(gpu_time_m); t_create_max = std::max(t_create_max, now_s() - c0); }
     tgsf_ctx* fctx = ctxs[k];
     if (timing) (void)L.profile(fctx, 1);
     for (;;) {
         std::shared_ptr<Batch> b = to_gpu->get();
         if (!b) break;
         const double g0 = now_s();
+        if (!first_entered.exchange(true)) t_first_enter = g0 - (t_start + t_prepass);
         if (b->res.size() < b->recs.size()) b->res.resize(b->recs.size());
         const size_t fneed = (size_t)(b->bases / (uint64_t)std::max(p.min_len, 1)) + b->recs.size() + 16;
         if (b->frags.size() < fneed) b->frags.resize(fneed);
diff --git a/tgsfilter_amd/host/run_report.cpp b/tgsfilter_amd/host/run_report.cpp
--- a/tgsfilter_amd/host/run_report.cpp
+++ b/tgsfilter_amd/host/run_report.cpp
@@ -279,6 +279,8 @@
                         "first batch filtered after %.3f, fill tail %.3f, closing the output %.3f; stages overlap) | stats+report %.3f | %s (fallocate %.3f, mapping the reserved pages %.3f, fill threads busy %.3f summed)\n",
                 now_s() - t_start, t_prepass, t_libwait, t_load, t_dev, t_pipe, t_parse, ctxs.size(), t_gpu, t_write, t_widle, t_first,
                 mapped.t_fill_tail, mapped.t_close, now_s() - t_p0 - t_pipe, mapped_out ? "output: fallocate + mapped fill" : "output: writev", mapped.sink.t_falloc, mapped.t_populate_wait(), t_busy);
+        fprintf(stderr, "PREPASS: behind it: longest tgsf_create among %zu feeders %.3f s, first tgsf_submit entered %.3f s after the pre-pass ended\n",
+                ctxs.size(), t_create_max, t_first_enter);
         fprintf(stderr, "RESERVE: planner waited %.3f s for pages of the output file\n", mapped.t_claim_wait);
     }
     if (timing) {
diff --git a/tgsfilter_amd/host/run_setup.cpp b/tgsfilter_amd/host/run_setup.cpp
--- a/tgsfilter_amd/host/run_setup.cpp
+++ b/tgsfilter_amd/host/run_setup.cpp
@@ -73,7 +73,7 @@
 void Run::open_input()
 {
     if (o.devices.empty()) o.devices.push_back(o.device);
-    lib_start(o.devices);
+    lib_start(o.devices, o.filter && o.adapter_file.empty() && !(sharded && link.rank > 0));
     if (sharded && shard_may_use_rccl) rccl_start();
 
     const bool coded = o.in_type == 2 || (o.in_file.size() > 3 && o.in_file.compare(o.in_file.size() - 3, 3, ".gz") == 0);
```
